# qitianwu/SGFormer

Measured on AMD Instinct MI355X. Metric: SGFormer fwd+bwd nodes/sec on ogbn-products full-graph, higher is better.
Workload: dtype bf16

## Files before the change

### include/sgf.h

```cpp
#ifndef SGF_H_
#define SGF_H_

#include <stddef.h>
#include <stdint.h>

#ifdef __cplusplus
extern "C" {
#endif

#define SGF_VERSION 666

#define SGF_F32 0
#define SGF_BF16 1
#define SGF_F32_BF16X3 2

#define SGF_OK 0
#define SGF_E_INVALID (-1)
#define SGF_E_WORKSPACE (-2)
#define SGF_E_HIP (-3)
#define SGF_E_UNSUPPORTED (-4)

int sgf_version(void);
const char* sgf_last_error(void);
int sgf_reload_env(void);

size_t sgf_csr_workspace_bytes(int64_t nnz, int64_t n);
int sgf_csr_build(const int64_t* edge_index, int64_t nnz, int64_t n, int64_t* rowptr,
                  int32_t* colind, float* val, int32_t* deg, void* workspace,
                  size_t workspace_bytes, void* stream);

int sgf_csr_transpose(const int64_t* edge_index, int64_t nnz, int64_t n, const int32_t* deg,
                      const int64_t* rowptr, const int32_t* colind, int64_t* t_rowptr,
                      int32_t* t_colind, float* t_val, int32_t* is_symmetric, void* workspace,
                      size_t workspace_bytes, void* stream);

size_t sgf_subgraph_workspace_bytes(int64_t nnz, int64_t n);
int sgf_subgraph_plan(const int64_t* edge_index, int64_t nnz, int64_t n, const int64_t* subset,
                      int64_t m, int32_t* relabel, int64_t* total, void* workspace,
                      size_t workspace_bytes, void* stream);
int sgf_subgraph_emit(const int64_t* edge_index, int64_t nnz, int64_t n, const int32_t* relabel,
                      int32_t relabel_nodes, int64_t total, int64_t* out, int64_t* out_eid,
                      void* workspace, size_t workspace_bytes, void* stream);

size_t sgf_subgraph_csr_plan_workspace_bytes(int64_t m);
size_t sgf_subgraph_csr_emit_workspace_bytes(int64_t m, int64_t total);
int sgf_subgraph_csr_plan(const int64_t* rowptr, const int32_t* colind, int64_t n, const int64_t* subset, int64_t m,
                          int32_t* local_of, int64_t* rowptr_b, int32_t* deg_b, int64_t* total, void* workspace,
                          size_t workspace_bytes, void* stream);
int sgf_subgraph_csr_emit(const int64_t* rowptr, const int32_t* colind, int64_t n, const int64_t* subset, int64_t m,
                          int32_t* local_of, const int64_t* rowptr_b, const int32_t* deg_b, int64_t total, int32_t* colind_b,
                          float* val_b, int64_t* edge_index_b, void* workspace, size_t workspace_bytes, void* stream);

size_t sgf_graph_prologue_workspace_bytes(int64_t m, int64_t n);
int sgf_graph_prologue_plan(const int64_t* edge_index, int64_t m, int64_t n, int32_t to_undirected,
                            int32_t remove_self_loops, int32_t add_self_loops, int64_t* total,
                            void* workspace, size_t workspace_bytes, void* stream);
int sgf_graph_prologue_emit(int64_t m, int64_t n, int32_t to_undirected, int32_t add_self_loops,
                            int64_t total, int64_t* out, void* workspace, size_t workspace_bytes,
                            void* stream);

int sgf_spmm(const int64_t* rowptr, const int32_t* colind, const float* val, const void* x,
             int64_t ldx, int64_t n_cols, void* y, int64_t ldy, int64_t n_rows, int32_t d,
             int32_t dtype, void* stream);

int32_t sgf_spmm_segment_len(void);
int32_t sgf_spmm_arm(int32_t d, int32_t dtype, int64_t ldx, int64_t ldy, int64_t n_cols, int32_t aligned16,
                     int32_t stream);
size_t sgf_spmm_split_workspace_bytes(int64_t long_segments, int32_t d);
int sgf_spmm_split(const int64_t* rowptr, const int32_t* colind, const float* val, const void* x,
                   int64_t ldx, int64_t n_cols, void* y, int64_t ldy, int64_t n_rows, int32_t d, int32_t dtype,
                   int64_t long_len, int64_t long_segments, void* workspace, size_t workspace_bytes,
                   void* stream);

size_t sgf_spmm_packed_bytes(int64_t n, int32_t slot_bytes);
int32_t sgf_spmm_packed_supported(int32_t d, int32_t dtype, int64_t ldx, int64_t ldy, int64_t n_cols, int32_t aligned16,
                                  int32_t slot_bytes);
int sgf_spmm_packed(const int64_t* rowptr, const int32_t* colind, const float* val, const void* x, int64_t ldx,
                    int64_t n_cols, const void* packed, int32_t slot_bytes, const int32_t* overflow, void* y, int64_t ldy,
                    int64_t n_rows, int32_t d, int32_t dtype, int64_t long_len, int64_t long_segments, void* workspace,
                    size_t workspace_bytes, void* stream);

int sgf_spmm_stream(const int64_t* rowptr, const int32_t* colind, const float* val, const void* x,
                    int64_t ldx, int64_t n_cols, void* y, int64_t ldy, int64_t n_rows, int32_t d, int32_t dtype,
                    int64_t long_len, int64_t long_segments, void* workspace, size_t workspace_bytes,
                    void* stream);

size_t sgf_reorder_workspace_bytes(int64_t nnz, int64_t n);
int sgf_reorder(const int64_t* edge_index, int64_t nnz, int64_t n, int32_t iters1, int32_t iters2,
                int32_t* perm, int32_t* inv, int32_t* community, void* workspace, size_t workspace_bytes,
                void* stream);
size_t sgf_spmm_plan_workspace_bytes(int64_t nnz, int64_t n, int32_t rows_per_block);
int sgf_spmm_plan(const int64_t* rowptr, const int32_t* colind, const float* val, int64_t n, int64_t nnz,
                  int32_t rows_per_block, int32_t lds_rows, int64_t long_len, int32_t* ecode, float* eval,
// ... 26 lines not shown
int sgf_spmm_tile_pack_layout(const int32_t* blk_row, int64_t nb, const int64_t* tile_ptr, const void* tiles,
                              int64_t n_frag, int32_t* grp, int64_t* pool_units, void* workspace,
                              size_t workspace_bytes, void* stream);
int sgf_spmm_tile_pack(const int32_t* blk_row, int64_t nb, const int64_t* tile_ptr, const void* tiles, int64_t n_frag,
                       const int32_t* grp, void* pool, int64_t pool_units, void* stream);
int sgf_spmm_tile(const int32_t* blk_row, int64_t nb, int32_t block_rows, const int32_t* sh_ptr, const int32_t* sh_cols,
                  const int64_t* tile_ptr, const int32_t* grp, const void* pool, const int64_t* rem_rowptr,
                  const int32_t* rem_col, const float* rem_val, const void* x, int64_t ldx, int64_t n_cols, void* y, int64_t ldy,
                  int64_t n_rows, int32_t d, int32_t dtype, int64_t long_len, int64_t long_segments,
                  void* workspace, size_t workspace_bytes, void* stream);

size_t sgf_neighbor_sample_workspace_bytes(int64_t m, int64_t edge_cap);
int sgf_neighbor_sample_mark(int32_t* local_of, const int32_t* ids, int64_t count, int32_t base, void* stream);
int sgf_neighbor_sample_hop(const int64_t* rowptr, const int32_t* colind, const int32_t* frontier, int64_t m,
                            int32_t frontier_local0, int32_t fanout, uint64_t seed, uint64_t batch, int32_t hop,
                            int32_t* local_of, int32_t n_known, int64_t edge_cap, int32_t* edge_src_local,
                            int32_t* edge_dst_local, int32_t* src_global, int32_t* new_nodes, int64_t* counts,
                            void* workspace, size_t workspace_bytes, void* stream);

size_t sgf_neighbor_sample_batch_workspace_bytes(int64_t batch_size, const int32_t* fanouts, int32_t hops, int64_t* node_cap,
                                                  int64_t* edge_cap);
int sgf_neighbor_sample_batch(const int64_t* rowptr, const int32_t* colind, const int32_t* seeds, int64_t batch_size,
                              const int32_t* fanouts, int32_t hops, uint64_t seed, uint64_t batch, int32_t* local_of,
                              int32_t* nodes, int64_t node_cap, int32_t* edge_src_local, int32_t* edge_dst_local,
                              int64_t edge_cap, int64_t* counts, void* workspace, size_t workspace_bytes, void* stream);

int32_t sgf_sampled_csr_supported(int32_t max_fanout);
size_t sgf_sampled_csr_build_workspace_bytes(int64_t node_cap, int64_t edge_cap);
int sgf_sampled_csr_build(const int32_t* edge_src_local, const int32_t* edge_dst_local, const int64_t* counts,
                          int64_t node_cap, int64_t edge_cap, int32_t max_fanout, int64_t* rowptr_b, int32_t* colind_b,
                          float* val_b, int32_t* deg_b, void* workspace, size_t workspace_bytes, void* stream);
size_t sgf_sampled_csr_transpose_workspace_bytes(int64_t n, int64_t nnz);
int sgf_sampled_csr_transpose(const int64_t* rowptr, const int32_t* colind, const float* val, int64_t n, int64_t nnz,
                              int64_t* t_rowptr, int32_t* t_colind, float* t_val, void* workspace, size_t workspace_bytes,
                              void* stream);

int sgf_gather_rows(const void* src, int64_t lds, int32_t src_dtype, int64_t n_src, const void* idx,
                    int32_t idx_is_int64, int64_t n_out, int32_t d, void* dst, int64_t ldd,
                    int32_t dst_dtype, void* stream);
int sgf_pad_rows(const void* src, int64_t lds, int32_t src_dtype, int64_t n_src, const void* idx, int32_t idx_is_int64,
                 int64_t n_out, int32_t d, int32_t d_pad, void* dst, int64_t ldd, int32_t dst_dtype, void* stream);

int64_t sgf_attn_stats_len(int32_t heads, int32_t d);
size_t sgf_attn_workspace_bytes(int64_t n, int32_t heads, int32_t d);
int32_t sgf_attn_max_blocks(void);
int32_t sgf_attn_tile_rows(int32_t kind, int32_t d, int32_t dtype);

int sgf_attn_fwd_reduce(const void* q, int64_t ldq, const void* k, int64_t ldk, const void* v,
                        int64_t ldv, int64_t n, int32_t heads, int32_t v_heads, int32_t d,
                        int32_t dtype, float* stats, void* workspace, size_t workspace_bytes,
                        void* stream);

int sgf_attn_fwd_apply(const void* q, int64_t ldq, const void* v, int64_t ldv, int64_t n,
                       double n_total, int32_t heads, int32_t v_heads, int32_t d, int32_t dtype,
                       const float* stats, void* out, int64_t ldo, float* den, void* o_heads,
                       void* stream);

int64_t sgf_attn_bstats_len(int32_t heads, int32_t d);

int sgf_attn_bwd_reduce(const void* q, int64_t ldq, const void* g, int64_t ldg, const void* o,
                        int64_t ldo, const float* den, int64_t n, int32_t heads, int32_t d,
                        int32_t dtype, float* bstats, void* workspace, size_t workspace_bytes,
                        void* stream);

int sgf_attn_bwd_apply(const void* q, int64_t ldq, const void* k, int64_t ldk, const void* v,
                       int64_t ldv, const void* g, int64_t ldg, const void* o, int64_t ldo,
                       const float* den, int64_t n, double n_total, int32_t heads,
                       int32_t v_heads, int32_t d, int32_t dtype, const float* stats,
                       float* bstats, void* dq, int64_t lddq, void* dk, int64_t lddk,
                       void* dv, int64_t lddv, void* stream);
int sgf_attn_bwd_reduce_heads(const void* q, int64_t ldq, const void* g, int64_t ldg, const void* o, int64_t ldo,
                              const float* den, int64_t n, int32_t heads, int32_t d, int32_t dtype, float* bstats,
                              void* workspace, size_t workspace_bytes, void* stream);
int sgf_attn_bwd_apply_heads(const void* q, int64_t ldq, const void* k, int64_t ldk, const void* v, int64_t ldv, const void* g,
                             int64_t ldg, const void* o, int64_t ldo, const float* den, int64_t n, double n_total,
                             int32_t heads, int32_t v_heads, int32_t d, int32_t dtype, const float* stats, float* bstats,
                             void* dq, int64_t lddq, void* dk, int64_t lddk, void* dv, int64_t lddv, void* stream);

int64_t sgf_attn_h_bstats_len(int32_t d);
int32_t sgf_attn_h_supported(int32_t d, int32_t dtype);
int sgf_attn_h_fwd(const void* h, int64_t ldh, int64_t n, int32_t d, int32_t dtype, const float* M,
                   const float* m, const float* w, const float* beta, void* out, int64_t ldo,
                   float* den, void* stream);
int sgf_attn_h_bwd_reduce(const void* h, int64_t ldh, const void* g, int64_t ldg, const void* o,
                          int64_t ldo, const float* den, int64_t n, int32_t d, int32_t dtype,
                          float* hstats, void* workspace, size_t workspace_bytes, void* stream);
int sgf_attn_h_bwd_apply(const void* h, int64_t ldh, const void* g, int64_t ldg, const void* o,
                         int64_t ldo, const float* den, int64_t n, int32_t d, int32_t dtype,
                         const float* M, const float* w, const float* D, const float* ds, void* dh,
                         int64_t lddh, void* workspace, size_t workspace_bytes, void* stream);
size_t sgf_attn_h_bwd_apply_workspace_bytes(int64_t n, int32_t d, int32_t dtype);
int32_t sgf_attn_h_bwd_split_supported(int32_t d, int32_t dtype);
int sgf_attn_h_bwd_pre(const void* g, int64_t ldg, const void* o, int64_t ldo, const float* den, int64_t n, int32_t d,
                       int32_t dtype, const float* M, const float* w, void* workspace, size_t workspace_bytes,
                       float* rowscal, void* stream);
int sgf_attn_h_bwd_reduce_scaled(const void* h, int64_t ldh, const void* g, int64_t ldg, const float* rowscal, int64_t n,
                                 int32_t d, int32_t dtype, float* hstats, void* workspace, size_t workspace_bytes,
                                 void* stream);
int sgf_attn_h_bwd_post(const void* h, int64_t ldh, int64_t n, int32_t d, int32_t dtype, const float* D, const float* ds,
                        const void* workspace, size_t workspace_bytes, const void* addend, int64_t ldadd, void* dh,
                        int64_t lddh, void* stream);

size_t sgf_attn_h_small_saved_bytes(int32_t d_in, int32_t d_out);
size_t sgf_attn_h_small_workspace_bytes(int32_t d_in, int32_t d_out);
int sgf_attn_h_small_fwd(const float* G, int64_t ldg, const float* s, float n_rows, float n_total, const float* wq,
                         const float* bq, const float* wk, const float* bk, const float* wv, const float* bv, int64_t ldw,
                         int32_t d_in, int32_t d_out, float* M, int64_t ldm, float* m, float* w, float* beta, void* saved,
                         size_t saved_bytes, void* stream);
int sgf_attn_h_small_bwd(const float* dM, int64_t lddm, const float* dw, const float* dm, const float* dbeta, float n_total,
                         int32_t d_in, int32_t d_out, const void* saved, size_t saved_bytes, float* dG2, int64_t lddg,
                         float* ds, float* gwq, float* gbq, float* gwk, float* gbk, float* gwv, float* gbv, int64_t ldgw,
                         void* workspace, size_t workspace_bytes, void* stream);

size_t sgf_gram_workspace_bytes(int64_t n, int32_t m, int32_t k);
int sgf_gram(const void* a, int64_t lda, int32_t m, const void* b, int64_t ldb, int32_t k,
             int64_t n, int32_t dtype, float* c, int64_t ldc, float* colsum_a, void* workspace,
             size_t workspace_bytes, void* stream);
int sgf_gram2(const void* a, int64_t lda, int32_t m, const void* b1, int64_t ldb1, const void* b2, int64_t ldb2, int32_t k,
              int64_t n, int32_t dtype, float* c1, int64_t ldc1, float* c2, int64_t ldc2, float* colsum_a, void* workspace,
              size_t workspace_bytes, void* stream);

int sgf_ln_fwd(const void* x, int64_t ldx, const void* res, int64_t ldr, float a, float b,
               const float* gamma, const float* beta, int32_t relu, float eps, int64_t n,
               int32_t d, int32_t dtype, void* y, int64_t ldy, float* mean, float* rstd,
               void* stream);

size_t sgf_ln_bwd_workspace_bytes(int64_t n, int32_t d);
int sgf_ln_bwd(const void* dy, int64_t lddy, const void* y, int64_t ldy, const void* x,
               int64_t ldx, const void* res, int64_t ldr, float a, float b, const float* gamma,
               int32_t relu, const float* mean, const float* rstd, int64_t n, int32_t d,
               int32_t dtype, void* dx, int64_t lddx, void* dres, int64_t lddres, float* dgamma,
               float* dbeta, void* workspace, size_t workspace_bytes, void* stream);

size_t sgf_colstats_workspace_bytes(int64_t n, int32_t d);
int sgf_colstats(const void* x, int64_t ldx, const float* shift, int64_t n, int32_t d,
                 int32_t dtype, float* stats, void* workspace, size_t workspace_bytes,
                 void* stream);
int sgf_bn_finalize(const float* sums, const float* shift, double n_total, float eps, float momentum, float* running_mean,
                    float* running_var, int32_t d, float* mean, float* rstd, void* stream);
int sgf_bn_apply(const void* x, int64_t ldx, const float* mean, const float* rstd,
                 const float* gamma, const float* beta, const void* res, int64_t ldr,
                 int32_t relu, int64_t n, int32_t d, int32_t dtype, void* y, int64_t ldy,
                 void* stream);
int sgf_bn_apply_packed(const void* x, int64_t ldx, const float* mean, const float* rstd, const float* gamma,
                        const float* beta, const void* res, int64_t ldr, int32_t relu, int64_t n, int32_t d, int32_t dtype,
                        void* y, int64_t ldy, void* packed, int32_t slot_bytes, int32_t* overflow, void* stream);
int sgf_bn_bwd_stats(const void* dy, int64_t lddy, const void* x, int64_t ldx, const float* mean,
                     const float* rstd, const float* gamma, const float* beta, int32_t relu,
                     int64_t n, int32_t d, int32_t dtype, float* stats, void* workspace,
                     size_t workspace_bytes, void* stream);
int sgf_bn_bwd_stats2(const void* dy, int64_t lddy, const void* dy2, int64_t lddy2, const void* x, int64_t ldx,
                      const float* mean, const float* rstd, const float* gamma, const float* beta, int32_t relu, int64_t n,
                      int32_t d, int32_t dtype, float* stats, void* workspace, size_t workspace_bytes, void* stream);
int32_t sgf_gram_ln_bwd_supported(int32_t m, int32_t k, int32_t dtype);
int sgf_gram_ln_bwd(const void* g, int64_t ldg, const void* xin, int64_t ldx, const float* mean, const float* rstd,
                    const float* gamma, const float* beta, int32_t relu, int32_t m, const void* b, int64_t ldb, int32_t k,
                    int64_t n, int32_t dtype, float* c, int64_t ldc, float* colsum, float* dgamma, float* dbeta, void* workspace,
                    size_t workspace_bytes, void* stream);
int32_t sgf_gram_bn_bwd_supported(int32_t m, int32_t k, int32_t dtype);
int sgf_gram_bn_bwd(const void* g1, int64_t ldg1, const void* g2, int64_t ldg2, const void* z, int64_t ldz, const float* mean,
                    const float* rstd, const float* gamma, const float* beta, int32_t relu, const float* stats, float inv_n,
                    int32_t training, int32_t m, const void* b, int64_t ldb, int32_t k, int64_t n, int32_t dtype, float* c,
                    int64_t ldc, float* colsum, void* workspace, size_t workspace_bytes, void* stream);
int32_t sgf_gram2_bn_bwd_supported(int32_t m, int32_t k, int64_t n, int32_t dtype);
int sgf_gram2_bn_bwd(const void* g, int64_t ldg, const void* z, int64_t ldz, const float* mean, const float* rstd,
                     const float* gamma, const float* beta, int32_t relu, const float* stats, float inv_n, int32_t training,
                     int32_t m, const void* b1, int64_t ldb1, const void* b2, int64_t ldb2, int32_t k, int64_t n, int32_t dtype,
                     void* dz, int64_t lddz, float* c1, int64_t ldc1, float* c2, int64_t ldc2, float* colsum, void* workspace,
                     size_t workspace_bytes, void* stream);
int sgf_bn_bwd_apply(const void* dy, int64_t lddy, const void* x, int64_t ldx, const float* mean,
                     const float* rstd, const float* gamma, const float* beta, int32_t relu,
                     const float* stats, float inv_n, int32_t training, int64_t n, int32_t d,
                     int32_t dtype, void* dx, int64_t lddx, void* stream);

int32_t sgf_combine_fc_supported(int32_t d, int32_t classes, int32_t dtype);
int sgf_combine_fc_fwd(const void* x1, int64_t ld1, float a, const void* x2, int64_t ld2, float b,
                       const float* w, const float* bias, int64_t n, int32_t d, int32_t classes,
                       int32_t dtype, float* logits, int64_t ldl, void* stream);
int sgf_combine_fc_bwd(const float* dlogits, int64_t lddl, const float* w, int64_t n, int32_t d,
                       int32_t classes, float a, float b, int32_t dtype, void* dx1, int64_t ld1, void* dx2,
                       int64_t ld2, void* stream);
int sgf_combine_fc_fwd_mapped(const void* x1, int64_t ld1, float a, const void* x2, int64_t ld2, float b, const float* w,
                              const float* bias, int64_t n, int32_t d, int32_t classes, int32_t dtype, float* logits,
                              int64_t ldl, const int32_t* row_map, void* stream);
int sgf_combine_fc_bwd_mapped(const float* dlogits, int64_t lddl, const float* w, int64_t n, int32_t d, int32_t classes,
                              float a, float b, int32_t dtype, void* dx1, int64_t ld1, void* dx2, int64_t ld2,
                              const int32_t* row_map, void* stream);
int sgf_combine_fc_bwd_g(const float* dlogits, int64_t lddl, const float* w, int64_t n, int32_t d, int32_t classes, float a,
                         float b, int32_t dtype, void* dx1, int64_t ld1, void* dx2, int64_t ld2, const int32_t* row_map,
                         void* g_out, int64_t ldg, void* stream);

int32_t sgf_gcn_epilogue_supported(int32_t d_in, int32_t d_out, int32_t dtype);
size_t sgf_gcn_epilogue_workspace_bytes(int64_t n, int32_t d_out);
int sgf_gcn_epilogue_stats(const void* a, int64_t lda, const void* w, int64_t ldw, const float* bias,
                           int64_t n, int32_t d_in, int32_t d_out, int32_t dtype, void* y, int64_t ldy,
                           const float* shift, float* stats, void* workspace, size_t workspace_bytes,
                           void* stream);
int sgf_gcn_epilogue_dx2(const void* dy, int64_t lddy, const void* w1, const void* w2, int64_t ldw, int64_t n, int32_t d,
                         int32_t dtype, void* dx1, int64_t lddx1, void* dx2, int64_t lddx2, int32_t pair, void* stream);

int32_t sgf_gcn_epilogue_dx2_acc_supported(int32_t d, int32_t dtype);
int sgf_gcn_epilogue_dx2_acc(const void* dz, int64_t lddz, const void* w, int64_t ldw, int64_t n, int32_t d, int32_t dtype,
                             void* dy, int64_t lddy, const void* gadd, int64_t ldg, const void* acc_in, int64_t ldai,
                             void* acc_out, int64_t ldao, void* stream);
int sgf_gcn_epilogue_dx(const void* dy, int64_t lddy, const void* w, int64_t ldw, int64_t n, int32_t d_in,
                        int32_t d_out, int32_t dtype, void* dx, int64_t lddx, void* stream);
int sgf_gcn_epilogue_apply(const void* y, int64_t ldy, const float* mean, const float* rstd, const float* gamma,
                           const float* beta, const void* res, int64_t ldr, int32_t relu, int64_t n, int32_t d,
                           int32_t dtype, void* out, int64_t ldo, void* stream);
int32_t sgf_gcn_bn_bwd_dx_supported(int32_t d, int32_t dtype);
size_t sgf_gcn_bn_bwd_dx_workspace_bytes(int64_t n, int32_t d);
int sgf_gcn_bn_bwd_dx(const void* gy, int64_t ldg, const void* z, int64_t ldz, const float* mean, const float* rstd,
                      const float* gamma, const float* beta, int32_t relu, const float* stats, float inv_n,
                      int32_t training, const void* w, int64_t ldw, int64_t n, int32_t d, int32_t dtype, void* dz,
                      int64_t lddz, void* dy, int64_t lddy, const void* acc_in, void* acc_out, size_t acc_bytes,
                      void* dx0, int64_t lddx0, int32_t add_gy, void* workspace, size_t workspace_bytes, void* stream);
int32_t sgf_gcn_epilogue_cat_supported(int32_t d, int32_t dtype);
int sgf_gcn_epilogue_cat(const void* a1, int64_t lda1, const void* a2, int64_t lda2, const void* w, int64_t ldw,
                         const float* bias, int64_t n, int32_t d, int32_t dtype, void* y, int64_t ldy, const float* shift,
                         float* stats, void* workspace, size_t workspace_bytes, void* stream);
size_t sgf_gcn_epilogue_partial_bytes(int64_t n, int32_t d_out);
size_t sgf_gcn_epilogue_dtype_partial_bytes(int64_t n, int32_t d_out, int32_t dtype);
int sgf_gcn_epilogue_partial(const void* a, int64_t lda, const void* w, int64_t ldw, const float* bias, int64_t n,
                             int32_t d_in, int32_t d_out, int32_t dtype, void* partial, size_t partial_bytes,
                             void* stream);
int sgf_gcn_epilogue_stats_add(const void* a, int64_t lda, const void* w, int64_t ldw, const void* partial,
                               size_t partial_bytes, int64_t n, int32_t d_in, int32_t d_out, int32_t dtype,
                               void* y, int64_t ldy, const float* shift, float* stats, void* workspace,
                               size_t workspace_bytes, void* stream);

int32_t sgf_stem_pair_supported(int32_t d_in, int32_t d_out, int32_t dtype);
int32_t sgf_row_lap_rows(int32_t kind, int32_t d, int32_t dtype);
int sgf_stem_pair(const void* x, int64_t ldx, int64_t n, int32_t d_in, const void* w0, int64_t ldw0,
                  const float* bias0, const void* w1, int64_t ldw1, const float* bias1, int32_t d_out, int32_t dtype,
                  void* y0, int64_t ldy0, void* y1, int64_t ldy1, const float* shift0, float* stats0, void* workspace,
                  size_t workspace_bytes, void* stream);

int sgf_gemm(const void* a, int64_t a_rs, int64_t a_cs, int32_t a_dtype, const void* b, int64_t b_rs, int64_t b_cs,
             int32_t b_dtype, int64_t m, int32_t n, int64_t k, float alpha, const float* alpha_dev, const float* bias,
             float beta, const void* addend, int64_t ldadd, int32_t add_dtype, void* c, int64_t ldc, int32_t c_dtype,
             void* stream);

int sgf_axpby(const void* x1, int64_t ld1, float a, const void* x2, int64_t ld2, float b,
              int64_t n, int32_t d, int32_t dtype, void* y, int64_t ldy, void* stream);

int sgf_dropout(const void* x, int64_t ldx, const void* res, int64_t ldr, float p, uint64_t seed,
                int64_t n, int32_t d, int32_t dtype, void* y, int64_t ldy, void* stream);

int sgf_dropout_dev(const void* x, int64_t ldx, const void* res, int64_t ldr, float p,
                    const uint64_t* seed_slot, int64_t n, int32_t d, int32_t dtype, void* y, int64_t ldy,
                    void* stream);

size_t sgf_nll_workspace_bytes(int64_t m);
int sgf_nll_fwd(const void* logits, int64_t ldl, int64_t n, int32_t c, int32_t dtype,
                const int64_t* labels, const int64_t* idx, int64_t m, float* loss_sum,
                void* workspace, size_t workspace_bytes, void* stream);
int sgf_nll_bwd(const void* logits, int64_t ldl, int64_t n, int32_t c, int32_t dtype,
                const int64_t* labels, const int64_t* idx, int64_t m, const float* gout,
                float inv_denom, void* dlogits, int64_t ldd, void* stream);

#define SGF_BCE_TARGET_F32 0
#define SGF_BCE_TARGET_I64 1
#define SGF_BCE_TARGET_CLASS 2
size_t sgf_bce_workspace_bytes(int64_t m, int32_t c);
int sgf_bce_fwd(const void* logits, int64_t ldl, int64_t n, int32_t c, int32_t dtype, const void* target,
                int64_t ldt, int32_t target_kind, const int64_t* idx, int64_t m, float inv_denom,
                float* loss_sum, void* workspace, size_t workspace_bytes, void* stream);
int sgf_bce_bwd(const void* logits, int64_t ldl, int64_t n, int32_t c, int32_t dtype, const void* target,
                int64_t ldt, int32_t target_kind, const int64_t* idx, int64_t m, const float* gout,
                float inv_denom, void* dlogits, int64_t ldd, void* stream);

#define SGF_METRIC_TARGET_F32 0
#define SGF_METRIC_TARGET_I64 1
size_t sgf_rocauc_workspace_bytes(int64_t m, int32_t c);
int sgf_rocauc_counts(const void* logits, int64_t ldl, int64_t n, int32_t c, int32_t dtype, const void* target,
                      int64_t ldt, int32_t target_kind, const int64_t* idx, int64_t m, int64_t* counts,
                      void* workspace, size_t workspace_bytes, void* stream);
size_t sgf_argmax_workspace_bytes(int64_t m, int32_t c);
int sgf_argmax_count(const void* logits, int64_t ldl, int64_t n, int32_t c, int32_t dtype, const void* labels,
                     int64_t label_stride, int32_t label_kind, const int64_t* idx, int64_t m, int64_t* counts,
                     void* workspace, size_t workspace_bytes, void* stream);

int32_t sgf_head_rows_supported(int32_t d, int32_t classes, int32_t dtype);
size_t sgf_head_rows_fwd_workspace_bytes(int64_t m);
size_t sgf_head_rows_bwd_workspace_bytes(int64_t m, int32_t d, int32_t classes);
int sgf_head_rows_fwd(const void* x1, int64_t ld1, float a, const void* x2, int64_t ld2, float b, const float* w,
                      const float* bias, int64_t n, int32_t d, int32_t classes, int32_t dtype, const int64_t* idx,
                      int64_t m, float* logits, int64_t ldl, const int64_t* labels, float* lse, float* loss_sum,
                      int64_t* counts, void* workspace, size_t workspace_bytes, void* stream);
int sgf_head_rows_bwd(const void* x1, int64_t ld1, float a, const void* x2, int64_t ld2, float b, const float* w,
                      int64_t n, int32_t d, int32_t classes, int32_t dtype, const int64_t* idx, int64_t m,
                      const float* dlogits, int64_t lddl, const float* logits, int64_t ldl, const float* lse,
                      const int64_t* labels, const float* gout, float inv_denom, void* dx1, int64_t ldd1, void* dx2,
                      int64_t ldd2, float* dw, float* db, void* workspace, size_t workspace_bytes, void* stream);

int32_t sgf_pair_sigmoid_supported(int32_t heads, int32_t v_heads, int32_t d, int32_t dtype);
size_t sgf_pair_sigmoid_workspace_bytes(int64_t n, int64_t l, int32_t heads);
int64_t sgf_pair_sigmoid_lap_rows(int32_t which, int32_t heads, int32_t d, int32_t dtype, int32_t laps);
int sgf_pair_sigmoid_fwd(const void* q, int64_t ldq, const void* k, int64_t ldk, const void* v, int64_t ldv, int64_t n,
                         int64_t l, int32_t heads, int32_t v_heads, int32_t d, int32_t dtype, void* out, int64_t ldo,
                         float* rowsum, void* stream);
int sgf_pair_sigmoid_bwd_q(const void* g, int64_t ldg, const void* out, int64_t ldo, const float* rowsum, const void* q,
                           int64_t ldq, const void* k, int64_t ldk, const void* v, int64_t ldv, int64_t n, int64_t l,
                           int32_t heads, int32_t v_heads, int32_t d, int32_t dtype, void* dq, int64_t lddq, void* workspace,
                           size_t workspace_bytes, void* stream);
int sgf_pair_sigmoid_bwd_kv(const void* g, int64_t ldg, const float* rowsum, const void* q, int64_t ldq, const void* k,
                            int64_t ldk, const void* v, int64_t ldv, int64_t n, int64_t l, int32_t heads, int32_t v_heads,
                            int32_t d, int32_t dtype, void* dk, int64_t lddk, void* dv, int64_t lddv, const void* workspace,
                            size_t workspace_bytes, void* stream);

int sgf_sum_n(const void* const* xs_host, const int64_t* lds_host, int32_t k, int64_t n, int32_t d,
              int32_t dtype, void* y, int64_t ldy, void* stream);

size_t sgf_colsum_workspace_bytes(int64_t n, int32_t d);
int sgf_colsum(const void* x, int64_t ldx, int64_t n, int32_t d, int32_t dtype, float* out,
               void* workspace, size_t workspace_bytes, void* stream);

int32_t sgf_comm_available(void);
int32_t sgf_comm_unique_id_bytes(void);
// ... 13 lines not shown
```

### sgformer_amd/_lib.py

```python
from __future__ import annotations

import ctypes
import os
from ctypes import c_char_p, c_double, c_float, c_int32, c_int64, c_size_t, c_uint64, c_void_p

_HERE = os.path.dirname(os.path.abspath(__file__))
LIB_PATH = os.path.join(_HERE, "lib", "libsgf.so")

SGF_F32 = 0
SGF_BF16 = 1
SGF_F32_BF16X3 = 2
SGF_OK = 0
SGF_E_INVALID = -1
SGF_E_WORKSPACE = -2
SGF_E_HIP = -3
SGF_E_UNSUPPORTED = -4
SGF_BCE_TARGET_F32 = 0
SGF_BCE_TARGET_I64 = 1
SGF_BCE_TARGET_CLASS = 2
SGF_METRIC_TARGET_F32 = 0
SGF_METRIC_TARGET_I64 = 1

_lib = None

# ... 6 lines not shown
    "sgf_csr_build": (c_int32, [_P, c_int64, c_int64, _P, _P, _P, _P, _P, c_size_t, _P]),
    "sgf_csr_transpose": (c_int32, [_P, c_int64, c_int64, _P, _P, _P, _P, _P, _P, _P, _P, c_size_t, _P]),
    "sgf_subgraph_workspace_bytes": (c_size_t, [c_int64, c_int64]),
    "sgf_subgraph_plan": (c_int32, [_P, c_int64, c_int64, _P, c_int64, _P, _P, _P, c_size_t, _P]),
    "sgf_subgraph_emit": (c_int32, [_P, c_int64, c_int64, _P, c_int32, c_int64, _P, _P, _P, c_size_t, _P]),
    "sgf_subgraph_csr_plan_workspace_bytes": (c_size_t, [c_int64]),
    "sgf_subgraph_csr_emit_workspace_bytes": (c_size_t, [c_int64, c_int64]),
    "sgf_subgraph_csr_plan": (c_int32, [_P, _P, c_int64, _P, c_int64, _P, _P, _P, _P, _P, c_size_t, _P]),
    "sgf_subgraph_csr_emit": (c_int32, [_P, _P, c_int64, _P, c_int64, _P, _P, _P, c_int64, _P, _P, _P, _P, c_size_t, _P]),
    "sgf_graph_prologue_workspace_bytes": (c_size_t, [c_int64, c_int64]),
    "sgf_graph_prologue_plan": (c_int32, [_P, c_int64, c_int64, c_int32, c_int32, c_int32, _P, _P, c_size_t, _P]),
    "sgf_graph_prologue_emit": (c_int32, [c_int64, c_int64, c_int32, c_int32, c_int64, _P, _P, c_size_t, _P]),
    "sgf_spmm": (c_int32, [_P, _P, _P, _P, c_int64, c_int64, _P, c_int64, c_int64, c_int32, c_int32, _P]),
    "sgf_spmm_segment_len": (c_int32, []),
    "sgf_spmm_arm": (c_int32, [c_int32, c_int32, c_int64, c_int64, c_int64, c_int32, c_int32]),
    "sgf_spmm_split_workspace_bytes": (c_size_t, [c_int64, c_int32]),
    "sgf_spmm_split": (c_int32, [_P, _P, _P, _P, c_int64, c_int64, _P, c_int64, c_int64, c_int32, c_int32, c_int64,
                                 c_int64, _P, c_size_t, _P]),
    "sgf_spmm_packed_bytes": (c_size_t, [c_int64, c_int32]),
    "sgf_spmm_packed_supported": (c_int32, [c_int32, c_int32, c_int64, c_int64, c_int64, c_int32, c_int32]),
    "sgf_spmm_packed": (c_int32, [_P, _P, _P, _P, c_int64, c_int64, _P, c_int32, _P, _P, c_int64, c_int64, c_int32, c_int32,
                                  c_int64, c_int64, _P, c_size_t, _P]),
    "sgf_spmm_stream": (c_int32, [_P, _P, _P, _P, c_int64, c_int64, _P, c_int64, c_int64, c_int32, c_int32, c_int64,
                                  c_int64, _P, c_size_t, _P]),
    "sgf_reorder_workspace_bytes": (c_size_t, [c_int64, c_int64]),
    "sgf_reorder": (c_int32, [_P, c_int64, c_int64, c_int32, c_int32, _P, _P, _P, _P, c_size_t, _P]),
    "sgf_spmm_plan_workspace_bytes": (c_size_t, [c_int64, c_int64, c_int32]),
    "sgf_spmm_plan": (c_int32, [_P, _P, _P, c_int64, c_int64, c_int32, c_int32, c_int64, _P, _P, _P, _P, _P, _P,
                                _P, c_size_t, _P]),
    "sgf_spmm_lds_rows_len": (c_int32, [c_int32]),
    "sgf_spmm_blocked_arm": (c_int32, [c_int32, c_int32, c_int64, c_int64, c_int64, c_int32, c_int32, c_int32]),
    "sgf_spmm_blocked": (c_int32, [_P, _P, _P, _P, _P, _P, _P, c_int64, _P, c_int64, c_int64, c_int32, c_int32,
                                   c_int32, c_int32, c_int64, c_int64, _P, c_size_t, _P]),
    "sgf_spmm_tile_supported": (c_int32, [c_int32, c_int32]),
    "sgf_spmm_tile_blocks": (c_int32, [_P, c_int64, c_int32, _P, c_int64, _P, _P]),
    "sgf_spmm_tile_plan_workspace_bytes": (c_size_t, [c_int64, c_int64, c_int64]),
    "sgf_spmm_tile_plan": (c_int32, [_P, _P, _P, c_int64, c_int64, _P, c_int64, c_int32, c_int32, c_int64, _P, _P, _P,
                                     _P, _P, _P, _P, _P, _P, c_size_t, _P]),
    "sgf_spmm_tile_fill": (c_int32, [_P, _P, _P, _P, c_int64, c_int64, _P, c_int64, _P, c_int64, _P, _P, _P, _P, _P]),
    "sgf_spmm_tile_sparse_len": (c_int32, []),
    "sgf_spmm_tile_pack_workspace_bytes": (c_size_t, [c_int64]),
    "sgf_spmm_tile_pack_layout": (c_int32, [_P, c_int64, _P, _P, c_int64, _P, _P, _P, c_size_t, _P]),
    "sgf_spmm_tile_pack": (c_int32, [_P, c_int64, _P, _P, c_int64, _P, _P, c_int64, _P]),
    "sgf_spmm_tile": (c_int32, [_P, c_int64, c_int32, _P, _P, _P, _P, _P, _P, _P, _P, _P, c_int64, c_int64, _P, c_int64,
                                c_int64, c_int32, c_int32, c_int64, c_int64, _P, c_size_t, _P]),
    "sgf_neighbor_sample_workspace_bytes": (c_size_t, [c_int64, c_int64]),
    "sgf_neighbor_sample_mark": (c_int32, [_P, _P, c_int64, c_int32, _P]),
    "sgf_neighbor_sample_batch_workspace_bytes": (c_size_t, [c_int64, _P, c_int32, _P, _P]),
    "sgf_neighbor_sample_batch": (c_int32, [_P, _P, _P, c_int64, _P, c_int32, c_uint64, c_uint64, _P, _P, c_int64, _P, _P,
                                            c_int64, _P, _P, c_size_t, _P]),
    "sgf_neighbor_sample_hop": (c_int32, [_P, _P, _P, c_int64, c_int32, c_int32, c_uint64, c_uint64, c_int32, _P, c_int32,
                                          c_int64, _P, _P, _P, _P, _P, _P, c_size_t, _P]),
    "sgf_sampled_csr_supported": (c_int32, [c_int32]),
    "sgf_sampled_csr_build_workspace_bytes": (c_size_t, [c_int64, c_int64]),
    "sgf_sampled_csr_build": (c_int32, [_P, _P, _P, c_int64, c_int64, c_int32, _P, _P, _P, _P, _P, c_size_t, _P]),
    "sgf_sampled_csr_transpose_workspace_bytes": (c_size_t, [c_int64, c_int64]),
    "sgf_sampled_csr_transpose": (c_int32, [_P, _P, _P, c_int64, c_int64, _P, _P, _P, _P, c_size_t, _P]),
    "sgf_gather_rows": (c_int32, [_P, c_int64, c_int32, c_int64, _P, c_int32, c_int64, c_int32, _P, c_int64,
                                  c_int32, _P]),
    "sgf_pad_rows": (c_int32, [_P, c_int64, c_int32, c_int64, _P, c_int32, c_int64, c_int32, c_int32, _P, c_int64,
                               c_int32, _P]),
    "sgf_attn_stats_len": (c_int64, [c_int32, c_int32]),
    "sgf_attn_bstats_len": (c_int64, [c_int32, c_int32]),
    "sgf_attn_workspace_bytes": (c_size_t, [c_int64, c_int32, c_int32]),
    "sgf_attn_max_blocks": (c_int32, []),
    "sgf_attn_tile_rows": (c_int32, [c_int32, c_int32, c_int32]),
    "sgf_row_lap_rows": (c_int32, [c_int32, c_int32, c_int32]),
    "sgf_attn_fwd_reduce": (c_int32, [_P, c_int64, _P, c_int64, _P, c_int64, c_int64, c_int32, c_int32,
                                      c_int32, c_int32, _P, _P, c_size_t, _P]),
    "sgf_attn_fwd_apply": (c_int32, [_P, c_int64, _P, c_int64, c_int64, c_double, c_int32, c_int32,
                                     c_int32, c_int32, _P, _P, c_int64, _P, _P, _P]),
    "sgf_attn_bwd_reduce": (c_int32, [_P, c_int64, _P, c_int64, _P, c_int64, _P, c_int64, c_int32,
                                      c_int32, c_int32, _P, _P, c_size_t, _P]),
    "sgf_attn_bwd_apply": (c_int32, [_P, c_int64, _P, c_int64, _P, c_int64, _P, c_int64, _P, c_int64,
                                     _P, c_int64, c_double, c_int32, c_int32, c_int32, c_int32, _P, _P,
                                     _P, c_int64, _P, c_int64, _P, c_int64, _P]),
    "sgf_attn_bwd_reduce_heads": (c_int32, [_P, c_int64, _P, c_int64, _P, c_int64, _P, c_int64, c_int32,
                                            c_int32, c_int32, _P, _P, c_size_t, _P]),
    "sgf_attn_bwd_apply_heads": (c_int32, [_P, c_int64, _P, c_int64, _P, c_int64, _P, c_int64, _P, c_int64,
                                           _P, c_int64, c_double, c_int32, c_int32, c_int32, c_int32, _P, _P,
                                           _P, c_int64, _P, c_int64, _P, c_int64, _P]),
    "sgf_attn_h_bstats_len": (c_int64, [c_int32]),
    "sgf_attn_h_fwd": (c_int32, [_P, c_int64, c_int64, c_int32, c_int32, _P, _P, _P, _P, _P, c_int64, _P, _P]),
    "sgf_attn_h_bwd_reduce": (c_int32, [_P, c_int64, _P, c_int64, _P, c_int64, _P, c_int64, c_int32, c_int32,
                                        _P, _P, c_size_t, _P]),
    "sgf_attn_h_bwd_apply": (c_int32, [_P, c_int64, _P, c_int64, _P, c_int64, _P, c_int64, c_int32, c_int32,
                                       _P, _P, _P, _P, _P, c_int64, _P, c_size_t, _P]),
    "sgf_attn_h_bwd_apply_workspace_bytes": (c_size_t, [c_int64, c_int32, c_int32]),
    "sgf_attn_h_bwd_split_supported": (c_int32, [c_int32, c_int32]),
    "sgf_attn_h_supported": (c_int32, [c_int32, c_int32]),
    "sgf_attn_h_bwd_pre": (c_int32, [_P, c_int64, _P, c_int64, _P, c_int64, c_int32, c_int32, _P, _P, _P, c_size_t, _P, _P]),
    "sgf_attn_h_bwd_reduce_scaled": (c_int32, [_P, c_int64, _P, c_int64, _P, c_int64, c_int32, c_int32, _P, _P, c_size_t,
                                               _P]),
    "sgf_attn_h_bwd_post": (c_int32, [_P, c_int64, c_int64, c_int32, c_int32, _P, _P, _P, c_size_t, _P, c_int64, _P,
                                      c_int64, _P]),
    "sgf_attn_h_small_saved_bytes": (c_size_t, [c_int32, c_int32]),
    "sgf_attn_h_small_workspace_bytes": (c_size_t, [c_int32, c_int32]),
    "sgf_attn_h_small_fwd": (c_int32, [_P, c_int64, _P, c_float, c_float, _P, _P, _P, _P, _P, _P, c_int64, c_int32, c_int32,
                                       _P, c_int64, _P, _P, _P, _P, c_size_t, _P]),
    "sgf_attn_h_small_bwd": (c_int32, [_P, c_int64, _P, _P, _P, c_float, c_int32, c_int32, _P, c_size_t, _P, c_int64, _P,
                                       _P, _P, _P, _P, _P, _P, c_int64, _P, c_size_t, _P]),
    "sgf_gram_workspace_bytes": (c_size_t, [c_int64, c_int32, c_int32]),
    "sgf_gram": (c_int32, [_P, c_int64, c_int32, _P, c_int64, c_int32, c_int64, c_int32, _P, c_int64, _P,
                           _P, c_size_t, _P]),
    "sgf_gram2": (c_int32, [_P, c_int64, c_int32, _P, c_int64, _P, c_int64, c_int32, c_int64, c_int32, _P, c_int64, _P,
                            c_int64, _P, _P, c_size_t, _P]),
    "sgf_ln_fwd": (c_int32, [_P, c_int64, _P, c_int64, c_float, c_float, _P, _P, c_int32, c_float,
                             c_int64, c_int32, c_int32, _P, c_int64, _P, _P, _P]),
    "sgf_ln_bwd_workspace_bytes": (c_size_t, [c_int64, c_int32]),
    "sgf_ln_bwd": (c_int32, [_P, c_int64, _P, c_int64, _P, c_int64, _P, c_int64, c_float, c_float, _P,
                             c_int32, _P, _P, c_int64, c_int32, c_int32, _P, c_int64, _P, c_int64, _P,
                             _P, _P, c_size_t, _P]),
    "sgf_colstats_workspace_bytes": (c_size_t, [c_int64, c_int32]),
    "sgf_colstats": (c_int32, [_P, c_int64, _P, c_int64, c_int32, c_int32, _P, _P, c_size_t, _P]),
    "sgf_bn_finalize": (c_int32, [_P, _P, c_double, c_float, c_float, _P, _P, c_int32, _P, _P, _P]),
    "sgf_bn_apply": (c_int32, [_P, c_int64, _P, _P, _P, _P, _P, c_int64, c_int32, c_int64, c_int32,
                               c_int32, _P, c_int64, _P]),
    "sgf_bn_apply_packed": (c_int32, [_P, c_int64, _P, _P, _P, _P, _P, c_int64, c_int32, c_int64, c_int32, c_int32, _P,
                                      c_int64, _P, c_int32, _P, _P]),
    "sgf_bn_bwd_stats": (c_int32, [_P, c_int64, _P, c_int64, _P, _P, _P, _P, c_int32, c_int64, c_int32,
                                   c_int32, _P, _P, c_size_t, _P]),
    "sgf_bn_bwd_stats2": (c_int32, [_P, c_int64, _P, c_int64, _P, c_int64, _P, _P, _P, _P, c_int32, c_int64, c_int32,
                                    c_int32, _P, _P, c_size_t, _P]),
    "sgf_gram_ln_bwd_supported": (c_int32, [c_int32, c_int32, c_int32]),
    "sgf_gram_ln_bwd": (c_int32, [_P, c_int64, _P, c_int64, _P, _P, _P, _P, c_int32, c_int32, _P, c_int64, c_int32, c_int64,
                                  c_int32, _P, c_int64, _P, _P, _P, _P, c_size_t, _P]),
    "sgf_gram_bn_bwd_supported": (c_int32, [c_int32, c_int32, c_int32]),
    "sgf_gram_bn_bwd": (c_int32, [_P, c_int64, _P, c_int64, _P, c_int64, _P, _P, _P, _P, c_int32, _P, c_float, c_int32,
                                  c_int32, _P, c_int64, c_int32, c_int64, c_int32, _P, c_int64, _P, _P, c_size_t, _P]),
    "sgf_gram2_bn_bwd_supported": (c_int32, [c_int32, c_int32, c_int64, c_int32]),
    "sgf_gram2_bn_bwd": (c_int32, [_P, c_int64, _P, c_int64, _P, _P, _P, _P, c_int32, _P, c_float, c_int32, c_int32, _P, c_int64,
                                   _P, c_int64, c_int32, c_int64, c_int32, _P, c_int64, _P, c_int64, _P, c_int64, _P, _P,
                                   c_size_t, _P]),
    "sgf_bn_bwd_apply": (c_int32, [_P, c_int64, _P, c_int64, _P, _P, _P, _P, c_int32, _P, c_float,
                                   c_int32, c_int64, c_int32, c_int32, _P, c_int64, _P]),
    "sgf_dropout": (c_int32, [_P, c_int64, _P, c_int64, c_float, c_uint64, c_int64, c_int32, c_int32, _P,
                              c_int64, _P]),
    "sgf_dropout_dev": (c_int32, [_P, c_int64, _P, c_int64, c_float, _P, c_int64, c_int32, c_int32, _P,
                                  c_int64, _P]),
    "sgf_nll_workspace_bytes": (c_size_t, [c_int64]),
    "sgf_nll_fwd": (c_int32, [_P, c_int64, c_int64, c_int32, c_int32, _P, _P, c_int64, _P, _P, c_size_t, _P]),
    "sgf_nll_bwd": (c_int32, [_P, c_int64, c_int64, c_int32, c_int32, _P, _P, c_int64, _P, c_float, _P,
                              c_int64, _P]),
    "sgf_bce_workspace_bytes": (c_size_t, [c_int64, c_int32]),
    "sgf_bce_fwd": (c_int32, [_P, c_int64, c_int64, c_int32, c_int32, _P, c_int64, c_int32, _P, c_int64, c_float, _P, _P,
                              c_size_t, _P]),
    "sgf_bce_bwd": (c_int32, [_P, c_int64, c_int64, c_int32, c_int32, _P, c_int64, c_int32, _P, c_int64, _P, c_float, _P,
                              c_int64, _P]),
    "sgf_rocauc_workspace_bytes": (c_size_t, [c_int64, c_int32]),
    "sgf_rocauc_counts": (c_int32, [_P, c_int64, c_int64, c_int32, c_int32, _P, c_int64, c_int32, _P, c_int64, _P, _P,
                                    c_size_t, _P]),
    "sgf_argmax_workspace_bytes": (c_size_t, [c_int64, c_int32]),
    "sgf_argmax_count": (c_int32, [_P, c_int64, c_int64, c_int32, c_int32, _P, c_int64, c_int32, _P, c_int64, _P, _P,
                                   c_size_t, _P]),
    "sgf_head_rows_supported": (c_int32, [c_int32, c_int32, c_int32]),
    "sgf_head_rows_fwd_workspace_bytes": (c_size_t, [c_int64]),
    "sgf_head_rows_bwd_workspace_bytes": (c_size_t, [c_int64, c_int32, c_int32]),
    "sgf_head_rows_fwd": (c_int32, [_P, c_int64, c_float, _P, c_int64, c_float, _P, _P, c_int64, c_int32, c_int32, c_int32,
                                    _P, c_int64, _P, c_int64, _P, _P, _P, _P, _P, c_size_t, _P]),
    "sgf_head_rows_bwd": (c_int32, [_P, c_int64, c_float, _P, c_int64, c_float, _P, c_int64, c_int32, c_int32, c_int32,
                                    _P, c_int64, _P, c_int64, _P, c_int64, _P, _P, _P, c_float, _P, c_int64, _P, c_int64,
                                    _P, _P, _P, c_size_t, _P]),
    "sgf_pair_sigmoid_supported": (c_int32, [c_int32, c_int32, c_int32, c_int32]),
    "sgf_pair_sigmoid_workspace_bytes": (c_size_t, [c_int64, c_int64, c_int32]),
    "sgf_pair_sigmoid_lap_rows": (c_int64, [c_int32, c_int32, c_int32, c_int32, c_int32]),
    "sgf_pair_sigmoid_fwd": (c_int32, [_P, c_int64, _P, c_int64, _P, c_int64, c_int64, c_int64, c_int32, c_int32, c_int32,
                                       c_int32, _P, c_int64, _P, _P]),
    "sgf_pair_sigmoid_bwd_q": (c_int32, [_P, c_int64, _P, c_int64, _P, _P, c_int64, _P, c_int64, _P, c_int64, c_int64,
                                         c_int64, c_int32, c_int32, c_int32, c_int32, _P, c_int64, _P, c_size_t, _P]),
    "sgf_pair_sigmoid_bwd_kv": (c_int32, [_P, c_int64, _P, _P, c_int64, _P, c_int64, _P, c_int64, c_int64, c_int64, c_int32,
                                          c_int32, c_int32, c_int32, _P, c_int64, _P, c_int64, _P, c_size_t, _P]),
    "sgf_sum_n": (c_int32, [_P, _P, c_int32, c_int64, c_int32, c_int32, _P, c_int64, _P]),
    "sgf_colsum_workspace_bytes": (c_size_t, [c_int64, c_int32]),
    "sgf_colsum": (c_int32, [_P, c_int64, c_int64, c_int32, c_int32, _P, _P, c_size_t, _P]),
    "sgf_combine_fc_supported": (c_int32, [c_int32, c_int32, c_int32]),
    "sgf_combine_fc_fwd": (c_int32, [_P, c_int64, c_float, _P, c_int64, c_float, _P, _P, c_int64, c_int32, c_int32,
                                     c_int32, _P, c_int64, _P]),
    "sgf_combine_fc_bwd": (c_int32, [_P, c_int64, _P, c_int64, c_int32, c_int32, c_float, c_float, c_int32, _P,
                                     c_int64, _P, c_int64, _P]),
    "sgf_combine_fc_fwd_mapped": (c_int32, [_P, c_int64, c_float, _P, c_int64, c_float, _P, _P, c_int64, c_int32, c_int32,
                                     c_int32, _P, c_int64, _P, _P]),
    "sgf_combine_fc_bwd_g": (c_int32, [_P, c_int64, _P, c_int64, c_int32, c_int32, c_float, c_float, c_int32, _P, c_int64, _P,
                                       c_int64, _P, _P, c_int64, _P]),
    "sgf_combine_fc_bwd_mapped": (c_int32, [_P, c_int64, _P, c_int64, c_int32, c_int32, c_float, c_float, c_int32, _P,
                                     c_int64, _P, c_int64, _P, _P]),
    "sgf_gcn_epilogue_supported": (c_int32, [c_int32, c_int32, c_int32]),
    "sgf_gcn_epilogue_workspace_bytes": (c_size_t, [c_int64, c_int32]),
    "sgf_gcn_epilogue_stats": (c_int32, [_P, c_int64, _P, c_int64, _P, c_int64, c_int32, c_int32, c_int32, _P, c_int64,
                                         _P, _P, _P, c_size_t, _P]),
    "sgf_gcn_epilogue_dx": (c_int32, [_P, c_int64, _P, c_int64, c_int64, c_int32, c_int32, c_int32, _P, c_int64, _P]),
    "sgf_gcn_epilogue_dx2": (c_int32, [_P, c_int64, _P, _P, c_int64, c_int64, c_int32, c_int32, _P, c_int64, _P, c_int64,
                                       c_int32, _P]),
    "sgf_gcn_epilogue_dx2_acc_supported": (c_int32, [c_int32, c_int32]),
    "sgf_gcn_epilogue_dx2_acc": (c_int32, [_P, c_int64, _P, c_int64, c_int64, c_int32, c_int32, _P, c_int64, _P, c_int64, _P,
                                           c_int64, _P, c_int64, _P]),
    "sgf_gcn_epilogue_apply": (c_int32, [_P, c_int64, _P, _P, _P, _P, _P, c_int64, c_int32, c_int64, c_int32,
                               c_int32, _P, c_int64, _P]),
    "sgf_gcn_bn_bwd_dx_supported": (c_int32, [c_int32, c_int32]),
    "sgf_gcn_bn_bwd_dx_workspace_bytes": (c_size_t, [c_int64, c_int32]),
    "sgf_gcn_bn_bwd_dx": (c_int32, [_P, c_int64, _P, c_int64, _P, _P, _P, _P, c_int32, _P, c_float, c_int32, _P, c_int64,
                                    c_int64, c_int32, c_int32, _P, c_int64, _P, c_int64, _P, _P, c_size_t, _P, c_int64,
                                    c_int32, _P, c_size_t, _P]),
    "sgf_gcn_epilogue_cat_supported": (c_int32, [c_int32, c_int32]),
    "sgf_gcn_epilogue_cat": (c_int32, [_P, c_int64, _P, c_int64, _P, c_int64, _P, c_int64, c_int32, c_int32, _P, c_int64,
                                       _P, _P, _P, c_size_t, _P]),
    "sgf_gcn_epilogue_partial_bytes": (c_size_t, [c_int64, c_int32]),
    "sgf_gcn_epilogue_dtype_partial_bytes": (c_size_t, [c_int64, c_int32, c_int32]),
    "sgf_gcn_epilogue_partial": (c_int32, [_P, c_int64, _P, c_int64, _P, c_int64, c_int32, c_int32, c_int32, _P,
                                           c_size_t, _P]),
    "sgf_gcn_epilogue_stats_add": (c_int32, [_P, c_int64, _P, c_int64, _P, c_size_t, c_int64, c_int32, c_int32,
                                             c_int32, _P, c_int64, _P, _P, _P, c_size_t, _P]),
    "sgf_stem_pair_supported": (c_int32, [c_int32, c_int32, c_int32]),
    "sgf_stem_pair": (c_int32, [_P, c_int64, c_int64, c_int32, _P, c_int64, _P, _P, c_int64, _P, c_int32, c_int32, _P,
                                c_int64, _P, c_int64, _P, _P, _P, c_size_t, _P]),
    "sgf_gemm": (c_int32, [_P, c_int64, c_int64, c_int32, _P, c_int64, c_int64, c_int32, c_int64, c_int32, c_int64, c_float,
                           _P, _P, c_float, _P, c_int64, c_int32, _P, c_int64, c_int32, _P]),
    "sgf_comm_available": (c_int32, []),
    "sgf_comm_unique_id_bytes": (c_int32, []),
    "sgf_comm_unique_id": (c_int32, [_P]),
    "sgf_comm_create": (c_int32, [_P, c_int32, c_int32, _P]),
    "sgf_comm_destroy": (c_int32, [_P]),
    "sgf_comm_all_reduce_f32": (c_int32, [_P, _P, c_int64, _P]),
    "sgf_comm_all_gather": (c_int32, [_P, _P, _P, c_int64, _P]),
    "sgf_comm_all_to_all": (c_int32, [_P, _P, _P, _P, _P, _P, _P, _P]),
    "sgf_axpby": (c_int32, [_P, c_int64, c_float, _P, c_int64, c_float, c_int64, c_int32, c_int32, _P,
                            c_int64, _P]),
}


class SgfError(RuntimeError):
    """A libsgf call returned a non-zero status (mirrors PyTorch: RuntimeError)."""


def load():
    global _lib
    if _lib is not None:
        return _lib
    if not os.path.exists(LIB_PATH):
        raise SgfError(
            f"libsgf.so not found at {LIB_PATH}: build it with `make` (or "
            "`python -c 'import __graft_entry__ as g; g.build()'`).  sgformer_amd has no CPU / "
            "eager fallback by design.")
    import torch
    lib = ctypes.CDLL(LIB_PATH, mode=ctypes.RTLD_GLOBAL)
    for name, (res, args) in SIGNATURES.items():
        fn = getattr(lib, name)
        fn.restype = res
        fn.argtypes = args
    _lib = lib
    return lib


def available() -> bool:
    return os.path.exists(LIB_PATH)


def check(rc: int, what: str):
    if rc != SGF_OK:
        msg = load().sgf_last_error()
        raise SgfError(f"{what} failed (rc={rc}): {msg.decode() if msg else '?'}")


def call(name: str, *args):
    rc = getattr(load(), name)(*args)
    check(rc, name)
```

### sgformer_amd/csrc/head.hip

```cpp
#include "common.h"

namespace sgf {
namespace {

typedef short bf16x8 __attribute__((ext_vector_type(8)));

constexpr int kHeadThreads = 256;
constexpr int kMaxClasses = 64;

__device__ __forceinline__ uint32_t pack2(float lo, float hi) {
  return static_cast<uint32_t>(f32_to_bf16(lo)) | (static_cast<uint32_t>(f32_to_bf16(hi)) << 16);
}
__device__ __forceinline__ float lo16(uint32_t u) { return __uint_as_float(u << 16); }
__device__ __forceinline__ float hi16(uint32_t u) { return __uint_as_float(u & 0xffff0000u); }

union Frag {
  bf16x8 v;
  uint4 u;
};

template <int DP>
__global__ __launch_bounds__(kHeadThreads) void k_head_fwd_bf16(
    const uint16_t* __restrict__ x1, int64_t ld1, float a, const uint16_t* __restrict__ x2, int64_t ld2, float b,
    const float* __restrict__ w, const float* __restrict__ bias, int64_t n, int d, int c,
// ... 101 lines not shown
  unsigned char* const patch = patch_all + wid * 32 * PROW;
  unsigned char* const pw = patch + 4 * hi * PROW + 2 * i31;
  const unsigned char* const pr = patch + (lane / LPR) * PROW + 16 * (lane % LPR);
  const int ks = (c + 15) / 16;
  const int64_t ntiles = (n + 31) / 32;
  constexpr int W = kHeadBwdThreads / 64;

  struct Raw {
    float g[KSMAX][8];
  };
  auto row_of = [&](int64_t t) -> int32_t {
    int64_t row = t * 32 + i31;
    if (row >= n) row = n - 1;
    if (t >= ntiles) return 0;
    return rmap ? rmap[row] : static_cast<int32_t>(row);
  };
  auto load_raw = [&](int32_t row, Raw& r) {
    const float* pg = dl + static_cast<int64_t>(row) * lddl;
#pragma unroll
    for (int s = 0; s < KSMAX; ++s) {
      if (s < ks) {
        const int k0 = 16 * s + 8 * hi;
#pragma unroll
        for (int j = 0; j < 8; ++j) r.g[s][j] = pg[k0 + j < c ? k0 + j : c - 1];
      }
    }
  };
  auto pack_frags = [&](const Raw& r, Frag (&fa)[KSMAX]) {
#pragma unroll
    for (int s = 0; s < KSMAX; ++s) {
      if (s < ks) {
        const int k0 = 16 * s + 8 * hi;
        float g[8];
#pragma unroll
        for (int j = 0; j < 8; ++j) g[j] = k0 + j < c ? r.g[s][j] : 0.f;
        fa[s].u.x = pack2(g[0], g[1]);
        fa[s].u.y = pack2(g[2], g[3]);
        fa[s].u.z = pack2(g[4], g[5]);
        fa[s].u.w = pack2(g[6], g[7]);
      }
    }
  };

  Frag cur[KSMAX];
  Raw raw_cur, raw_nxt;
  int64_t tile = static_cast<int64_t>(blockIdx.x) * W + wid;
  const int64_t step = static_cast<int64_t>(gridDim.x) * W;
  int32_t row_nxt = 0;
  if (tile < ntiles) {
    load_raw(row_of(tile), raw_cur);
    row_nxt = row_of(tile + step);
  }
  for (; tile < ntiles; tile += step) {
    const bool more = tile + step < ntiles;
    if (more) load_raw(row_nxt, raw_nxt);
    const int32_t row_nn = row_of(tile + 2 * step);
    pack_frags(raw_cur, cur);
    if (gout != nullptr && tile * 32 + i31 < n) {
#pragma unroll
      for (int s = 0; s < KSMAX; ++s)
        if (s < ks) *reinterpret_cast<uint4*>(gout + (tile * 32 + i31) * ldgo + 16 * s + 8 * hi) = cur[s].u;
    }
#pragma unroll
    for (int h = 0; h < NH; ++h) {
      if (HW * h >= d) break;
      f32x16 acc[NT];
#pragma unroll
      for (int t = 0; t < NT; ++t)
#pragma unroll
        for (int r = 0; r < 16; ++r) acc[t][r] = 0.f;
#pragma unroll
      for (int s = 0; s < KSMAX; ++s) {
        if (s < ks) {
          const int k0 = 16 * s + 8 * hi;
#pragma unroll
          for (int t = 0; t < NT; ++t) {
            const bf16x8 bt = *reinterpret_cast<const bf16x8*>(&wt[(HW * h + 32 * t + i31) * PITCH + k0]);
            acc[t] = __builtin_amdgcn_mfma_f32_32x32x16_bf16(cur[s].v, bt, acc[t], 0, 0, 0);
          }
        }
      }
#pragma unroll
      for (int which = 0; which < 2; ++which) {
        const float sc = which == 0 ? a : b;
        uint16_t* const dst = which == 0 ? dx1 : dx2;
        const int64_t ld = which == 0 ? ld1 : ld2;
#pragma unroll
        for (int t = 0; t < NT; ++t) {
#pragma unroll
          for (int r = 0; r < 16; r += 2) {
            const uint32_t v = pack2(sc * acc[t][r], sc * acc[t][r + 1]);
            const int rl = (r & 3) + 8 * (r >> 2);
            *reinterpret_cast<uint16_t*>(pw + rl * PROW + 64 * t) = static_cast<uint16_t>(v & 0xffffu);
            *reinterpret_cast<uint16_t*>(pw + (rl + 1) * PROW + 64 * t) = static_cast<uint16_t>(v >> 16);
          }
        }
        __builtin_amdgcn_fence(__ATOMIC_RELEASE, "wavefront");
        __builtin_amdgcn_wave_barrier();
        __builtin_amdgcn_fence(__ATOMIC_ACQUIRE, "wavefront");
        const int fcol = HW * h + 8 * (lane % LPR);
#pragma unroll
        for (int j = 0; j < 32 / RPI; ++j) {
          const uint4 v = *reinterpret_cast<const uint4*>(pr + RPI * j * PROW);
          const int64_t orow = tile * 32 + RPI * j + lane / LPR;
          if (fcol < d && orow < n) *reinterpret_cast<uint4*>(dst + orow * ld + fcol) = v;
        }
        __builtin_amdgcn_fence(__ATOMIC_RELEASE, "wavefront");
        __builtin_amdgcn_wave_barrier();
        __builtin_amdgcn_fence(__ATOMIC_ACQUIRE, "wavefront");
      }
    }
    raw_cur = raw_nxt;
    row_nxt = row_nn;
  }
}

inline int head_grid(int64_t n) {
  int64_t b = (n + 127) / 128;
  const int64_t cap = static_cast<int64_t>(kNumCU) * 4;
  if (b > cap) b = cap;
  if (b < 1) b = 1;
  return static_cast<int>(b);
}

inline int head_bwd_grid(int64_t n) {
  int64_t nb = ((n + 31) / 32 + kHeadBwdThreads / 64 - 1) / (kHeadBwdThreads / 64);
  if (nb > kNumCU) nb = kNumCU;
  return static_cast<int>(nb);
}

int check_head(const char* fn, int64_t n, int d, int c, int dtype) {
  SGF_REQUIRE(n >= 0 && d > 0 && c > 0, SGF_E_INVALID, "%s: bad size", fn);
  if (f32_storage(dtype)) {
    SGF_REQUIRE(linear_f32_supported(d, c), SGF_E_UNSUPPORTED,
                "%s: fp32 storage needs d and classes multiples of 4 up to 256 (d=%d, classes=%d; pad the class rows of W)", fn, d, c);
    return SGF_OK;
  }
  SGF_REQUIRE(dtype == SGF_BF16, SGF_E_UNSUPPORTED, "%s: unknown dtype %d", fn, dtype);
  if (c > kMaxClasses) {
    SGF_REQUIRE(linear_f32_supported(d, c), SGF_E_UNSUPPORTED,
                "%s: more than %d classes need d and classes multiples of 4 up to 256 (d=%d, classes=%d)", fn, kMaxClasses, d, c);
    return SGF_OK;
  }
  SGF_REQUIRE(d % 32 == 0 && d <= 256 && c <= kMaxClasses, SGF_E_UNSUPPORTED,
              "%s: needs d %% 32 == 0, d <= 256, classes <= %d (d=%d, classes=%d)", fn, kMaxClasses, d, c);
  return SGF_OK;
}

}

int64_t head_lap_rows(bool bwd, int64_t n) {
  return bwd ? static_cast<int64_t>(head_bwd_grid(n)) * (kHeadBwdThreads / 64) * 32
             : static_cast<int64_t>(head_grid(n)) * (kHeadThreads / 64) * 32;
}

}

using namespace sgf;

extern "C" int32_t sgf_combine_fc_supported(int32_t d, int32_t classes, int32_t dtype) {
  if (f32_storage(dtype)) return linear_f32_supported(d, classes) ? 1 : 0;
  if (dtype != SGF_BF16 || d <= 0 || classes <= 0) return 0;
  if (classes > kMaxClasses) return linear_f32_supported(d, classes) ? 1 : 0;
  return d % 32 == 0 && d <= 256 ? 1 : 0;
}

static int combine_fc_fwd_impl(const char* fn, const void* x1, int64_t ld1, float a, const void* x2, int64_t ld2, float b,
                               const float* w, const float* bias, int64_t n, int32_t d, int32_t classes, int32_t dtype,
                               float* logits, int64_t ldl, const int32_t* rmap, void* stream) {
  int rc = check_head(fn, n, d, classes, dtype);
  if (rc != SGF_OK) return rc;
  if (n == 0) return SGF_OK;
  SGF_REQUIRE(!rmap || (dtype == SGF_BF16 && classes <= kMaxClasses), SGF_E_UNSUPPORTED,
              "%s: a row map needs bf16 storage and at most %d classes", fn, kMaxClasses);
  if (f32_storage(dtype)) {
    SGF_REQUIRE(x1 && x2 && w && logits && ld1 >= d && ld2 >= d && ldl >= classes, SGF_E_INVALID,
                "%s: bad pointer / ld", fn);
    return linear_f32_dual(x1, ld1, x2, ld2, a, b, n, d, classes, w, d, 1, bias, logits, ldl, nullptr, 0, 1.f, 1.f, 0, 0,
                           static_cast<hipStream_t>(stream), dtype == SGF_F32_BF16X3);
  }
  if (classes > kMaxClasses) {
    SGF_REQUIRE(x1 && x2 && w && logits && ld1 >= d && ld2 >= d && ldl >= classes, SGF_E_INVALID,
                "%s: bad pointer / ld", fn);
    return linear_f32_dual(x1, ld1, x2, ld2, a, b, n, d, classes, w, d, 1, bias, logits, ldl, nullptr, 0, 1.f, 1.f, 1, 0,
                           static_cast<hipStream_t>(stream));
  }
  SGF_REQUIRE(x1 && x2 && w && bias && logits && ld1 % 8 == 0 && ld2 % 8 == 0 && ld1 >= d && ld2 >= d && ldl >= classes,
              SGF_E_INVALID, "%s: bad pointer / ld", fn);
  SGF_REQUIRE(reinterpret_cast<uintptr_t>(x1) % 16 == 0 && reinterpret_cast<uintptr_t>(x2) % 16 == 0 &&
                  reinterpret_cast<uintptr_t>(w) % 16 == 0,
              SGF_E_INVALID, "%s: x1 / x2 / w must be 16-byte aligned", fn);
  hipStream_t st = static_cast<hipStream_t>(stream);
  const dim3 grid(head_grid(n)), block(kHeadThreads);
#define SGF_HEAD_FWD(DP_)                                                                                        \
  hipLaunchKernelGGL((k_head_fwd_bf16<DP_>), grid, block, 0, st, static_cast<const uint16_t*>(x1), ld1, a,       \
                     static_cast<const uint16_t*>(x2), ld2, b, w, bias, n, d, classes, logits, ldl, rmap)
  if (d <= 64) SGF_HEAD_FWD(64);
  else if (d <= 128) SGF_HEAD_FWD(128);
  else SGF_HEAD_FWD(256);
#undef SGF_HEAD_FWD
  SGF_LAUNCH_CHECK();
  return SGF_OK;
}

extern "C" int sgf_combine_fc_fwd(const void* x1, int64_t ld1, float a, const void* x2, int64_t ld2, float b,
                                  const float* w, const float* bias, int64_t n, int32_t d, int32_t classes,
                                  int32_t dtype, float* logits, int64_t ldl, void* stream) {
  return combine_fc_fwd_impl("sgf_combine_fc_fwd", x1, ld1, a, x2, ld2, b, w, bias, n, d, classes, dtype, logits, ldl, nullptr,
                             stream);
}

extern "C" int sgf_combine_fc_fwd_mapped(const void* x1, int64_t ld1, float a, const void* x2, int64_t ld2, float b,
                                         const float* w, const float* bias, int64_t n, int32_t d, int32_t classes,
                                         int32_t dtype, float* logits, int64_t ldl, const int32_t* row_map, void* stream) {
  SGF_REQUIRE(row_map || n == 0, SGF_E_INVALID, "sgf_combine_fc_fwd_mapped: null row_map");
  return combine_fc_fwd_impl("sgf_combine_fc_fwd_mapped", x1, ld1, a, x2, ld2, b, w, bias, n, d, classes, dtype, logits, ldl,
                             row_map, stream);
}

static int combine_fc_bwd_impl(const char* fn, const float* dlogits, int64_t lddl, const float* w, int64_t n, int32_t d,
                               int32_t classes, float a, float b, int32_t dtype, void* dx1, int64_t ld1, void* dx2,
                               int64_t ld2, const int32_t* rmap, void* stream, void* gout = nullptr, int64_t ldgo = 0) {
  int rc = check_head(fn, n, d, classes, dtype);
  if (rc != SGF_OK) return rc;
  if (n == 0) return SGF_OK;
  SGF_REQUIRE(!rmap || (dtype == SGF_BF16 && classes <= kMaxClasses), SGF_E_UNSUPPORTED,
              "%s: a row map needs bf16 storage and at most %d classes", fn, kMaxClasses);
  if (f32_storage(dtype)) {
    SGF_REQUIRE(dlogits && w && dx1 && dx2 && lddl >= classes && ld1 >= d && ld2 >= d, SGF_E_INVALID,
                "%s: bad pointer / ld", fn);
    return linear_f32_dual(dlogits, lddl, nullptr, 0, 1.f, 0.f, n, classes, d, w, d, 0, nullptr, dx1, ld1, dx2, ld2, a, b, 0, 0,
                           static_cast<hipStream_t>(stream), dtype == SGF_F32_BF16X3);
  }
  if (classes > kMaxClasses) {
    SGF_REQUIRE(dlogits && w && dx1 && dx2 && lddl >= classes && ld1 >= d && ld2 >= d, SGF_E_INVALID,
                "%s: bad pointer / ld", fn);
    return linear_f32_dual(dlogits, lddl, nullptr, 0, 1.f, 0.f, n, classes, d, w, d, 0, nullptr, dx1, ld1, dx2, ld2, a, b, 0, 1,
                           static_cast<hipStream_t>(stream));
  }
  SGF_REQUIRE(dlogits && w && dx1 && dx2 && lddl >= classes && ld1 >= d && ld2 >= d && ld1 % 8 == 0 && ld2 % 8 == 0 &&
                  reinterpret_cast<uintptr_t>(dx1) % 16 == 0 && reinterpret_cast<uintptr_t>(dx2) % 16 == 0,
              SGF_E_INVALID, "%s: bad pointer / ld (dx1 / dx2: 16-byte aligned, ld %% 8 == 0)", fn);
  SGF_REQUIRE(n < (static_cast<int64_t>(1) << 31), SGF_E_UNSUPPORTED, "%s: more than 2^31 - 1 rows", fn);
  hipStream_t st = static_cast<hipStream_t>(stream);
  const dim3 grid(static_cast<unsigned>(head_bwd_grid(n))), block(kHeadBwdThreads);
#define SGF_HEAD_BWD(DP_)                                                                                   \
  hipLaunchKernelGGL((k_head_bwd_bf16<DP_>), grid, block, 0, st, dlogits, lddl, w, n, d, classes, a, b,       \
                     static_cast<uint16_t*>(dx1), ld1, static_cast<uint16_t*>(dx2), ld2, rmap,                \
                     static_cast<uint16_t*>(gout), ldgo)
  if (d <= 64) SGF_HEAD_BWD(64);
  else if (d <= 128) SGF_HEAD_BWD(128);
  else SGF_HEAD_BWD(256);
#undef SGF_HEAD_BWD
  SGF_LAUNCH_CHECK();
  return SGF_OK;
}

extern "C" int sgf_combine_fc_bwd(const float* dlogits, int64_t lddl, const float* w, int64_t n, int32_t d,
                                  int32_t classes, float a, float b, int32_t dtype, void* dx1, int64_t ld1,
                                  void* dx2, int64_t ld2, void* stream) {
  return combine_fc_bwd_impl("sgf_combine_fc_bwd", dlogits, lddl, w, n, d, classes, a, b, dtype, dx1, ld1, dx2, ld2, nullptr,
                             stream);
}

extern "C" int sgf_combine_fc_bwd_g(const float* dlogits, int64_t lddl, const float* w, int64_t n, int32_t d, int32_t classes,
                                    float a, float b, int32_t dtype, void* dx1, int64_t ld1, void* dx2, int64_t ld2,
                                    const int32_t* row_map, void* g_out, int64_t ldg, void* stream) {
  const char* fn = "sgf_combine_fc_bwd_g";
  SGF_REQUIRE(dtype == SGF_BF16 && classes >= 1 && classes <= kMaxClasses, SGF_E_UNSUPPORTED,
              "%s: bf16 storage and at most %d classes", fn, kMaxClasses);
  SGF_REQUIRE(n == 0 || (g_out && ldg >= (classes + 15) / 16 * 16 && ldg % 8 == 0 && reinterpret_cast<uintptr_t>(g_out) % 16 == 0),
              SGF_E_INVALID, "%s: g_out must be 16-byte aligned with ldg %% 8 == 0 and ldg >= classes rounded up to 16", fn);
  return combine_fc_bwd_impl(fn, dlogits, lddl, w, n, d, classes, a, b, dtype, dx1, ld1, dx2, ld2, row_map, stream, g_out, ldg);
}

extern "C" int sgf_combine_fc_bwd_mapped(const float* dlogits, int64_t lddl, const float* w, int64_t n, int32_t d,
                                         int32_t classes, float a, float b, int32_t dtype, void* dx1, int64_t ld1,
                                         void* dx2, int64_t ld2, const int32_t* row_map, void* stream) {
  SGF_REQUIRE(row_map || n == 0, SGF_E_INVALID, "sgf_combine_fc_bwd_mapped: null row_map");
  return combine_fc_bwd_impl("sgf_combine_fc_bwd_mapped", dlogits, lddl, w, n, d, classes, a, b, dtype, dx1, ld1, dx2, ld2,
                             row_map, stream);
}
```

### sgformer_amd/csrc/rowgemm.hip

```cpp
#include "common.h"

#include <cstdlib>

namespace sgf {
namespace {

typedef short bf16x8 __attribute__((ext_vector_type(8)));
typedef float f32x16 __attribute__((ext_vector_type(16)));
typedef float f32x2 __attribute__((ext_vector_type(2)));
typedef __bf16 bf16x2 __attribute__((ext_vector_type(2)));
typedef uint32_t u32x4 __attribute__((ext_vector_type(4)));

constexpr int kRgWaves = 8;
constexpr int kRgThreads = kRgWaves * 64;
constexpr int kStageStride = 144;
constexpr int kStageBytes = 16 * kStageStride;

struct RowGemmArgs {
  const uint16_t* a; int64_t lda;
  const uint16_t* w; int64_t ldw; int trans;
  const float* bias;
  const float* shift;
  float* spart;
  uint16_t* y; int64_t ldy;
// ... 768 lines not shown
    f32x16 acc[NS];
#pragma unroll
    for (int w = 0; w < NS; ++w)
#pragma unroll
      for (int r = 0; r < 16; ++r) acc[w][r] = 0.f;

#pragma unroll
    for (int half = 0; half < KS / RING; ++half) {
      if (half == role)
        bn_bwd_dx_phase<D, ROLES, true, DBG>(half, G, Z, acc, coef, bfrag0, identp, dzrsrc, dzoff, row_ok, grsrc, zrsrc, cg, cz,
                                             ng, nz, hi);
      else
        bn_bwd_dx_phase<D, ROLES, false, DBG>(half, G, Z, acc, coef, bfrag0, identp, dzrsrc, dzoff, row_ok, grsrc, zrsrc, cg, cz,
                                              ng, nz, hi);
    }

    const uint32_t acc_off = static_cast<uint32_t>((t * (NSD * 2 * 64) + (2 * role * 2) * 64 + lane) * 16);
    if (p.acc_in != nullptr) {
      u32x4 av[2][2];
#pragma unroll
      for (int c = 0; c < 2; ++c)
#pragma unroll
        for (int q = 0; q < 2; ++q)
          av[c][q] = __builtin_amdgcn_raw_buffer_load_b128(airsrc, static_cast<int>(acc_off + (c * 2 + q) * 1024), 0, kStreamIn);
#pragma unroll
      for (int c = 0; c < 2; ++c)
#pragma unroll
        for (int q = 0; q < 2; ++q) {
          const uint32_t d4[4] = {av[c][q].x, av[c][q].y, av[c][q].z, av[c][q].w};
#pragma unroll
          for (int e = 0; e < 4; ++e) {
            acc[2 + c][8 * q + 2 * e] += __uint_as_float(d4[e] << 16);
            acc[2 + c][8 * q + 2 * e + 1] += __uint_as_float(d4[e] & 0xffff0000u);
          }
        }
    }
#pragma unroll
    for (int u = 0; u < 2; ++u) {
      if (u == 1 && p.dx0 == nullptr) {
#pragma unroll
        for (int c = 0; c < 2; ++c)
#pragma unroll
          for (int q = 0; q < 2; ++q) {
            const u32x4 v = {cvt_pk_bf16(acc[2 + c][8 * q + 0], acc[2 + c][8 * q + 1]),
                             cvt_pk_bf16(acc[2 + c][8 * q + 2], acc[2 + c][8 * q + 3]),
                             cvt_pk_bf16(acc[2 + c][8 * q + 4], acc[2 + c][8 * q + 5]),
                             cvt_pk_bf16(acc[2 + c][8 * q + 6], acc[2 + c][8 * q + 7])};
            if (!(DBG & 4))
              __builtin_amdgcn_raw_buffer_store_b128(v, aorsrc, static_cast<int>(acc_off + (c * 2 + q) * 1024), 0, kStreamOut);
          }
        continue;
      }
      const int64_t ldo = u == 1 ? p.lddx0 : p.lddy;
      const uint32_t ooff = static_cast<uint32_t>(((row0 + (lane >> 3)) * ldo + c0 + 8 * (lane & 7)) * 2);
#pragma unroll
      for (int hh = 0; hh < 2; ++hh) {
#pragma unroll
        for (int c = 0; c < 2; ++c) {
#pragma unroll
          for (int r = 8 * hh; r < 8 * hh + 8; r += 2) {
            const uint32_t v = cvt_pk_bf16(acc[2 * u + c][r], acc[2 * u + c][r + 1]);
            const int rl = (r & 3) + 8 * ((r >> 2) & 1);
            *reinterpret_cast<uint16_t*>(st_w + rl * kStageStride + 64 * c) = static_cast<uint16_t>(v & 0xffffu);
            *reinterpret_cast<uint16_t*>(st_w + (rl + 1) * kStageStride + 64 * c) = static_cast<uint16_t>(v >> 16);
          }
        }
        wave_lds_sync();
#pragma unroll
        for (int q = 0; q < 2; ++q) {
          const uint4 v4 = *reinterpret_cast<const uint4*>(st_r + 8 * q * kStageStride);
          const u32x4 v = {v4.x, v4.y, v4.z, v4.w};
          const bool ok = !tail || row0 + 16 * hh + 8 * q + (lane >> 3) < p.n;
          const uint32_t off = ok ? ooff + static_cast<uint32_t>((16 * hh + 8 * q) * ldo * 2) : 0xffffff00u;
          if (DBG & 4) continue;
          if (u == 1) __builtin_amdgcn_raw_buffer_store_b128(v, dxrsrc, static_cast<int>(off), 0, kStreamOut);
          else __builtin_amdgcn_raw_buffer_store_b128(v, dyrsrc, static_cast<int>(off), 0, kStreamOut);
        }
        wave_lds_sync();
      }
    }
  }
}

constexpr int kHF = 0, kHB1 = 1, kHB2 = 2;

struct HRowArgs {
  const uint16_t* a; int64_t lda;
  const uint16_t* a2; int64_t lda2;
  const float* bmat; int trans_b;
  const float* cvec;
  const float* dvec; const float* beta;
  float* den;
  uint16_t* out; int64_t ldo;
  uint4* part;
  int64_t n;
  float2* rowscal;
  const uint16_t* addend; int64_t ldadd;
};

template <int D, int MODE>
__global__ __launch_bounds__(kRgThreads, 2) void k_hrow_bf16(HRowArgs p) {
  constexpr int KS = D / 16, NS = D / 32;
  constexpr int BT = D * 2 + 16;
  __shared__ __attribute__((aligned(16))) unsigned char lds[D * BT + kRgWaves * kStageBytes + D * 4 + 2 * D * 2];
  unsigned char* const ldsB = lds;
  const int tid = threadIdx.x;
  const int lane = tid & 63;
  const int wave = __builtin_amdgcn_readfirstlane(tid >> 6);
  const int i31 = lane & 31;
  const int hi = lane >> 5;
  unsigned char* const stg = lds + D * BT + wave * kStageBytes;
  float* const cvec = reinterpret_cast<float*>(lds + D * BT + kRgWaves * kStageBytes);
  uint16_t* const wdot = reinterpret_cast<uint16_t*>(lds + D * BT + kRgWaves * kStageBytes + D * 4);

  if (p.trans_b) {
    for (int c = tid; c < D * (D / 8); c += kRgThreads) {
      const int j = c / (D / 8), q = c % (D / 8);
      const float4 f0 = *reinterpret_cast<const float4*>(p.bmat + j * D + 8 * q);
      const float4 f1 = *reinterpret_cast<const float4*>(p.bmat + j * D + 8 * q + 4);
      uint4 v;
      v.x = cvt_pk_bf16(f0.x, f0.y); v.y = cvt_pk_bf16(f0.z, f0.w);
      v.z = cvt_pk_bf16(f1.x, f1.y); v.w = cvt_pk_bf16(f1.z, f1.w);
      *reinterpret_cast<uint4*>(ldsB + j * BT + 16 * q) = v;
    }
  } else {
    for (int c = tid; c < D * (D / 4); c += kRgThreads) {
      const int k = c / (D / 4), q = c % (D / 4);
      const float4 f = *reinterpret_cast<const float4*>(p.bmat + k * D + 4 * q);
      const uint32_t lo = cvt_pk_bf16(f.x, f.y), hi2 = cvt_pk_bf16(f.z, f.w);
      *reinterpret_cast<uint16_t*>(ldsB + (4 * q + 0) * BT + 2 * k) = static_cast<uint16_t>(lo & 0xffffu);
      *reinterpret_cast<uint16_t*>(ldsB + (4 * q + 1) * BT + 2 * k) = static_cast<uint16_t>(lo >> 16);
      *reinterpret_cast<uint16_t*>(ldsB + (4 * q + 2) * BT + 2 * k) = static_cast<uint16_t>(hi2 & 0xffffu);
      *reinterpret_cast<uint16_t*>(ldsB + (4 * q + 3) * BT + 2 * k) = static_cast<uint16_t>(hi2 >> 16);
    }
  }
  for (int c = tid; c < D; c += kRgThreads) {
    cvec[c] = p.cvec[c];
    if (MODE == kHF) {
      const float wv = p.dvec[c];
      const uint32_t whi = cvt_pk_bf16(wv, 0.f) & 0xffffu;
      wdot[c] = static_cast<uint16_t>(whi);
      wdot[D + c] = static_cast<uint16_t>(cvt_pk_bf16(wv - __uint_as_float(whi << 16), 0.f) & 0xffffu);
    }
  }
  __syncthreads();
  const float beta = MODE == kHF ? p.beta[0] : 0.f;

  const int64_t ntiles = (p.n + 31) / 32;
  const int64_t nwaves = static_cast<int64_t>(gridDim.x) * kRgWaves;
  auto load_tile = [&](int64_t t, bf16x8 (&dst)[KS]) {
    int64_t row = t * 32 + i31;
    if (row >= p.n) row = p.n - 1;
    const uint16_t* src = p.a + row * p.lda + 8 * hi;
#pragma unroll
    for (int s = 0; s < KS; ++s) dst[s] = *reinterpret_cast<const bf16x8*>(src + 16 * s);
  };
  const unsigned char* const bfrag0 = ldsB + i31 * BT + 16 * hi;
  unsigned char* const st_w = stg + 4 * hi * kStageStride + 2 * i31;
  const unsigned char* const st_r = stg + (lane >> 3) * kStageStride + 16 * (lane & 7);

  bf16x8 cur[KS], nxt[KS];
  int64_t t = static_cast<int64_t>(blockIdx.x) * kRgWaves + wave;
  if (t < ntiles) load_tile(t, cur);
  for (; t < ntiles; t += nwaves) {
    const int64_t tn = t + nwaves;
    if (tn < ntiles) load_tile(tn, nxt);
    const int64_t row0 = t * 32;
    const bool tail = row0 + 32 > p.n;
    uint16_t* const yrow = p.out + (row0 + (lane >> 3)) * p.ldo + 8 * (lane & 7);
    uint4* const ptile = MODE != kHF ? p.part + t * (NS * 2 * 64) + lane : nullptr;

    float rs[16], rc[16];
    if (MODE == kHF) {
      f32x16 dacc;
#pragma unroll
      for (int r = 0; r < 16; ++r) dacc[r] = 0.f;
#pragma unroll
      for (int s = 0; s < KS; ++s) {
        const unsigned char* wb = reinterpret_cast<const unsigned char*>(wdot) + 32 * s + 16 * hi;
        const bf16x8 b = *reinterpret_cast<const bf16x8*>(wb);
        const bf16x8 bl = *reinterpret_cast<const bf16x8*>(wb + 2 * D);
        dacc = __builtin_amdgcn_mfma_f32_32x32x16_bf16(cur[s], b, dacc, 0, 0, 0);
        dacc = __builtin_amdgcn_mfma_f32_32x32x16_bf16(cur[s], bl, dacc, 0, 0, 0);
      }
#pragma unroll
      for (int r = 0; r < 16; ++r) {
        const float den = dacc[r] + beta;
        rs[r] = 1.0f / den;
        rc[r] = rs[r];
        dacc[r] = den;
      }
      if (i31 == 0) {
#pragma unroll
        for (int q = 0; q < 4; ++q) {
          const int64_t r0 = row0 + 8 * q + 4 * hi;
          if (!tail) {
            *reinterpret_cast<float4*>(p.den + r0) = make_float4(dacc[4 * q], dacc[4 * q + 1], dacc[4 * q + 2], dacc[4 * q + 3]);
          } else {
#pragma unroll
            for (int j = 0; j < 4; ++j)
              if (r0 + j < p.n) p.den[r0 + j] = dacc[4 * q + j];
          }
        }
      }
    } else if (MODE == kHB1) {
      int64_t row = row0 + i31;
      if (row >= p.n) row = p.n - 1;
      const uint16_t* po = p.a2 + row * p.lda2 + 8 * hi;
      float dot = 0.f;
#pragma unroll
      for (int s = 0; s < KS; ++s) {
        const uint4 o = *reinterpret_cast<const uint4*>(po + 16 * s);
        const uint4 g = *reinterpret_cast<const uint4*>(&cur[s]);
        const uint32_t ov[4] = {o.x, o.y, o.z, o.w}, gv[4] = {g.x, g.y, g.z, g.w};
#pragma unroll
        for (int e = 0; e < 4; ++e) {
          dot = fmaf(__uint_as_float(gv[e] << 16), __uint_as_float(ov[e] << 16), dot);
          dot = fmaf(__uint_as_float(gv[e] & 0xffff0000u), __uint_as_float(ov[e] & 0xffff0000u), dot);
        }
      }
      dot += __shfl_xor(dot, 32, 64);
      const float inv_row = 1.0f / p.den[row];
      const float coef_row = -dot * inv_row;
      if (p.rowscal && hi == 0 && row0 + i31 < p.n) p.rowscal[row0 + i31] = make_float2(inv_row, coef_row);
#pragma unroll
      for (int r = 0; r < 16; ++r) {
        const int src = (r & 3) + 8 * (r >> 2) + 4 * hi;
        rs[r] = __shfl(inv_row, src, 64);
        rc[r] = __shfl(coef_row, src, 64);
      }
    } else {
#pragma unroll
      for (int r = 0; r < 16; ++r) {
        rs[r] = 1.f;
        rc[r] = 1.f;
      }
    }

#pragma unroll
    for (int u = 0; u < NS / 2; ++u) {
      f32x16 acc[2];
#pragma unroll
      for (int r = 0; r < 16; ++r) {
        acc[0][r] = 0.f;
        acc[1][r] = 0.f;
      }
      const unsigned char* const bu = bfrag0 + 64 * u * BT;
      uint4 addend[2][2];
      if (MODE == kHB2) {
#pragma unroll
        for (int c = 0; c < 2; ++c)
#pragma unroll
          for (int q = 0; q < 2; ++q) addend[c][q] = ptile[((2 * u + c) * 2 + q) * 64];
      }
#pragma unroll
      for (int s = 0; s < KS; ++s) {
        const bf16x8 b0 = *reinterpret_cast<const bf16x8*>(bu + 32 * s);
        const bf16x8 b1 = *reinterpret_cast<const bf16x8*>(bu + 32 * BT + 32 * s);
        acc[0] = __builtin_amdgcn_mfma_f32_32x32x16_bf16(cur[s], b0, acc[0], 0, 0, 0);
        acc[1] = __builtin_amdgcn_mfma_f32_32x32x16_bf16(cur[s], b1, acc[1], 0, 0, 0);
      }
      float vc[2];
#pragma unroll
      for (int c = 0; c < 2; ++c) vc[c] = cvec[32 * (2 * u + c) + i31];
#pragma unroll
      for (int c = 0; c < 2; ++c)
#pragma unroll
        for (int r = 0; r < 16; ++r) {
          if (MODE == kHB2) acc[c][r] += vc[c];
          else acc[c][r] = fmaf(rs[r], acc[c][r], rc[r] * vc[c]);
        }
      if (MODE == kHB2) {
#pragma unroll
        for (int c = 0; c < 2; ++c)
#pragma unroll
          for (int q = 0; q < 2; ++q) {
            const uint4 v = addend[c][q];
            const uint32_t d4[4] = {v.x, v.y, v.z, v.w};
#pragma unroll
            for (int e = 0; e < 4; ++e) {
              acc[c][8 * q + 2 * e] += __uint_as_float(d4[e] << 16);
              acc[c][8 * q + 2 * e + 1] += __uint_as_float(d4[e] & 0xffff0000u);
            }
          }
      }
      if (MODE == kHB1) {
#pragma unroll
        for (int c = 0; c < 2; ++c)
#pragma unroll
          for (int q = 0; q < 2; ++q) {
            uint4 v;
            v.x = cvt_pk_bf16(acc[c][8 * q + 0], acc[c][8 * q + 1]);
            v.y = cvt_pk_bf16(acc[c][8 * q + 2], acc[c][8 * q + 3]);
            v.z = cvt_pk_bf16(acc[c][8 * q + 4], acc[c][8 * q + 5]);
            v.w = cvt_pk_bf16(acc[c][8 * q + 6], acc[c][8 * q + 7]);
            ptile[((2 * u + c) * 2 + q) * 64] = v;
          }
        __builtin_amdgcn_sched_barrier(0);
        continue;
      }
#pragma unroll
      for (int hh = 0; hh < 2; ++hh) {
#pragma unroll
        for (int c = 0; c < 2; ++c) {
#pragma unroll
          for (int r = 8 * hh; r < 8 * hh + 8; r += 2) {
            const uint32_t v = cvt_pk_bf16(acc[c][r], acc[c][r + 1]);
            const int rl = (r & 3) + 8 * ((r >> 2) & 1);
            *reinterpret_cast<uint16_t*>(st_w + rl * kStageStride + 64 * c) = static_cast<uint16_t>(v & 0xffffu);
            *reinterpret_cast<uint16_t*>(st_w + (rl + 1) * kStageStride + 64 * c) = static_cast<uint16_t>(v >> 16);
          }
        }
        wave_lds_sync();
#pragma unroll
        for (int q = 0; q < 2; ++q) {
          uint4 v = *reinterpret_cast<const uint4*>(st_r + 8 * q * kStageStride);
          if (!tail || row0 + 16 * hh + 8 * q + (lane >> 3) < p.n) {
            if (MODE == kHB2 && p.addend) {
              const uint4 ad = *reinterpret_cast<const uint4*>(p.addend + (row0 + 16 * hh + 8 * q + (lane >> 3)) * p.ldadd +
                                                               64 * u + 8 * (lane & 7));
              const uint32_t a4[4] = {ad.x, ad.y, ad.z, ad.w};
              uint32_t v4[4] = {v.x, v.y, v.z, v.w};
#pragma unroll
              for (int e = 0; e < 4; ++e)
                v4[e] = cvt_pk_bf16(__uint_as_float(v4[e] << 16) + __uint_as_float(a4[e] << 16),
                                    __uint_as_float(v4[e] & 0xffff0000u) + __uint_as_float(a4[e] & 0xffff0000u));
              v = make_uint4(v4[0], v4[1], v4[2], v4[3]);
            }
            *reinterpret_cast<uint4*>(yrow + (16 * hh + 8 * q) * p.ldo + 64 * u) = v;
          }
        }
        wave_lds_sync();
      }
    }
#pragma unroll
    for (int s = 0; s < KS; ++s) cur[s] = nxt[s];
  }
}

constexpr int kStemMaxK = 128;
constexpr int kStemKS = kStemMaxK / 16;

struct StemArgs {
  const uint16_t* x; int64_t ldx; int d_in;
  const uint16_t* w0; int64_t ldw0; const float* b0;
  const uint16_t* w1; int64_t ldw1; const float* b1;
  const float* shift;
  float* spart;
  uint16_t* y0; int64_t ldy0;
  uint16_t* y1; int64_t ldy1;
  int64_t n;
};

template <int D, bool STATS>
__global__ __launch_bounds__(kRgThreads, 2) void k_stem_bf16(StemArgs p) {
  constexpr int NS1 = D / 32;
  constexpr int BT = kStemMaxK * 2 + 16;
  __shared__ __attribute__((aligned(16))) unsigned char lds[2 * D * BT + kRgWaves * kStageBytes + 3 * D * 4];
  const int tid = threadIdx.x;
  const int lane = tid & 63;
  const int wave = __builtin_amdgcn_readfirstlane(tid >> 6);
  const int i31 = lane & 31;
  const int hi = lane >> 5;
  unsigned char* const ldsB = lds;
  unsigned char* const stg = lds + 2 * D * BT + wave * kStageBytes;
  float* const cvec = reinterpret_cast<float*>(lds + 2 * D * BT + kRgWaves * kStageBytes);
  const int nout = p.w1 ? 2 : 1;
  const int ks = (p.d_in + 15) / 16;

  for (int c = tid; c < nout * D * (kStemMaxK / 4); c += kRgThreads) {
    const int j = c / (kStemMaxK / 4), q = c % (kStemMaxK / 4);
    const uint16_t* wsrc = j < D ? p.w0 + static_cast<int64_t>(j) * p.ldw0 : p.w1 + static_cast<int64_t>(j - D) * p.ldw1;
    uint2 v = make_uint2(0u, 0u);
    if (4 * q < p.d_in) v = *reinterpret_cast<const uint2*>(wsrc + 4 * q);
    *reinterpret_cast<uint2*>(ldsB + j * BT + 8 * q) = v;
  }
  for (int c = tid; c < D; c += kRgThreads) {
    cvec[c] = p.b0 ? p.b0[c] : 0.f;
    cvec[D + c] = (p.w1 && p.b1) ? p.b1[c] : 0.f;
    cvec[2 * D + c] = (STATS && p.shift) ? p.shift[c] : 0.f;
  }
  __syncthreads();

  float s1[NS1], s2[NS1];
#pragma unroll
  for (int w = 0; w < NS1; ++w) {
    s1[w] = 0.f;
    s2[w] = 0.f;
  }

  const int64_t ntiles = (p.n + 31) / 32;
  const int64_t nwaves = static_cast<int64_t>(gridDim.x) * kRgWaves;
  auto load_tile = [&](int64_t t, bf16x8 (&dst)[kStemKS]) {
    int64_t row = t * 32 + i31;
    if (row >= p.n) row = p.n - 1;
    const uint16_t* src = p.x + row * p.ldx + 8 * hi;
#pragma unroll
    for (int s = 0; s < kStemKS; ++s) {
      const int k0 = 16 * s + 8 * hi;
      uint2 lo = make_uint2(0u, 0u), hi2 = make_uint2(0u, 0u);
      if (k0 < p.d_in) lo = *reinterpret_cast<const uint2*>(src + 16 * s);
      if (k0 + 4 < p.d_in) hi2 = *reinterpret_cast<const uint2*>(src + 16 * s + 4);
      const uint4 v = make_uint4(lo.x, lo.y, hi2.x, hi2.y);
      dst[s] = *reinterpret_cast<const bf16x8*>(&v);
    }
  };
  const unsigned char* const bfrag0 = ldsB + i31 * BT + 16 * hi;
  unsigned char* const st_w = stg + 4 * hi * kStageStride + 2 * i31;
  const unsigned char* const st_r = stg + (lane >> 3) * kStageStride + 16 * (lane & 7);

  bf16x8 cur[kStemKS], nxt[kStemKS];
  int64_t t = static_cast<int64_t>(blockIdx.x) * kRgWaves + wave;
  if (t < ntiles) load_tile(t, cur);
  for (; t < ntiles; t += nwaves) {
    const int64_t tn = t + nwaves;
    if (tn < ntiles) load_tile(tn, nxt);
    const int64_t row0 = t * 32;
    const bool tail = row0 + 32 > p.n;
    for (int o = 0; o < nout; ++o) {
      uint16_t* const yrow = (o == 0 ? p.y0 + (row0 + (lane >> 3)) * p.ldy0 : p.y1 + (row0 + (lane >> 3)) * p.ldy1) +
                             8 * (lane & 7);
      const int64_t ldy = o == 0 ? p.ldy0 : p.ldy1;
#pragma unroll
      for (int u = 0; u < NS1 / 2; ++u) {
        f32x16 acc[2];
#pragma unroll
        for (int r = 0; r < 16; ++r) {
          acc[0][r] = 0.f;
          acc[1][r] = 0.f;
        }
        const unsigned char* const bu = bfrag0 + (o * D + 64 * u) * BT;
#pragma unroll
        for (int s = 0; s < kStemKS; ++s) {
          if (s < ks) {
            const bf16x8 b0 = *reinterpret_cast<const bf16x8*>(bu + 32 * s);
            const bf16x8 b1 = *reinterpret_cast<const bf16x8*>(bu + 32 * BT + 32 * s);
            acc[0] = __builtin_amdgcn_mfma_f32_32x32x16_bf16(cur[s], b0, acc[0], 0, 0, 0);
            acc[1] = __builtin_amdgcn_mfma_f32_32x32x16_bf16(cur[s], b1, acc[1], 0, 0, 0);
          }
        }
        float bias_c[2], shift_c[2];
#pragma unroll
        for (int c = 0; c < 2; ++c) {
          bias_c[c] = cvec[o * D + 32 * (2 * u + c) + i31];
          shift_c[c] = STATS ? cvec[2 * D + 32 * (2 * u + c) + i31] : 0.f;
        }
#pragma unroll
        for (int hh = 0; hh < 2; ++hh) {
          uint32_t pk[2][4];
#pragma unroll
          for (int c = 0; c < 2; ++c) {
#pragma unroll
            for (int r = 8 * hh; r < 8 * hh + 8; r += 2) {
              const uint32_t v = cvt_pk_bf16(acc[c][r] + bias_c[c], acc[c][r + 1] + bias_c[c]);
              const int rl = (r & 3) + 8 * ((r >> 2) & 1);
              *reinterpret_cast<uint16_t*>(st_w + rl * kStageStride + 64 * c) = static_cast<uint16_t>(v & 0xffffu);
              *reinterpret_cast<uint16_t*>(st_w + (rl + 1) * kStageStride + 64 * c) = static_cast<uint16_t>(v >> 16);
              pk[c][(r >> 1) & 3] = v;
            }
          }
          if (STATS && o == 0) {
#pragma unroll
            for (int c = 0; c < 2; ++c)
#pragma unroll
              for (int q = 0; q < 4; ++q) {
                const int64_t ra = row0 + 16 * hh + ((2 * q) & 3) + 8 * (q >> 1) + 4 * hi;
                const float v0 = (!tail || ra < p.n) ? __uint_as_float(pk[c][q] << 16) - shift_c[c] : 0.f;
                const float v1 = (!tail || ra + 1 < p.n) ? __uint_as_float(pk[c][q] & 0xffff0000u) - shift_c[c] : 0.f;
                s1[2 * u + c] += v0 + v1;
                s2[2 * u + c] = fmaf(v0, v0, fmaf(v1, v1, s2[2 * u + c]));
              }
          }
          wave_lds_sync();
#pragma unroll
          for (int q = 0; q < 2; ++q) {
            const uint4 v = *reinterpret_cast<const uint4*>(st_r + 8 * q * kStageStride);
            if (!tail || row0 + 16 * hh + 8 * q + (lane >> 3) < p.n)
              *reinterpret_cast<uint4*>(yrow + (16 * hh + 8 * q) * ldy + 64 * u) = v;
          }
          wave_lds_sync();
        }
      }
    }
#pragma unroll
    for (int s = 0; s < kStemKS; ++s) cur[s] = nxt[s];
  }

  if (STATS) {
    __syncthreads();
    static_assert(kRgWaves * 2 * D * 4 <= kRgWaves * kStageBytes, "reduction scratch must fit the staging patches");
    float* const redb = reinterpret_cast<float*>(lds + 2 * D * BT);
#pragma unroll
    for (int w = 0; w < NS1; ++w) {
      const float a1s = s1[w] + __shfl_xor(s1[w], 32, 64);
      const float a2s = s2[w] + __shfl_xor(s2[w], 32, 64);
      if (hi == 0) {
        redb[(wave * 2 + 0) * D + 32 * w + i31] = a1s;
        redb[(wave * 2 + 1) * D + 32 * w + i31] = a2s;
      }
    }
    __syncthreads();
    for (int c = tid; c < 2 * D; c += kRgThreads) {
      float s = 0.f;
#pragma unroll
      for (int v = 0; v < kRgWaves; ++v) s += redb[v * 2 * D + c];
      p.spart[static_cast<int64_t>(blockIdx.x) * 2 * D + c] = s;
    }
  }
}

__global__ __launch_bounds__(256) void k_rowgemm_stats(const float* __restrict__ part, int nblk, int len,
                                                       float* __restrict__ stats) {
  __shared__ float red[256];
  const int c = blockIdx.x * 64 + (threadIdx.x & 63);
  const int g = threadIdx.x >> 6;
  float s = 0.f;
  if (c < len)
    for (int b = g; b < nblk; b += 4) s += part[static_cast<int64_t>(b) * len + c];
  red[threadIdx.x] = s;
  __syncthreads();
  if (g == 0 && c < len) stats[c] = (red[threadIdx.x] + red[64 + threadIdx.x]) + (red[128 + threadIdx.x] + red[192 + threadIdx.x]);
}

int grid_blocks(int64_t n) {
  const int64_t tiles = (n + 31) / 32;
  int64_t b = (tiles + kRgWaves - 1) / kRgWaves;
  if (b > kNumCU) b = kNumCU;
  if (b < 1) b = 1;
  return static_cast<int>(b);
}

int dx2_pair_vblocks(int64_t n) { return grid_blocks(n) / 16 * 8; }
int dx2_acc_vblocks(int64_t n, int d) {
  if (d != 256) return grid_blocks(n);
  const int pairs = dx2_pair_vblocks(n);
  return pairs < 8 ? 8 : pairs;
}
int bn_bwd_dx_vblocks(int64_t n, int d) {
  const int roles = d / 64;
  int vblocks = (grid_blocks(n) + roles - 1) / roles;
  if (roles > 1) {
    vblocks = (vblocks + 7) / 8 * 8;
    if (vblocks > kNumCU / roles) vblocks = kNumCU / roles;
  }
  return vblocks;
}
int cat_vblocks(int64_t n, int d) {
  int vblocks = grid_blocks(n);
  if (d == 256) {
    vblocks = (vblocks + 1) / 2;
    vblocks = (vblocks + 7) / 8 * 8;
    if (vblocks > kNumCU / 2) vblocks = kNumCU / 2;
  }
  return vblocks;
}

inline const uint16_t* bf(const void* p) { return static_cast<const uint16_t*>(p); }
inline uint16_t* bf(void* p) { return static_cast<uint16_t*>(p); }
inline const float* fl(const void* p) { return static_cast<const float*>(p); }
inline float* fl(void* p) { return static_cast<float*>(p); }

inline bool bf16_rows(int d, int dtype) { return dtype == SGF_BF16 && (d == 64 || d == 128 || d == 256); }
template <typename F>
int by_width(const char* fn, int d, F&& f) {
// ... 26 lines not shown
        case 6: return launch(k_rowgemm_bf16<256, false, 0, 6>, blocks, a, st);
      }
    }
#endif
    return launch(k_rowgemm_bf16<D, STATS, IO>, blocks, a, st);
  });
}

bool supported(int32_t d_in, int32_t d_out, int32_t dtype) {
  if (f32_storage(dtype)) return linear_f32_supported(d_in, d_out);
  return d_in == d_out && bf16_rows(d_in, dtype);
}

struct RowOp {
  const void* p;
  int64_t ld;
  int width;
  bool optional = false;
};
bool rows16(const void* p, int64_t ld) { return reinterpret_cast<uintptr_t>(p) % 16 == 0 && ld % 8 == 0; }
template <size_t K>
bool rows_given(const RowOp (&ops)[K]) {
  for (const RowOp& o : ops)
    if (!o.p && !o.optional) return false;
  return true;
}
template <size_t K>
int rows_fit(const char* fn, const RowOp (&ops)[K]) {
  for (const RowOp& o : ops)
    SGF_REQUIRE(!o.p || o.ld >= o.width, SGF_E_INVALID, "%s: leading dimension smaller than the width", fn);
  for (const RowOp& o : ops)
    SGF_REQUIRE(!o.p || rows16(o.p, o.ld), SGF_E_INVALID,
                "%s: rows must be 16-byte aligned (pointers %% 16, leading dims %% 8 elements)", fn);
  return SGF_OK;
}
inline bool fits_u32_bytes(int64_t n, int64_t ld) {
  return static_cast<uint64_t>(n) * static_cast<uint64_t>(ld) * 2 < 0xffffff00ull;
}
inline size_t tile_bytes(int64_t n, int d) { return static_cast<size_t>((n + 31) / 32) * 32 * static_cast<size_t>(d) * 2; }

int check_common(const char* who, const void* a, int64_t lda, const void* w, int64_t ldw, int64_t n, int32_t d_in,
                 int32_t d_out, int32_t dtype, const void* y, int64_t ldy) {
  SGF_REQUIRE(n >= 0, SGF_E_INVALID, "%s: negative n", who);
  SGF_REQUIRE(supported(d_in, d_out, dtype), SGF_E_UNSUPPORTED,
              "%s: bf16 storage with d_in == d_out in {64, 128, 256}, or fp32 storage with widths %% 4 == 0 up to 256 "
              "(got %d -> %d, dtype %d)", who, d_in, d_out, dtype);
  if (n == 0) return SGF_OK;
  SGF_REQUIRE(a && w && y, SGF_E_INVALID, "%s: null pointer", who);
  if (f32_storage(dtype)) {
    SGF_REQUIRE(lda >= d_in && ldy >= d_out && lda % 4 == 0 && ldy % 4 == 0 && ldw % 4 == 0 &&
                    reinterpret_cast<uintptr_t>(a) % 16 == 0 && reinterpret_cast<uintptr_t>(y) % 16 == 0,
                SGF_E_INVALID, "%s: rows must be 16-byte aligned (pointers %% 16, leading dims %% 4 elements)", who);
    return SGF_OK;
  }
  const RowOp rows[] = {{a, lda, d_in}, {y, ldy, d_out}, {w, ldw, d_in > d_out ? d_in : d_out}};
  return rows_fit(who, rows);
}

int check_bf16_rows(const char* fn, int64_t n, int d, int dtype) {
  SGF_REQUIRE(n >= 0, SGF_E_INVALID, "%s: negative n", fn);
  SGF_REQUIRE(bf16_rows(d, dtype), SGF_E_UNSUPPORTED, "%s: bf16 storage, d in {64, 128, 256} (got d = %d, dtype %d)", fn, d,
              dtype);
  return SGF_OK;
}

template <int MODE>
int launch_hrow(const char* fn, const HRowArgs& a, int d, hipStream_t st) {
  return by_width(fn, d, [&](auto w) { return launch(k_hrow_bf16<decltype(w)::value, MODE>, grid_blocks(a.n), a, st); });
}

}

bool hrow_supported(int d, int dtype, const void* a, int64_t lda, const void* b, int64_t ldb, const void* c, int64_t ldc,
                    const void* o, int64_t ldo) {
  return bf16_rows(d, dtype) && rows16(a, lda) && (!b || rows16(b, ldb)) && (!c || rows16(c, ldc)) && rows16(o, ldo);
}

size_t hrow_partial_bytes(int64_t n, int d) { return tile_bytes(n, d); }

int hrow_fwd(const void* h, int64_t ldh, int64_t n, int d, const float* M, const float* m, const float* w,
             const float* beta, void* out, int64_t ldo, float* den, hipStream_t st) {
  HRowArgs a{bf(h), ldh, nullptr, 0, M, 0, m, w, beta, den, bf(out), ldo, nullptr, n, nullptr, nullptr, 0};
  return launch_hrow<kHF>("hrow_fwd", a, d, st);
}

int hrow_bwd_pre(const void* g, int64_t ldg, const void* o, int64_t ldo, const float* den, int64_t n, int d,
                 const float* M, const float* w, void* partial, float* rowscal, hipStream_t st) {
  HRowArgs a{bf(g), ldg, bf(o), ldo, M, 1, w, nullptr, nullptr, const_cast<float*>(den), nullptr, 0,
             static_cast<uint4*>(partial), n, reinterpret_cast<float2*>(rowscal), nullptr, 0};
  return launch_hrow<kHB1>("hrow_bwd_pre", a, d, st);
}

int hrow_bwd_post(const void* h, int64_t ldh, int64_t n, int d, const float* Dm, const float* ds, const void* partial,
                  const void* addend, int64_t ldadd, void* dh, int64_t lddh, hipStream_t st) {
  HRowArgs b{bf(h), ldh, nullptr, 0, Dm, 0, ds, nullptr, nullptr, nullptr, bf(dh), lddh,
             const_cast<uint4*>(static_cast<const uint4*>(partial)), n, nullptr, bf(addend), ldadd};
  return launch_hrow<kHB2>("hrow_bwd_post", b, d, st);
}

int hrow_bwd(const void* h, int64_t ldh, const void* g, int64_t ldg, const void* o, int64_t ldo, const float* den,
             int64_t n, int d, const float* M, const float* w, const float* Dm, const float* ds, void* dh, int64_t lddh,
             void* partial, hipStream_t st) {
  int rc = hrow_bwd_pre(g, ldg, o, ldo, den, n, d, M, w, partial, nullptr, st);
  if (rc != SGF_OK) return rc;
  return hrow_bwd_post(h, ldh, n, d, Dm, ds, partial, nullptr, 0, dh, lddh, st);
}

}

using namespace sgf;

extern "C" int32_t sgf_row_lap_rows(int32_t kind, int32_t d, int32_t dtype) {
  if (dtype != SGF_BF16) return -1;
  const int64_t cap_n = static_cast<int64_t>(1) << 40;
  if (kind == 6 || kind == 7) {
    if (d <= 0 || d % 32 != 0 || d > 256) return -1;
    return static_cast<int32_t>(head_lap_rows(kind == 7, cap_n));
  }
  if (!bf16_rows(d, dtype)) return -1;
  int vblocks;
  switch (kind) {
    case 0: case 5: vblocks = grid_blocks(cap_n); break;
    case 1: vblocks = dx2_pair_vblocks(cap_n); break;
    case 2: vblocks = dx2_acc_vblocks(cap_n, d); break;
    case 3: vblocks = bn_bwd_dx_vblocks(cap_n, d); break;
    case 4: vblocks = cat_vblocks(cap_n, d); break;
    default: return -1;
  }
  return vblocks * kRgWaves * 32;
}

extern "C" int32_t sgf_gcn_epilogue_supported(int32_t d_in, int32_t d_out, int32_t dtype) {
  return supported(d_in, d_out, dtype) ? 1 : 0;
}

extern "C" size_t sgf_gcn_epilogue_workspace_bytes(int64_t n, int32_t d_out) {
  if (n < 0 || d_out <= 0) return 0;
  int b = grid_blocks(n) > linear_f32_blocks(n) ? grid_blocks(n) : linear_f32_blocks(n);
  if (b < 8) b = 8;
  return static_cast<size_t>(b) * 2 * static_cast<size_t>(d_out) * sizeof(float);
}

namespace {

int zero_stats(float* stats, int d_out, hipStream_t st) {
  return stats ? zero_floats(stats, 2 * d_out, st) : SGF_OK;
}

int stats_partials(const char* fn, const float* stats, void* workspace, size_t bytes, int64_t n, int d_out, float** spart) {
  *spart = nullptr;
  if (!stats) return SGF_OK;
  const size_t need = sgf_gcn_epilogue_workspace_bytes(n, d_out);
  SGF_REQUIRE(workspace && bytes >= need, SGF_E_WORKSPACE, "%s: workspace %zu < %zu", fn, bytes, need);
  *spart = static_cast<float*>(workspace);
  return SGF_OK;
}

int finalize_stats(int rc, const float* spart, int nblk, int d_out, float* stats, hipStream_t st) {
  if (rc != SGF_OK || !stats) return rc;
  hipLaunchKernelGGL(k_rowgemm_stats, dim3((2 * d_out + 63) / 64), dim3(256), 0, st, spart, nblk, 2 * d_out, stats);
  SGF_LAUNCH_CHECK();
  return SGF_OK;
}

int linear_f32_stats(const void* a, int64_t lda, int64_t n, int d_in, int d_out, const void* w, int64_t ldw, const float* bias,
                     const void* addend, const float* shift, void* y, int64_t ldy, float* spart, float* stats, int dtype,
// ... 168 lines not shown
extern "C" size_t sgf_gcn_epilogue_partial_bytes(int64_t n, int32_t d_out) {
  return n < 0 || d_out <= 0 ? 0 : tile_bytes(n, d_out);
}

extern "C" size_t sgf_gcn_epilogue_dtype_partial_bytes(int64_t n, int32_t d_out, int32_t dtype) {
  if (f32_storage(dtype)) return n < 0 || d_out <= 0 ? 0 : static_cast<size_t>(n) * static_cast<size_t>(d_out) * 4;
  return sgf_gcn_epilogue_partial_bytes(n, d_out);
}

extern "C" int sgf_gcn_epilogue_partial(const void* a, int64_t lda, const void* w, int64_t ldw, const float* bias,
                                        int64_t n, int32_t d_in, int32_t d_out, int32_t dtype, void* partial,
                                        size_t partial_bytes, void* stream) {
  const char* fn = "sgf_gcn_epilogue_partial";
  int rc = check_common(fn, a, lda, w, ldw, n, d_in, d_out, dtype, partial, d_out);
  if (rc != SGF_OK || n == 0) return rc;
  const size_t need = sgf_gcn_epilogue_dtype_partial_bytes(n, d_out, dtype);
  SGF_REQUIRE(partial_bytes >= need, SGF_E_WORKSPACE, "%s: partial buffer %zu < %zu", fn, partial_bytes, need);
  hipStream_t st = static_cast<hipStream_t>(stream);
  if (f32_storage(dtype))
    return linear_f32(fl(a), lda, n, d_in, d_out, fl(w), ldw, 1, bias, nullptr, 0, nullptr, fl(partial), d_out, nullptr, st,
                      dtype == SGF_F32_BF16X3);
  RowGemmArgs args{bf(a), lda, bf(w), ldw, 0, bias, nullptr, nullptr, nullptr, 0, n, static_cast<uint4*>(partial)};
  return launch_rowgemm<false, 1>(fn, args, d_out, grid_blocks(n), st);
}

extern "C" int sgf_gcn_epilogue_stats_add(const void* a, int64_t lda, const void* w, int64_t ldw, const void* partial,
                                          size_t partial_bytes, int64_t n, int32_t d_in, int32_t d_out, int32_t dtype,
                                          void* y, int64_t ldy, const float* shift, float* stats, void* workspace,
                                          size_t workspace_bytes, void* stream) {
  const char* fn = "sgf_gcn_epilogue_stats_add";
  int rc = check_common(fn, a, lda, w, ldw, n, d_in, d_out, dtype, y, ldy);
  if (rc != SGF_OK) return rc;
  hipStream_t st = static_cast<hipStream_t>(stream);
  if (n == 0) return zero_stats(stats, d_out, st);
  SGF_REQUIRE(partial && reinterpret_cast<uintptr_t>(partial) % 16 == 0 &&
                  partial_bytes >= sgf_gcn_epilogue_dtype_partial_bytes(n, d_out, dtype),
              SGF_E_INVALID, "%s: partial buffer missing, misaligned or too small", fn);
  float* spart;
  rc = stats_partials(fn, stats, workspace, workspace_bytes, n, d_out, &spart);
  if (rc != SGF_OK) return rc;
  if (f32_storage(dtype))
    return linear_f32_stats(a, lda, n, d_in, d_out, w, ldw, nullptr, partial, shift, y, ldy, spart, stats, dtype, st);
  const int blocks = grid_blocks(n);
  RowGemmArgs args{bf(a), lda, bf(w), ldw, 0, nullptr, shift, spart, bf(y), ldy, n,
                   const_cast<uint4*>(static_cast<const uint4*>(partial))};
  rc = !stats ? launch_rowgemm<false, 2>(fn, args, d_out, blocks, st) : launch_rowgemm<true, 2>(fn, args, d_out, blocks, st);
  return finalize_stats(rc, spart, blocks, d_out, stats, st);
}

extern "C" int sgf_gcn_epilogue_apply(const void* y, int64_t ldy, const float* mean, const float* rstd,
                                      const float* gamma, const float* beta, const void* res, int64_t ldr,
                                      int32_t relu, int64_t n, int32_t d, int32_t dtype, void* out, int64_t ldo,
                                      void* stream) {
  SGF_REQUIRE(n <= 0 || (y && mean && rstd && out), SGF_E_INVALID, "sgf_gcn_epilogue_apply: null pointer");
  return sgf_bn_apply(y, ldy, mean, rstd, gamma, beta, res, ldr, relu, n, d, dtype, out, ldo, stream);
}

extern "C" int32_t sgf_stem_pair_supported(int32_t d_in, int32_t d_out, int32_t dtype) {
  return d_in > 0 && d_in % 4 == 0 && d_in <= kStemMaxK && bf16_rows(d_out, dtype) ? 1 : 0;
}

extern "C" int sgf_stem_pair(const void* x, int64_t ldx, int64_t n, int32_t d_in, const void* w0, int64_t ldw0,
                             const float* bias0, const void* w1, int64_t ldw1, const float* bias1, int32_t d_out,
                             int32_t dtype, void* y0, int64_t ldy0, void* y1, int64_t ldy1, const float* shift0,
                             float* stats0, void* workspace, size_t workspace_bytes, void* stream) {
  const char* fn = "sgf_stem_pair";
  SGF_REQUIRE(n >= 0, SGF_E_INVALID, "%s: negative n", fn);
  SGF_REQUIRE(sgf_stem_pair_supported(d_in, d_out, dtype), SGF_E_UNSUPPORTED,
              "%s: bf16 storage, d_in %% 4 == 0, d_in <= %d, d_out in {64, 128, 256} (got %d -> %d, dtype %d)", fn,
              kStemMaxK, d_in, d_out, dtype);
  hipStream_t st = static_cast<hipStream_t>(stream);
  if (n == 0) return zero_stats(stats0, d_out, st);
  SGF_REQUIRE(x && w0 && y0 && (!w1 || y1), SGF_E_INVALID, "%s: null pointer", fn);
  SGF_REQUIRE(ldx >= d_in && ldx % 4 == 0 && reinterpret_cast<uintptr_t>(x) % 8 == 0 && ldw0 >= d_in && ldw0 % 4 == 0 &&
                  reinterpret_cast<uintptr_t>(w0) % 8 == 0 &&
                  (!w1 || (ldw1 >= d_in && ldw1 % 4 == 0 && reinterpret_cast<uintptr_t>(w1) % 8 == 0)),
              SGF_E_INVALID, "%s: rows of x / W must be 8-byte aligned (pointers %% 8, leading dims %% 4 elements)", fn);
  SGF_REQUIRE(ldy0 >= d_out && rows16(y0, ldy0) && (!w1 || (ldy1 >= d_out && rows16(y1, ldy1))), SGF_E_INVALID,
              "%s: rows of y must be 16-byte aligned", fn);
  float* spart;
  int rc = stats_partials(fn, stats0, workspace, workspace_bytes, n, d_out, &spart);
  if (rc != SGF_OK) return rc;
  const int blocks = grid_blocks(n);
  StemArgs a{bf(x), ldx, d_in, bf(w0), ldw0, bias0, bf(w1), ldw1, bias1, shift0, spart, bf(y0), ldy0, bf(y1), ldy1, n};
  rc = by_width(fn, d_out, [&](auto w_) {
    return by_flag(stats0, [&](auto s) { return launch(k_stem_bf16<decltype(w_)::value, decltype(s)::value>, blocks, a, st); });
  });
  return finalize_stats(rc, spart, blocks, d_out, stats0, st);
}
```

### sgformer_amd/linear.py

```python
from __future__ import annotations

import os
from functools import partial
from typing import NamedTuple, Optional

import torch
import torch.nn.functional as F

from .kernels import _pair_gram, _rows, _rows16

_F32 = torch.float32
_BF16 = torch.bfloat16

from .graph import K, _has


def _f32c(t):
    return None if t is None else t.detach().float().contiguous()


def _switch(name: str, default: bool) -> bool:
    v = os.environ.get(name)
    return default if v is None else (v != "0" if default else v == "1")


_BN_SAMPLE_ROWS = 1024


class BNSums(NamedTuple):
    sums: torch.Tensor
    shift: Optional[torch.Tensor]
    count: float

    def moments(self):
        d = self.sums.numel() // 2
        m1 = self.sums[:d] / max(self.count, 1.0)
        mean = m1 if self.shift is None else self.shift + m1
        return mean, (self.sums[d:] / max(self.count, 1.0) - m1 * m1).clamp_min_(0.0), self.count


def _shifted_sums(launch, d: int, n: int, device, shard):
    ns = min(n, _BN_SAMPLE_ROWS)
    _, st_s = launch(ns, None, True)
    count = float(n)
    if shard is None:
        shift = st_s[:d] * (1.0 / float(max(ns, 1)))
    else:
        samp = torch.cat([st_s[:d], torch.full((1,), float(ns), dtype=_F32, device=device)])
        shard.all_reduce(samp)
        count = float(shard.n_global)
        shift = (samp[:d] / samp[d].clamp_min(1.0)).contiguous()
    out, st = launch(None, shift, True)
    if shard is not None:
        shard.all_reduce(st)
    return out, BNSums(st, shift, count)


def _column_sums(x: torch.Tensor, shard=None) -> BNSums:
    x = _rows(x.detach())
    return _shifted_sums(lambda rows, shift, _: (None, K.colstats(x if rows is None else x[:rows], shift)),
                         x.shape[1], x.shape[0], x.device, shard)[1]


def batch_stats(x: torch.Tensor, shard=None):
    K.check(x)
    return _column_sums(x, shard).moments()


def _bn_param_grads(stats, d: int, g32, be32, dtype, shard):
    dgamma = stats[d:].to(dtype) if g32 is not None else None
    dbeta = stats[:d].to(dtype) if be32 is not None else None
    if shard is not None and g32 is not None:
        dgamma, dbeta = shard.unsum(dgamma), shard.unsum(dbeta)
    return dgamma, dbeta


class _Linear(torch.autograd.Function):

    @staticmethod
    def forward(ctx, w, b, want_stats: bool, shard, *xs):
        K.check(*xs)
        dt = xs[0].dtype
        wc = w if w.dtype == dt else w.to(dt)
        widths = [x.shape[1] for x in xs]
        if sum(widths) != w.shape[1]:
            raise RuntimeError(f"linear: input widths {widths} do not add up to {w.shape[1]}")
        offs = [sum(widths[:i]) for i in range(len(widths))]
        fused = (len(xs) <= 2 and all(_streaming_linear_ok(x, wc[:, o:o + k]) for x, o, k in zip(xs, offs, widths)))
        if fused:
            xr = [_rows16(x) for x in xs]
            y, stats = _linear_with_stats(xr, wc, _f32c(b), shard) if want_stats else _streaming_linear(xr, wc, _f32c(b))
        else:
            y = K.gemm(xs[0], wc[:, :widths[0]].t(), bias=_f32c(b))
            off = widths[0]
            for x, k in zip(xs[1:], widths[1:]):
                K.gemm(x, wc[:, off:off + k].t(), out=y, beta=1.0, addend=y)
                off += k
            stats = _column_sums(y, shard) if want_stats else None
        ctx.save_for_backward(wc, *xs)
        ctx.meta = (w.dtype, None if b is None else b.dtype, widths)
        return y, stats

    @staticmethod
    def backward(ctx, g, _):
        wc, *xs = ctx.saved_tensors
        wdtype, bdtype, widths = ctx.meta
        g = g.contiguous()
        need_w, need_b = ctx.needs_input_grad[0], ctx.needs_input_grad[1] and bdtype is not None
        dxs, off = [], 0
        for i, k in enumerate(widths):
            if not ctx.needs_input_grad[4 + i]:
                dxs.append(None)
            elif _streaming_linear_ok(g, wc[:, off:off + k], dx=True):
                dxs.append(K.gcn_epilogue_dx(_rows16(g), wc[:, off:off + k]))
            else:
                dxs.append(K.gemm(g, wc[:, off:off + k]))
            off += k
        dw, db = _linear_param_grads(g, xs, widths, need_w, need_b, wdtype, bdtype)
        return (dw, db, None, None, *dxs)


def _linear_param_grads(g, xs, widths, need_w, need_b, wdtype, bdtype):
    dw = db = None
    if need_w or need_b:
        m = g.shape[1]
        gp = _rows(g if m % 4 == 0 else F.pad(g, (0, 4 - m % 4)))
        dw = torch.empty((gp.shape[1], sum(widths)), dtype=_F32, device=g.device)
        off = 0
        if (len(xs) == 2 and widths[0] == widths[1] and widths[0] % 4 == 0 and _has(K, "gram2") and gp.dtype == _BF16
                and xs[0].dtype == _BF16 and xs[1].dtype == _BF16 and _pair_gram()):
            k = widths[0]
            db = K.gram2(gp, _rows(xs[0]), _rows(xs[1]), dw[:, :k], dw[:, k:], want_colsum=need_b)
            xs, widths = [], []
        for i, (x, k) in enumerate(zip(xs, widths)):
            if k % 4 == 0 and off % 4 == 0:
                _, cs = K.gram(gp, _rows(x), out=dw[:, off:off + k], want_colsum=(i == 0 and need_b))
            elif k % 4 == 0:
                blk, cs = K.gram(gp, _rows(x), want_colsum=(i == 0 and need_b))
                dw[:, off:off + k] = blk
            else:
                xp = _rows(F.pad(x, (0, 4 - k % 4)))
                blk, cs = K.gram(gp, xp, want_colsum=(i == 0 and need_b))
                dw[:, off:off + k] = blk[:, :k]
            if i == 0:
                db = cs
            off += k
        dw = dw[:m].to(wdtype) if need_w else None
        db = db[:m].to(bdtype) if need_b else None
    return dw, db


def _batchnorm_of(book, launch, d: int, n: int, device, shard):
    if book.use_batch():
        out, stats = _shifted_sums(launch, d, n, device, shard)
        mean, rstd, count, used = book.from_sums(stats)
    else:
        out = launch(None, None, False)[0]
        mean, rstd, count, used = book.running()
    return out, _f32c(mean), _f32c(rstd), count, used


def _stem_launch(x, w0c, w1c, b32):
    def launch(rows, shift, want_stats):
        if rows is not None:
            return None, K.stem_pair(x[:rows], w0c, b32[0], None, None, None, want_stats0=True)[2]
        y0, y1, st = K.stem_pair(x, w0c, b32[0], w1c, b32[1], shift, want_stats0=want_stats)
        return (y0, y1), st
    return launch


class _StemPair(torch.autograd.Function):

    @staticmethod
    def forward(ctx, x, w0, b0, w1, b1, want_stats: bool, shard):
        K.check(x)
        dt = x.dtype
        w0c, w1c = w0.to(dt), w1.to(dt)
        launch = _stem_launch(x, w0c, w1c, [_f32c(b0), _f32c(b1)])
        if want_stats:
            (y0, y1), stats = _shifted_sums(launch, w0.shape[0], x.shape[0], x.device, shard)
        else:
            (y0, y1), stats = launch(None, None, False)[0], None
        ctx.save_for_backward(x, w0c, w1c)
        ctx.meta = (w0.dtype, None if b0 is None else b0.dtype, w1.dtype, None if b1 is None else b1.dtype)
        return y0, y1, stats

    @staticmethod
    def backward(ctx, g0, g1, _):
        x, w0c, w1c = ctx.saved_tensors
        wd0, bd0, wd1, bd1 = ctx.meta
        k = [x.shape[1]]
        dw0, db0 = _linear_param_grads(g0.contiguous(), [x], k, ctx.needs_input_grad[1],
                                       ctx.needs_input_grad[2] and bd0 is not None, wd0, bd0)
        dw1, db1 = _linear_param_grads(g1.contiguous(), [x], k, ctx.needs_input_grad[3],
                                       ctx.needs_input_grad[4] and bd1 is not None, wd1, bd1)
        dx = None
        if ctx.needs_input_grad[0]:
            dx = K.gemm(g0.contiguous(), w0c)
            K.gemm(g1.contiguous(), w1c, out=dx, beta=1.0, addend=dx)
        return dx, dw0, db0, dw1, db1, None, None


class _StemPairBN(torch.autograd.Function):

    @staticmethod
    def forward(ctx, x, w0, b0, w1, b1, gamma, beta, book, shard, ln_gamma=None, ln_beta=None, ln_cfg=None, pack=None):
        K.check(x)
        dt = x.dtype
        w0c, w1c = w0.to(dt), w1.to(dt)
        (y0, y1), mean, rstd, n_tot, training = _batchnorm_of(book, _stem_launch(x, w0c, w1c, [_f32c(b0), _f32c(b1)]),
                                                              w0.shape[0], x.shape[0], x.device, shard)
        g32, be32 = _f32c(gamma), _f32c(beta)
        if pack is not None:
            x0, pack["out"] = K.bn_apply_packed(y0, mean, rstd, g32, be32, None, True, pack["slot_bytes"])
        else:
            x0 = K.bn_apply(y0, mean, rstd, g32, be32, None, True)
        out1, ln_saved = y1, (None, None, None, None, None)
        if ln_cfg is not None:
            eps, ln_relu, affine = ln_cfg
            lg32, lb32 = (_f32c(ln_gamma), _f32c(ln_beta)) if affine else (None, None)
            out1, lmean, lrstd = K.ln_fwd(_rows(y1), None, 1.0, 0.0, lg32, lb32, bool(ln_relu), float(eps))
            ln_saved = (y1, lmean, lrstd, lg32, lb32)
        ctx.save_for_backward(x, w0c, w1c, y0, g32, be32, mean, rstd, *ln_saved)
        ctx.meta = (w0.dtype, None if b0 is None else b0.dtype, w1.dtype, None if b1 is None else b1.dtype,
                    None if gamma is None else gamma.dtype, bool(training), float(n_tot), shard,
                    None if ln_cfg is None else (bool(ln_cfg[1]), None if ln_gamma is None else ln_gamma.dtype))
        return x0, x0.view_as(x0), out1

    @staticmethod
    def backward(ctx, ga, gb, g1):
        x, w0c, w1c, y0, g32, be32, mean, rstd, y1, lmean, lrstd, lg32, lb32 = ctx.saved_tensors
        wd0, bd0, wd1, bd1, gdt, training, n_tot, shard, ln_meta = ctx.meta
        d = y0.shape[1]
        if ga is None:
            ga, gb = gb, None
        if ga is None:
            ga = torch.zeros_like(y0)
        ga = _rows(ga.contiguous())
        gb = None if gb is None else _rows(gb.contiguous())
        stats = K.bn_bwd_stats2(ga, gb, y0, mean, rstd, g32, be32, True)
        if shard is not None:
            shard.all_reduce(stats)
        inv_n = 1.0 / max(n_tot, 1.0)
        dw0, db0 = K.gram_bn_bwd(ga, gb, y0, mean, rstd, g32, be32, True, stats, inv_n, training, _rows(x))
        dw0 = dw0.to(wd0) if ctx.needs_input_grad[1] else None
        db0 = db0.to(bd0) if (ctx.needs_input_grad[2] and bd0 is not None) else None
        dlg = dlb = None
        if ln_meta is not None:
            ln_relu, lgdt = ln_meta
            dw1, db1, dlg, dlb = K.gram_ln_bwd(_rows(g1.contiguous()), y1, lmean, lrstd, lg32, lb32, ln_relu, _rows(x))
            dw1 = dw1.to(wd1) if ctx.needs_input_grad[3] else None
            db1 = db1.to(bd1) if (ctx.needs_input_grad[4] and bd1 is not None) else None
            dlg, dlb = (dlg.to(lgdt), dlb.to(lgdt)) if lg32 is not None else (None, None)
        else:
            dw1, db1 = _linear_param_grads(g1.contiguous(), [x], [x.shape[1]], ctx.needs_input_grad[3],
                                           ctx.needs_input_grad[4] and bd1 is not None, wd1, bd1)
        dgamma, dbeta = _bn_param_grads(stats, d, g32, be32, gdt, shard)
        dx = None
        if ctx.needs_input_grad[0]:
            g = ga if gb is None else ga + gb
            dz = K.bn_bwd_apply(g, y0, mean, rstd, g32, be32, True, stats, inv_n, training)
            gl = g1
            if ln_meta is not None:
                gl = K.ln_bwd(_rows(g1.contiguous()), None, y1, None, 1.0, 0.0, lg32, False, lmean, lrstd)[0] \
                    if not ln_meta[0] else None
                if gl is None:
                    raise NotImplementedError("features that require a gradient behind the fused LayerNorm stem: set "
                                              "SGF_STEM_LN_FUSED=0")
            dx = K.gemm(dz, w0c)
            K.gemm(gl.contiguous(), w1c, out=dx, beta=1.0, addend=dx)
        return dx, dw0, db0, dw1, db1, dgamma, dbeta, None, None, dlg, dlb, None, None


def stem_pair_bn_supported(x, w0, w1) -> bool:
    return stem_pair_supported(x, w0, w1) and _has(K, "gram_bn_bwd_supported", w0.shape[0], x.shape[1], x.dtype)


def stem_pair_bn(x, w0, b0, w1, b1, gamma, beta, book, shard=None, ln=None, pack=None):
    if ln is None:
        return _StemPairBN.apply(x, w0, b0, w1, b1, gamma, beta, book, shard, None, None, None, pack)
    lg, lb, eps, relu = ln
    return _StemPairBN.apply(x, w0, b0, w1, b1, gamma, beta, book, shard, lg, lb, (eps, relu, lg is not None), pack)


def stem_ln_supported(x, w1) -> bool:
    return (_has(K, "gram_ln_bwd_supported", w1.shape[0], x.shape[1], x.dtype) and not x.requires_grad
            and _switch("SGF_STEM_LN_FUSED", True))


def stem_pair_supported(x, w0, w1) -> bool:
    return (x.dim() == 2 and x.shape[0] > 0 and w0.shape == w1.shape and x.stride(-1) == 1
            and (x.stride(0) * x.element_size()) % 8 == 0 and x.data_ptr() % 8 == 0
            and K.stem_pair_supported(x.shape[1], w0.shape[0], x.dtype))


def stem_pair(x, w0, b0, w1, b1, want_stats0=False, shard=None):
    y0, y1, stats = _StemPair.apply(x, w0, b0, w1, b1, bool(want_stats0), shard)
    return (y0, y1), (None if stats is None else stats.moments())


def _streaming_linear_ok(x: torch.Tensor, wc: torch.Tensor, dx: bool = False) -> bool:
    return (x.dim() == 2 and x.shape[0] > 0 and wc.stride(-1) == 1 and (wc.stride(0) * wc.element_size()) % 16 == 0
            and wc.data_ptr() % 16 == 0 and x.shape[1] == (wc.shape[0] if dx else wc.shape[1])
            and K.gcn_epilogue_supported(wc.shape[1], wc.shape[0], x.dtype))
# ... 146 lines not shown
```

### sgformer_amd/ops.py

```python
from __future__ import annotations

from typing import Optional

import torch
import torch.nn.functional as F

from . import kernels as _kernels
from .kernels import HipKernels, LONG_ROW, _SEGMENT, _workspace
from .kernels import _rows, _rows16

_F32 = torch.float32
_BF16 = torch.bfloat16


from . import graph as _graph
from .graph import *
from .graph import K, graph_cache, _own_block_spmm, _sharded_spmm, _tile_params, _block_shape, _mode
from .linear import _bn_param_grads, _f32c, _has, _switch


def set_kernels(table):
    global K
    prev, K = K, table
    _graph.K = _linear.K = table
# ... 30 lines not shown
                n_total = float(shard.n_global)
        out, den, o_heads = K.attn_fwd_apply(q, v, stats, n_total, heads, v_heads, d)
        per_head = bool(per_head) and heads > 1
        ctx.save_for_backward(qkv, v_ext, out, den, o_heads, stats)
        ctx.meta = (heads, d, n_total, shard, per_head)
        return o_heads if per_head else out

    @staticmethod
    def backward(ctx, g):
        qkv, v_ext, out, den, o_heads, stats = ctx.saved_tensors
        heads, d, n_total, shard, per_head = ctx.meta
        g = _rows(g.contiguous())
        hd = heads * d
        q, k, v, v_heads = _split(qkv, v_ext, heads, d)
        o = out if heads == 1 else o_heads
        kw = {"per_head": True} if per_head else {}
        bstats = K.attn_bwd_reduce(q, g, o, den, heads, d, **kw)
        if shard is not None:
            shard.all_reduce(bstats)
        dqkv = torch.empty_like(qkv)
        dv_ext = torch.empty_like(v_ext) if v_ext is not None else None
        dv = dqkv[:, 2 * hd:] if v_ext is None else dv_ext
        K.attn_bwd_apply(q, k, v, g, o, den, stats, bstats, n_total, heads, v_heads, d,
                         dqkv[:, :hd], dqkv[:, hd:2 * hd], dv, **kw)
        return dqkv, dv_ext, None, None, None, None, None


def attention(qkv: torch.Tensor, v_ext: Optional[torch.Tensor], heads: int, d: int, shard=None,
              n_total=None, per_head: bool = False):
    return _Attention.apply(qkv, v_ext, heads, d, shard, n_total, per_head)


class _MM(torch.autograd.Function):

    @staticmethod
    def forward(ctx, a, b):
        ctx.save_for_backward(a, b)
        return K.gemm(a, b)

    @staticmethod
    def backward(ctx, g):
        a, b = ctx.saved_tensors
        ga = K.gemm(g, b.t()) if ctx.needs_input_grad[0] else None
        gb = K.gemm(a.t(), g) if ctx.needs_input_grad[1] else None
        return ga, gb


def mm(a: torch.Tensor, b: torch.Tensor) -> torch.Tensor:
    return _MM.apply(a, b)


def _attn_h_small_packed(Gt, Wqk, Wv, n_total: float, sum_v: bool = False):
    d = Wv.shape[0]
    D = Gt.shape[0] - 1
    PG = mm(Wqk, Gt)
    ssq = (PG * Wqk).view(2, -1).sum(1)
    c = torch.rsqrt(ssq[0] * ssq[1])
    PK = PG[d:]
    SZ = torch.cat([mm(PK, Wv.t()), PK[:, D:]], 1)
    U = mm(Wqk[:d].t(), SZ) * c
    if sum_v:
        Mm = torch.cat([U[:D, :d], (U[D, :d] + mm(Wv, Gt[:, D:]).view(-1))[None]], 0)
    else:
        Mm = torch.add(U[:, :d], Wv.t(), alpha=n_total)
    wb = U[:, d].contiguous()
    return Mm[:D], Mm[D], wb[:D], wb[D:] + n_total


def _attn_h_pack(G, s, n_rows: float, wq, bq, wk, bk, wv, bv):
    D = G.shape[0]
    Gt = torch.empty((D + 1, D + 1), dtype=_F32, device=G.device)
    Gt[:D, :D] = G
    Gt[:D, D] = s
    Gt[D, :D] = s
    Gt[D, D].fill_(n_rows)
    Wqk = torch.cat([torch.cat([wq, wk], 0), torch.cat([bq, bk])[:, None]], 1)
    Wv = torch.cat([wv, bv[:, None]], 1)
    return Gt, Wqk, Wv


class _AttentionFromInput(torch.autograd.Function):

    @staticmethod
    def forward(ctx, h, wq, bq, wk, bk, wv, bv, shard, n_override, sum_v=False, tap=None):
        K.check(h)
        h = _rows(h)
        n, d = h.shape
        ctx.tap = tap
        if tap is not None:
            tap["armed"] = tap["sibling"] = True
        f32 = [t.detach().float() for t in (wq, bq, wk, bk)]
        if wv is None:
            f32 += [torch.eye(d, dtype=_F32, device=h.device), torch.zeros(d, dtype=_F32, device=h.device)]
        else:
            f32 += [wv.detach().float(), bv.detach().float()]
        G, s = K.gram(h, h)
        n_rows = float(n)
        if shard is not None:
            gs = torch.cat([G.reshape(-1), s])
            shard.all_reduce(gs)
            G, s = gs[:d * d].reshape(d, d), gs[d * d:]
            n_rows = float(shard.n_global)
        n_total = n_rows if n_override is None else float(n_override)
        di = f32[0].shape[1]
        if sum_v:
            with torch.enable_grad():
                leaves = [t.requires_grad_(True) for t in _attn_h_pack(G, s, n_rows, *f32)]
                small = _attn_h_small_packed(*leaves, n_total, sum_v=True)
            M, m, w, beta = (t.detach().contiguous() for t in small)
            ctx.small = (leaves, small, None)
        else:
            M, m, w, beta, saved = K.attn_h_small_fwd(G, s, n_rows, n_total, f32[0], f32[1], f32[2], f32[3],
                                                      None if wv is None else f32[4], None if wv is None else f32[5])
            ctx.small = (None, None, saved)
        out, den = K.attn_h_fwd(h, M, m, w, beta)
        ctx.save_for_backward(h, out, den, G, s, M, w, *f32)
        ctx.meta = (n_rows, n_total, shard, wv is None,
                    [None if t is None else t.dtype for t in (wq, bq, wk, bk, wv, bv)], bool(sum_v))
        return out

    @staticmethod
    def backward(ctx, g):
        h, out, den, G, s, M, w, *f32 = ctx.saved_tensors
        n_rows, n_total, shard, v_is_h, dtypes, sum_v = ctx.meta
        d = h.shape[1]
        g = _rows(g.contiguous())
        split = K.attn_h_bwd_split_supported(h, g, out)
        if split:
            rowscal = K.attn_h_bwd_pre(g, out, den, M, w)
            hstats = K.attn_h_bwd_reduce_scaled(h, g, rowscal)
        else:
            hstats = K.attn_h_bwd_reduce(h, g, out, den)
        if shard is not None:
            shard.all_reduce(hstats)
        dM, dw_, dm = hstats[:d * d].reshape(d, d), hstats[d * d:d * d + d], hstats[d * d + d:d * d + 2 * d]
        dbeta = hstats[d * d + 2 * d:]
        leaves, small, saved = ctx.small
        do, di = f32[0].shape
        if saved is None:
            gGt, gWqk, gWv = torch.autograd.grad(small, leaves, grad_outputs=(dM, dm, dw_, dbeta), retain_graph=True)
            Dm = gGt[:di, :di]
            D = (Dm + Dm.t()).contiguous()
            ds = gGt[:di, di] + gGt[di, :di]
            grads = (None, None, gWqk[:do, :di].contiguous(), gWqk[:do, di].contiguous(), gWqk[do:, :di].contiguous(),
                     gWqk[do:, di].contiguous(), gWv[:, :di].contiguous(), gWv[:, di].contiguous())
        else:
            D, ds, *pgr = K.attn_h_small_bwd(dM, dw_, dm, dbeta, n_total, saved, di, do, want_v=not v_is_h)
            grads = (None, None, *pgr)
        extra = None
        if ctx.tap is not None:
            extra = ctx.tap.pop("grad", None)
            if extra is None:
                ctx.tap["armed"] = False
        if split:
            fold = extra is not None and extra.dtype == h.dtype and extra.shape == h.shape
            dh = K.attn_h_bwd_post(h, D, ds.contiguous(), _rows16(extra) if fold else None)
            if extra is not None and not fold:
                dh = dh + extra
        else:
            dh = K.attn_h_bwd_apply(h, g, out, den, M, w, D, ds.contiguous())
            if extra is not None:
                dh = dh + extra
        pg = list(grads[2:])
        if shard is not None:
            pg = [None if t is None else shard.unsum(t) for t in pg]
        if v_is_h:
            pg[4] = pg[5] = None
        pg = [None if (t is None or dt is None) else t.to(dt) for t, dt in zip(pg, dtypes)]
        return (dh, *pg, None, None, None, None)


def attention_from_input(h, wq, bq, wk, bk, wv=None, bv=None, shard=None, n_total=None, sum_v=False, tap=None):
    return _AttentionFromInput.apply(h, wq, bq, wk, bk, wv, bv, shard, n_total, sum_v, tap)


class _GradTap(torch.autograd.Function):

    @staticmethod
    def forward(ctx, x, holder):
        ctx.holder = holder
        return x.view_as(x)

    @staticmethod
    def backward(ctx, g):
        holder = ctx.holder
        if holder.get("armed"):
            holder["grad"] = g
            return None, None
        holder["armed"] = bool(holder.get("sibling"))
        return g, None


def grad_tap(x, holder):
    if not (torch.is_grad_enabled() and x.requires_grad):
        return x
    return _GradTap.apply(x, holder)


def attention_stats(q: torch.Tensor, k: torch.Tensor, v: torch.Tensor):
    K.check(q, k, v)
    n, heads, d = q.shape
    q2, k2, v2 = (_rows(t.reshape(n, -1)) for t in (q, k, v))
    return K.attn_fwd_reduce(q2, k2, v2, heads, v.shape[1], d)


class _LNResAct(torch.autograd.Function):
    @staticmethod
    def forward(ctx, x, res, a: float, b: float, gamma, beta, relu: bool, eps: float):
        K.check(x, res, gamma)
        x, res = _rows(x), _rows(res)
        has_ln = gamma is not None
        g32, b32 = (_f32c(gamma), _f32c(beta)) if has_ln else (None, None)
        y, mean, rstd = K.ln_fwd(x, res, a, b, g32, b32, relu, eps)
        ctx.save_for_backward(x, res, y if relu else None, g32, mean, rstd)
        ctx.meta = (float(a), float(b), bool(relu), gamma.dtype if has_ln else None)
        return y

    @staticmethod
    def backward(ctx, gy):
        x, res, y, g32, mean, rstd = ctx.saved_tensors
        a, b, relu, pdtype = ctx.meta
        gy = _rows(gy.contiguous())
        dx, dres, dgamma, dbeta = K.ln_bwd(gy, y, x, res, a, b, g32, relu, mean, rstd)
        if g32 is not None:
            dgamma, dbeta = dgamma.to(pdtype), dbeta.to(pdtype)
        return dx, dres, None, None, dgamma, dbeta, None, None


def ln_res_act(x, res, a, b, gamma, beta, relu, eps=1e-5):
    return _LNResAct.apply(x, res, a, b, gamma, beta, relu, eps)


class _BNActRes(torch.autograd.Function):
    @staticmethod
    def forward(ctx, x, res, gamma, beta, mean, rstd, relu: bool, training: bool, n_tot: float,
                shard):
        K.check(x, res)
        x, res = _rows(x), _rows(res)
        g32, b32, mean, rstd = _f32c(gamma), _f32c(beta), _f32c(mean), _f32c(rstd)
        y = K.bn_apply(x, mean, rstd, g32, b32, res, relu)
        ctx.save_for_backward(x, g32, b32, mean, rstd)
        ctx.meta = (bool(relu), bool(training), float(n_tot), shard, res is not None,
                    gamma.dtype if gamma is not None else None)
        return y

    @staticmethod
    def backward(ctx, gy):
        x, g32, b32, mean, rstd = ctx.saved_tensors
        relu, training, n_tot, shard, has_res, pdtype = ctx.meta
        gy = _rows(gy.contiguous())
        d = x.shape[1]
        stats = K.bn_bwd_stats(gy, x, mean, rstd, g32, b32, relu)
        if shard is not None:
            shard.all_reduce(stats)
        dx = K.bn_bwd_apply(gy, x, mean, rstd, g32, b32, relu, stats, 1.0 / max(n_tot, 1.0), training)
        dgamma, dbeta = _bn_param_grads(stats, d, g32, b32, pdtype, shard)
# ... 150 lines not shown
    def backward(ctx, g):
        (idx_inv,) = ctx.saved_tensors
        return K.gather_rows(g, idx_inv, ctx.in_dtype), None, None, None


def permute_rows(x: torch.Tensor, idx: torch.Tensor, idx_inv: torch.Tensor, out_dtype=None) -> torch.Tensor:
    return _PermuteRows.apply(x, idx, idx_inv, out_dtype)


def gather_rows(x: torch.Tensor, idx: torch.Tensor, out_dtype=None) -> torch.Tensor:
    K.check(x, idx)
    return K.gather_rows(x, idx, out_dtype)


class _FanOut(torch.autograd.Function):
    @staticmethod
    def forward(ctx, x, k: int):
        ctx.k = k
        return tuple(x.view_as(x) for _ in range(k))

    @staticmethod
    def backward(ctx, *grads):
        gs = [g for g in grads if g is not None]
        if not gs:
            return None, None
        if len(gs) == 1:
            return gs[0], None
        if gs[0].shape[1] % 4 != 0 or len(gs) > 8:
            out = gs[0]
            for g in gs[1:]:
                out = out + g
            return out, None
        return K.sum_n(gs), None


def fan_out(x: torch.Tensor, k: int):
    if k <= 1 or not x.requires_grad:
        return tuple(x for _ in range(max(k, 1)))
    return _FanOut.apply(x, k)


class _Axpby(torch.autograd.Function):
    @staticmethod
    def forward(ctx, x1, x2, a: float, b: float):
        K.check(x1, x2)
        ctx.ab = (float(a), float(b))
        return K.axpby(_rows(x1), a, _rows(x2), b)

    @staticmethod
    def backward(ctx, g):
        a, b = ctx.ab
        ga = g * a
        return ga, (ga if a == b else g * b), None, None


def axpby(x1, x2, a, b):
    return _Axpby.apply(x1, x2, a, b)


class _CombineFC(torch.autograd.Function):
    @staticmethod
    def forward(ctx, x1, x2, w, bias, a: float, b: float, row_map=None):
        K.check(x1, x2)
        x1, x2 = _rows16(x1), _rows16(x2)
        ctx.row_map = row_map
        w32, b32 = _f32c(w), _f32c(bias)
        c = w32.shape[0]
        if (x1.dtype == _F32 or c > 64) and c % 4 != 0:
            w32, b32 = F.pad(w32, (0, 0, 0, 4 - c % 4)), F.pad(b32, (0, 4 - c % 4))
        ctx.save_for_backward(x1, x2, w32)
        ctx.meta = (float(a), float(b), w.dtype, bias.dtype, c)
        out = K.combine_fc_fwd(x1, a, x2, b, w32, b32) if row_map is None else K.combine_fc_fwd(x1, a, x2, b, w32, b32, row_map)
        return out if out.shape[1] == c else out[:, :c]

    @staticmethod
    def backward(ctx, g):
        x1, x2, w32 = ctx.saved_tensors
        a, b, wdtype, bdtype, c = ctx.meta
        g = g.float()
        if w32.shape[0] != g.shape[1]:
            g = F.pad(g, (0, w32.shape[0] - g.shape[1]))
        g = g.contiguous()
        row_map = ctx.row_map
        if x1.dtype == _BF16 and _has(K, "combine_fc_bwd_g") and g.shape[1] <= 64:
            dx1, dx2, gp = K.combine_fc_bwd_g(g, w32, a, b, row_map)
        else:
            dx1, dx2 = K.combine_fc_bwd(g, w32, a, b, x1.dtype) if row_map is None else K.combine_fc_bwd(g, w32, a, b, x1.dtype,
                                                                                                           row_map)
            gp = K.gather_rows(g, row_map, x1.dtype) if row_map is not None else g.to(x1.dtype)
            if gp.shape[1] % 4 != 0:
                gp = F.pad(gp, (0, 4 - gp.shape[1] % 4))
            gp = _rows(gp)
        dw1, db = K.gram(gp, x1, want_colsum=True)
        dw2, _ = K.gram(gp, x2, want_colsum=False)
        return dx1, dx2, (a * dw1 + b * dw2)[:c].to(wdtype), db[:c].to(bdtype), None, None, None


def combine_fc(x1, x2, w, bias, a: float, b: float, row_map=None) -> torch.Tensor:
    return _CombineFC.apply(x1, x2, w, bias, a, b, row_map)


def combine_fc_mapped_supported(x: torch.Tensor, classes: int) -> bool:
    return (x.dim() == 2 and _switch("SGF_HEAD_MAPPED", True)
            and _has(K, "combine_fc_mapped_supported", x.shape[1], classes, x.dtype))


def combine_fc_supported(x: torch.Tensor, classes: int) -> bool:
    if x.dim() == 2 and x.dtype == _BF16 and classes > 64 and not _switch("SGF_HEAD_WIDE", False):
        return False
    return x.dim() == 2 and K.combine_fc_supported(x.shape[1], classes, x.dtype)



from . import linear as _linear
from .linear import *
from .linear import (_BN_SAMPLE_ROWS, _Linear, _LinearBNActRes, _StemPair, _StemPairBN, _acc_in_place, _fused_bwd, _linear_param_grads,
                     _linear_with_stats, _streaming_linear, _streaming_linear_ok)
```

### sgformer_amd/ours.py

```python
from __future__ import annotations

from dataclasses import dataclass
from typing import Optional

import torch
import torch.nn as nn
import torch.nn.functional as F

from . import head_rows, ops

__all__ = ["GraphConvLayer", "GraphConv", "TransConvLayer", "TransConv", "SGFormer",
           "full_attention_conv"]

_NO_SHARD = None

DEFAULT_COMPUTE_DTYPE = None

import os as _os
OVERLAP_BRANCHES = _os.environ.get("SGF_OVERLAP", "1") == "1"
OVERLAP_MIN_NODES = 65536

PACKED_SLOT_BYTES = (384, 0, 0)
_side_streams = {}

# ... 222 lines not shown
    def _fused_layers(self, x0):
        return (self.use_bn and not self._drop_on and len(self.convs) > 0 and all(c.use_init for c in self.convs)
                and all(ops.gcn_layer_fused_ok(x0, c.W.weight) for c in self.convs))

    def _stage(self, bn, x, res, relu, stats=None):
        fuse_res = res is not None and not self._drop_on
        if self.use_bn:
            x = self._bn_act_res(bn, x, res if fuse_res else None, relu, stats)
        else:
            if relu:
                x = torch.relu(x)
            if fuse_res:
                x = x + res
        return _drop(x, self.dropout, self.training, res if (res is not None and not fuse_res) else None)

    def forward(self, x, edge_index, stem=None):
        ops._require_cuda(x, None if isinstance(edge_index, ops.CSRGraph) else edge_index)
        x_first = packed = None
        if stem is not None and stem.gcn_first is not None:
            x, x_first = stem.gcn, stem.gcn_first
            packed = stem.pack.pop("out", None) if stem.pack is not None else None
        else:
            if stem is not None:
                x, stats0 = stem.gcn, stem.gcn_stats
            else:
                x, stats0 = _lin(x, self.fcs[0]), None
            x = self._stage(self.bns[0], x, None, True, stats0)
        if self._fused_layers(x):
            x0, chain = x, ops.GradChain()
            if x_first is not None:
                x = x_first
            for i, conv in enumerate(self.convs):
                bn = self.bns[i + 1]
                y = conv.propagate(x, edge_index, packed)
                packed = None
                req = self.pack_request(i + 1, x0.shape[0], x0.dtype, edge_index) if self.use_act else None
                x = ops.linear_bn_act_res(y, x0, conv.W.weight, conv.W.bias, bn.weight, bn.bias, _BNBook(self, bn),
                                          self.use_act, self.use_residual, self._shard, chain, i == 0, req)
                packed = req.pop("out", None) if req is not None else None
            return x
        uses_init = [c.use_init for c in self.convs]
        k = 1 + sum(uses_init) + (len(self.convs) if self.use_residual else 0)
        hub = list(ops.fan_out(x, k)) if k <= 8 else [x] * k
        x = hub.pop()
        for i, conv in enumerate(self.convs):
            want = self.use_bn and _BNBook(self, self.bns[i + 1]).use_batch()
            x0 = hub.pop() if uses_init[i] else None
            if want:
                x, stats = conv(x, edge_index, x0, bn_stats=True)
            else:
                x, stats = conv(x, edge_index, x0), None
            x = self._stage(self.bns[i + 1], x, hub.pop() if self.use_residual else None, self.use_act, stats)
        return x


class TransConvLayer(nn.Module):

    def __init__(self, in_channels, out_channels, num_heads, use_weight=True):
        super().__init__()
        self.Wk = nn.Linear(in_channels, out_channels * num_heads)
        self.Wq = nn.Linear(in_channels, out_channels * num_heads)
        if use_weight:
            self.Wv = nn.Linear(in_channels, out_channels * num_heads)
        self.out_channels = out_channels
        self.num_heads = num_heads
        self.use_weight = use_weight
        self._shard = _NO_SHARD

    def reset_parameters(self):
        self.Wk.reset_parameters()
        self.Wq.reset_parameters()
        if self.use_weight:
            self.Wv.reset_parameters()

    def _project(self, query_input, source_input):
        ws = [self.Wq.weight, self.Wk.weight] + ([self.Wv.weight] if self.use_weight else [])
        bs = [self.Wq.bias, self.Wk.bias] + ([self.Wv.bias] if self.use_weight else [])
        if query_input is source_input:
            return ops.linear(query_input, torch.cat(ws, 0), torch.cat(bs, 0))
        q = ops.linear(query_input, ws[0], bs[0])
        kv = ops.linear(source_input, torch.cat(ws[1:], 0), torch.cat(bs[1:], 0))
        return torch.cat([q, kv], 1)

    def forward(self, query_input, source_input, output_attn=False, grad_tap=None):
        ops._require_cuda(query_input, source_input)
        h, d = self.num_heads, self.out_channels
        if (h == 1 and query_input is source_input and not output_attn and query_input.shape[1] == d
                and d % 4 == 0 and d <= 256):
            wv, bv = (self.Wv.weight, self.Wv.bias) if self.use_weight else (None, None)
            return ops.attention_from_input(query_input, self.Wq.weight, self.Wq.bias, self.Wk.weight,
                                            self.Wk.bias, wv, bv, self._shard, tap=grad_tap)
        qkv = self._project(query_input, source_input)
        v_ext = None
        if not self.use_weight:
            if source_input.shape[1] != d:
                raise RuntimeError(f"use_weight=False needs in_channels == out_channels ({d})")
            v_ext = source_input
        final_output = ops.attention(qkv, v_ext, h, d, self._shard)
        if output_attn:
            n = qkv.shape[0]
            qs = qkv[:, :h * d].reshape(n, h, d)
            ks = qkv[:, h * d:2 * h * d].reshape(n, h, d)
            return final_output, _attention_matrix(qs, ks)
        return final_output


class TransConv(nn.Module):

    def __init__(self, in_channels, hidden_channels, num_layers=2, num_heads=1, dropout=0.5,
                 use_bn=True, use_residual=True, use_weight=True, use_act=True, alpha=None,
                 layer_cls=None):
        super().__init__()
        layer_cls = layer_cls or TransConvLayer
        self.convs = nn.ModuleList()
        self.fcs = nn.ModuleList()
        self.fcs.append(nn.Linear(in_channels, hidden_channels))
        self.bns = nn.ModuleList()
        self.bns.append(nn.LayerNorm(hidden_channels))
        for _ in range(num_layers):
            self.convs.append(layer_cls(hidden_channels, hidden_channels, num_heads=num_heads,
                                        use_weight=use_weight))
            self.bns.append(nn.LayerNorm(hidden_channels))
        self.dropout = dropout
        self.activation = F.relu
        self.use_bn = use_bn
        self.use_residual = use_residual
        self.use_act = use_act
        self.alpha = alpha

    _attn_post_act = True

    def reset_parameters(self):
        for conv in self.convs:
            conv.reset_parameters()
        for bn in self.bns:
            bn.reset_parameters()
        for fc in self.fcs:
            fc.reset_parameters()

    def _mix(self):
        return (0.5, 0.5) if self.alpha is None else (float(self.alpha), 1.0 - float(self.alpha))

    def _ln(self, ln: nn.LayerNorm, x, res, a, b, relu):
        if res is None and not self.use_bn and not relu:
            return x
        gamma, beta = (ln.weight, ln.bias) if self.use_bn else (None, None)
        return ops.ln_res_act(x, res, a, b, gamma, beta, relu, ln.eps)

    def _embed(self, x, training, stem=None):
        if stem is not None and stem.trans_normed:
            return _drop(stem.trans, self.dropout, training)
        x = _lin(x, self.fcs[0]) if stem is None else stem.trans
        x = self._ln(self.bns[0], x, None, 1.0, 0.0, True)
        return _drop(x, self.dropout, training)

    def forward(self, x, stem=None):
        ops._require_cuda(x)
        x = self._embed(x, self.training, stem)
        layer_ = [x]
        a, b = self._mix()
        for i, conv in enumerate(self.convs):
            if self.use_residual and layer_[i] is x:
                holder = {}
                h = conv(x, x, grad_tap=holder)
                x = self._ln(self.bns[i + 1], h, ops.grad_tap(x, holder), a, b, self.use_act)
            elif self.use_residual:
                h = conv(x, x)
                x = self._ln(self.bns[i + 1], h, layer_[i], a, b, self.use_act)
            else:
                h = conv(x, x)
                x = self._ln(self.bns[i + 1], h, None, 1.0, 0.0, self.use_act)
            x = _drop(x, self.dropout, self.training)
            layer_.append(x)
        return x

    def get_attentions(self, x):
        x = self._embed(x, False)
        layer_, attentions = [x], []
        a, b = self._mix()
        for i, conv in enumerate(self.convs):
            h, attn = conv(x, x, output_attn=True)
            attentions.append(attn)
            res = layer_[i] if self.use_residual else None
            x = self._ln(self.bns[i + 1], h, res, a if res is not None else 1.0,
                         b if res is not None else 0.0, self.use_act and self._attn_post_act)
            layer_.append(x)
        return torch.stack(attentions, dim=0)


class SGFormer(nn.Module):

    def __init__(self, in_channels, hidden_channels, out_channels,
                 trans_num_layers=1, trans_num_heads=1, trans_dropout=0.5, trans_use_bn=True,
                 trans_use_residual=True, trans_use_weight=True, trans_use_act=True,
                 gnn_num_layers=1, gnn_dropout=0.5, gnn_use_weight=True, gnn_use_init=False,
                 gnn_use_bn=True, gnn_use_residual=True, gnn_use_act=True,
                 use_graph=True, graph_weight=0.8, aggregate='add', alpha=None, compute_dtype='default',
                 trans_cls=None):
        super().__init__()
        self.compute_dtype = DEFAULT_COMPUTE_DTYPE if isinstance(compute_dtype, str) else compute_dtype
        self.logits_dtype = None
        self.trans_conv = (trans_cls or TransConv)(
            in_channels, hidden_channels, num_layers=trans_num_layers, num_heads=trans_num_heads,
            dropout=trans_dropout, use_bn=trans_use_bn, use_residual=trans_use_residual,
            use_weight=trans_use_weight, use_act=trans_use_act, alpha=alpha)
        self.graph_conv = GraphConv(in_channels, hidden_channels, gnn_num_layers, gnn_dropout,
                                    gnn_use_bn, gnn_use_residual, gnn_use_weight, gnn_use_init,
                                    gnn_use_act)
        self.use_graph = use_graph
        self.graph_weight = graph_weight
        self.aggregate = aggregate
        self.overlap_branches = OVERLAP_BRANCHES
        if aggregate == 'add':
            self.fc = nn.Linear(hidden_channels, out_channels)
        elif aggregate == 'cat':
            self.fc = nn.Linear(2 * hidden_channels, out_channels)
        else:
            raise ValueError(f'Invalid aggregate type:{aggregate}')
        self.params1 = list(self.trans_conv.parameters())
        self.params2 = list(self.graph_conv.parameters()) if self.graph_conv is not None else []
        self.params2.extend(list(self.fc.parameters()))

    def _forward_on_gpu_from_host(self, x, edge_index):
        if not torch.cuda.is_available():
            ops._require_cuda(x)
        if torch.is_grad_enabled():
            raise RuntimeError("sgformer_amd: CPU tensors with autograd enabled — there is no CPU fallback "
                               "and training runs on MI355X only; move the model and inputs to the GPU")
        dev = torch.device("cuda", torch.cuda.current_device())
        state = {k: v.to(dev) for k, v in list(self.named_parameters()) + list(self.named_buffers())}
        out = torch.func.functional_call(self, state, (x.to(dev), edge_index.to(dev)))
        for k, v in self.named_buffers():
            v.copy_(state[k])
        return out.to(x.device)

    def forward(self, x, edge_index):
        return self._forward(x, edge_index)

    def forward_rows(self, x, edge_index, rows):
        if isinstance(rows, bool) or not (isinstance(rows, int) or torch.is_tensor(rows)):
            raise TypeError(f"forward_rows: rows must be an int, an int64 index tensor or a bool mask, got {type(rows).__name__}")
        return self._forward(x, edge_index, rows)

    def _forward(self, x, edge_index, rows=None, ce_labels=None):
        if rows is None and not x.is_cuda and ops.K.name == "hip" and not next(self.parameters()).is_cuda:
# ... 162 lines not shown
```

Measured before the change: 29.79 million.

## Fuse LayerNorm epilogue into attention row kernel and stem; single-output combine bwd

Adds an LN mode to the attention-from-input row kernel, which applies the residual mix, LayerNorm, affine and ReLU in the epilogue while the output tile is still in registers. This removes a separate LN kernel launch and a full read/write of the activations. It also adds a stem-pair variant with fused LN and a single-output combine_fc backward for the a==b case, which writes dx once and aliases it instead of writing two buffers. The LN epilogue adds register and LDS pressure to the row kernel and delays the next-tile prefetch for D=256, which could reduce occupancy or overlap.

```diff
diff --git a/include/sgf.h b/include/sgf.h
--- a/include/sgf.h
+++ b/include/sgf.h
@@ -8,7 +8,7 @@
 extern "C" {
 #endif
 
-#define SGF_VERSION 666
+#define SGF_VERSION 667
 
 #define SGF_F32 0
 #define SGF_BF16 1
@@ -201,6 +201,11 @@
 int sgf_attn_h_fwd(const void* h, int64_t ldh, int64_t n, int32_t d, int32_t dtype, const float* M,
                    const float* m, const float* w, const float* beta, void* out, int64_t ldo,
                    float* den, void* stream);
+int32_t sgf_attn_h_ln_supported(int32_t d, int32_t dtype);
+int sgf_attn_h_ln_fwd(const void* h, int64_t ldh, int64_t n, int32_t d, int32_t dtype, const float* M, const float* m,
+                      const float* w, const float* beta, void* out, int64_t ldo, float* den, float a, float b,
+                      const float* ln_gamma, const float* ln_beta, int32_t relu, float eps, void* y, int64_t ldy,
+                      float* ln_mean, float* ln_rstd, void* stream);
 int sgf_attn_h_bwd_reduce(const void* h, int64_t ldh, const void* g, int64_t ldg, const void* o,
                           int64_t ldo, const float* den, int64_t n, int32_t d, int32_t dtype,
                           float* hstats, void* workspace, size_t workspace_bytes, void* stream);
@@ -308,6 +313,9 @@
 int sgf_combine_fc_bwd_g(const float* dlogits, int64_t lddl, const float* w, int64_t n, int32_t d, int32_t classes, float a,
                          float b, int32_t dtype, void* dx1, int64_t ld1, void* dx2, int64_t ld2, const int32_t* row_map,
                          void* g_out, int64_t ldg, void* stream);
+int sgf_combine_fc_bwd_g_single(const float* dlogits, int64_t lddl, const float* w, int64_t n, int32_t d, int32_t classes,
+                                float a, int32_t dtype, void* dx, int64_t ldx, const int32_t* row_map, void* g_out,
+                                int64_t ldg, void* stream);
 
 int32_t sgf_gcn_epilogue_supported(int32_t d_in, int32_t d_out, int32_t dtype);
 size_t sgf_gcn_epilogue_workspace_bytes(int64_t n, int32_t d_out);
@@ -354,6 +362,11 @@
                   const float* bias0, const void* w1, int64_t ldw1, const float* bias1, int32_t d_out, int32_t dtype,
                   void* y0, int64_t ldy0, void* y1, int64_t ldy1, const float* shift0, float* stats0, void* workspace,
                   size_t workspace_bytes, void* stream);
+int sgf_stem_pair_ln(const void* x, int64_t ldx, int64_t n, int32_t d_in, const void* w0, int64_t ldw0, const float* bias0,
+                     const void* w1, int64_t ldw1, const float* bias1, int32_t d_out, int32_t dtype, void* y0, int64_t ldy0,
+                     void* y1, int64_t ldy1, const float* shift0, float* stats0, const float* ln_gamma, const float* ln_beta,
+                     int32_t relu, float eps, void* yn, int64_t ldyn, float* ln_mean, float* ln_rstd, void* workspace,
+                     size_t workspace_bytes, void* stream);
 
 int sgf_gemm(const void* a, int64_t a_rs, int64_t a_cs, int32_t a_dtype, const void* b, int64_t b_rs, int64_t b_cs,
              int32_t b_dtype, int64_t m, int32_t n, int64_t k, float alpha, const float* alpha_dev, const float* bias,
diff --git a/sgformer_amd/_lib.py b/sgformer_amd/_lib.py
--- a/sgformer_amd/_lib.py
+++ b/sgformer_amd/_lib.py
@@ -112,6 +112,9 @@
                                            _P, c_int64, _P, c_int64, _P, c_int64, _P]),
     "sgf_attn_h_bstats_len": (c_int64, [c_int32]),
     "sgf_attn_h_fwd": (c_int32, [_P, c_int64, c_int64, c_int32, c_int32, _P, _P, _P, _P, _P, c_int64, _P, _P]),
+    "sgf_attn_h_ln_supported": (c_int32, [c_int32, c_int32]),
+    "sgf_attn_h_ln_fwd": (c_int32, [_P, c_int64, c_int64, c_int32, c_int32, _P, _P, _P, _P, _P, c_int64, _P, c_float, c_float,
+                                    _P, _P, c_int32, c_float, _P, c_int64, _P, _P, _P]),
     "sgf_attn_h_bwd_reduce": (c_int32, [_P, c_int64, _P, c_int64, _P, c_int64, _P, c_int64, c_int32, c_int32,
                                         _P, _P, c_size_t, _P]),
     "sgf_attn_h_bwd_apply": (c_int32, [_P, c_int64, _P, c_int64, _P, c_int64, _P, c_int64, c_int32, c_int32,
@@ -212,6 +215,8 @@
                                      c_int32, _P, c_int64, _P, _P]),
     "sgf_combine_fc_bwd_g": (c_int32, [_P, c_int64, _P, c_int64, c_int32, c_int32, c_float, c_float, c_int32, _P, c_int64, _P,
                                        c_int64, _P, _P, c_int64, _P]),
+    "sgf_combine_fc_bwd_g_single": (c_int32, [_P, c_int64, _P, c_int64, c_int32, c_int32, c_float, c_int32, _P, c_int64, _P, _P,
+                                              c_int64, _P]),
     "sgf_combine_fc_bwd_mapped": (c_int32, [_P, c_int64, _P, c_int64, c_int32, c_int32, c_float, c_float, c_int32, _P,
                                      c_int64, _P, c_int64, _P, _P]),
     "sgf_gcn_epilogue_supported": (c_int32, [c_int32, c_int32, c_int32]),
@@ -243,6 +248,9 @@
     "sgf_stem_pair_supported": (c_int32, [c_int32, c_int32, c_int32]),
     "sgf_stem_pair": (c_int32, [_P, c_int64, c_int64, c_int32, _P, c_int64, _P, _P, c_int64, _P, c_int32, c_int32, _P,
                                 c_int64, _P, c_int64, _P, _P, _P, c_size_t, _P]),
+    "sgf_stem_pair_ln": (c_int32, [_P, c_int64, c_int64, c_int32, _P, c_int64, _P, _P, c_int64, _P, c_int32, c_int32, _P,
+                                   c_int64, _P, c_int64, _P, _P, _P, _P, c_int32, c_float, _P, c_int64, _P, _P, _P, c_size_t,
+                                   _P]),
     "sgf_gemm": (c_int32, [_P, c_int64, c_int64, c_int32, _P, c_int64, c_int64, c_int32, c_int64, c_int32, c_int64, c_float,
                            _P, _P, c_float, _P, c_int64, c_int32, _P, c_int64, c_int32, _P]),
     "sgf_comm_available": (c_int32, []),
diff --git a/sgformer_amd/csrc/head.hip b/sgformer_amd/csrc/head.hip
--- a/sgformer_amd/csrc/head.hip
+++ b/sgformer_amd/csrc/head.hip
@@ -207,6 +207,7 @@
       }
 #pragma unroll
       for (int which = 0; which < 2; ++which) {
+        if (which == 1 && dx2 == nullptr) break;
         const float sc = which == 0 ? a : b;
         uint16_t* const dst = which == 0 ? dx1 : dx2;
         const int64_t ld = which == 0 ? ld1 : ld2;
@@ -345,7 +346,8 @@
 
 static int combine_fc_bwd_impl(const char* fn, const float* dlogits, int64_t lddl, const float* w, int64_t n, int32_t d,
                                int32_t classes, float a, float b, int32_t dtype, void* dx1, int64_t ld1, void* dx2,
-                               int64_t ld2, const int32_t* rmap, void* stream, void* gout = nullptr, int64_t ldgo = 0) {
+                               int64_t ld2, const int32_t* rmap, void* stream, void* gout = nullptr, int64_t ldgo = 0,
+                               bool single = false) {
   int rc = check_head(fn, n, d, classes, dtype);
   if (rc != SGF_OK) return rc;
   if (n == 0) return SGF_OK;
@@ -363,7 +365,11 @@
     return linear_f32_dual(dlogits, lddl, nullptr, 0, 1.f, 0.f, n, classes, d, w, d, 0, nullptr, dx1, ld1, dx2, ld2, a, b, 0, 1,
                            static_cast<hipStream_t>(stream));
   }
-  SGF_REQUIRE(dlogits && w && dx1 && dx2 && lddl >= classes && ld1 >= d && ld2 >= d && ld1 % 8 == 0 && ld2 % 8 == 0 &&
+  if (single) {
+    dx2 = nullptr;
+    ld2 = ld1;
+  }
+  SGF_REQUIRE(dlogits && w && dx1 && (dx2 || single) && lddl >= classes && ld1 >= d && ld2 >= d && ld1 % 8 == 0 && ld2 % 8 == 0 &&
                   reinterpret_cast<uintptr_t>(dx1) % 16 == 0 && reinterpret_cast<uintptr_t>(dx2) % 16 == 0,
               SGF_E_INVALID, "%s: bad pointer / ld (dx1 / dx2: 16-byte aligned, ld %% 8 == 0)", fn);
   SGF_REQUIRE(n < (static_cast<int64_t>(1) << 31), SGF_E_UNSUPPORTED, "%s: more than 2^31 - 1 rows", fn);
@@ -399,6 +405,18 @@
   return combine_fc_bwd_impl(fn, dlogits, lddl, w, n, d, classes, a, b, dtype, dx1, ld1, dx2, ld2, row_map, stream, g_out, ldg);
 }
 
+extern "C" int sgf_combine_fc_bwd_g_single(const float* dlogits, int64_t lddl, const float* w, int64_t n, int32_t d,
+                                           int32_t classes, float a, int32_t dtype, void* dx, int64_t ldx,
+                                           const int32_t* row_map, void* g_out, int64_t ldg, void* stream) {
+  const char* fn = "sgf_combine_fc_bwd_g_single";
+  SGF_REQUIRE(dtype == SGF_BF16 && classes >= 1 && classes <= kMaxClasses, SGF_E_UNSUPPORTED,
+              "%s: bf16 storage and at most %d classes", fn, kMaxClasses);
+  SGF_REQUIRE(n == 0 || (g_out && ldg >= (classes + 15) / 16 * 16 && ldg % 8 == 0 && reinterpret_cast<uintptr_t>(g_out) % 16 == 0),
+              SGF_E_INVALID, "%s: g_out must be 16-byte aligned with ldg %% 8 == 0 and ldg >= classes rounded up to 16", fn);
+  return combine_fc_bwd_impl(fn, dlogits, lddl, w, n, d, classes, a, a, dtype, dx, ldx, nullptr, ldx, row_map, stream, g_out, ldg,
+                             true);
+}
+
 extern "C" int sgf_combine_fc_bwd_mapped(const float* dlogits, int64_t lddl, const float* w, int64_t n, int32_t d,
                                          int32_t classes, float a, float b, int32_t dtype, void* dx1, int64_t ld1,
                                          void* dx2, int64_t ld2, const int32_t* row_map, void* stream) {
diff --git a/sgformer_amd/csrc/rowgemm.hip b/sgformer_amd/csrc/rowgemm.hip
--- a/sgformer_amd/csrc/rowgemm.hip
+++ b/sgformer_amd/csrc/rowgemm.hip
@@ -874,7 +874,87 @@
   }
 }
 
-constexpr int kHF = 0, kHB1 = 1, kHB2 = 2;
+template <int NU>
+__device__ __forceinline__ float ln8_row_sum(const float (&part)[NU]) {
+  static_assert(NU == 1 || NU == 2 || NU == 4, "rows of 64 / 128 / 256 columns");
+  float v = NU == 4 ? (part[0] + part[NU == 4 ? 2 : 0]) + (part[NU == 4 ? 1 : 0] + part[NU == 4 ? 3 : 0])
+                    : (NU == 2 ? part[0] + part[NU - 1] : part[0]);
+  v += __shfl_xor(v, 4, 64);
+  v += __shfl_xor(v, 2, 64);
+  v += __shfl_xor(v, 1, 64);
+  return v;
+}
+
+template <int D, bool RES>
+__device__ __forceinline__ void ln8_row_epilogue(const uint4 (&keep)[D / 64], const uint4 (&res)[D / 64], const float* gb,
+                                                 float a, float b, float eps, int relu, int lane, bool ok, uint16_t* yrow,
+                                                 float* mean, float* rstd) {
+  constexpr int NU = D / 64;
+  constexpr float inv_d = 1.0f / static_cast<float>(D);
+  auto unpack = [&](int u, float (&v)[8]) {
+    const uint32_t xu[4] = {keep[u].x, keep[u].y, keep[u].z, keep[u].w};
+#pragma unroll
+    for (int e = 0; e < 4; ++e) {
+      v[2 * e] = a * __uint_as_float(xu[e] << 16);
+      v[2 * e + 1] = a * __uint_as_float(xu[e] & 0xffff0000u);
+    }
+    if (RES) {
+      const uint32_t ru[4] = {res[u].x, res[u].y, res[u].z, res[u].w};
+#pragma unroll
+      for (int e = 0; e < 4; ++e) {
+        v[2 * e] = fmaf(b, __uint_as_float(ru[e] << 16), v[2 * e]);
+        v[2 * e + 1] = fmaf(b, __uint_as_float(ru[e] & 0xffff0000u), v[2 * e + 1]);
+      }
+    }
+  };
+  float ps[NU];
+#pragma unroll
+  for (int u = 0; u < NU; ++u) {
+    float v[8];
+    unpack(u, v);
+    ps[u] = ((v[0] + v[1]) + (v[2] + v[3])) + ((v[4] + v[5]) + (v[6] + v[7]));
+  }
+  const float mu = ln8_row_sum<NU>(ps) * inv_d;
+#pragma unroll
+  for (int u = 0; u < NU; ++u) {
+    float v[8];
+    unpack(u, v);
+    float sq = 0.f;
+#pragma unroll
+    for (int e = 0; e < 8; ++e) sq = fmaf(v[e] - mu, v[e] - mu, sq);
+    ps[u] = sq;
+  }
+  const float rs = 1.0f / sqrtf(ln8_row_sum<NU>(ps) * inv_d + eps);
+  if ((lane & 7) == 0 && ok) {
+    *mean = mu;
+    *rstd = rs;
+  }
+#pragma unroll
+  for (int u = 0; u < NU; ++u) {
+    const float* gp = gb + 64 * u + 8 * (lane & 7);
+    const float4 g0 = *reinterpret_cast<const float4*>(gp), g1 = *reinterpret_cast<const float4*>(gp + 4);
+    const float4 b0 = *reinterpret_cast<const float4*>(gp + D), b1 = *reinterpret_cast<const float4*>(gp + D + 4);
+    const float g[8] = {g0.x, g0.y, g0.z, g0.w, g1.x, g1.y, g1.z, g1.w};
+    const float be[8] = {b0.x, b0.y, b0.z, b0.w, b1.x, b1.y, b1.z, b1.w};
+    float v[8], o[8];
+    unpack(u, v);
+#pragma unroll
+    for (int e = 0; e < 8; ++e) {
+      o[e] = (v[e] - mu) * rs * g[e] + be[e];
+      if (relu) o[e] = fmaxf(o[e], 0.f);
+    }
+    if (ok) {
+      uint4 ov;
+      ov.x = static_cast<uint32_t>(f32_to_bf16(o[0])) | (static_cast<uint32_t>(f32_to_bf16(o[1])) << 16);
+      ov.y = static_cast<uint32_t>(f32_to_bf16(o[2])) | (static_cast<uint32_t>(f32_to_bf16(o[3])) << 16);
+      ov.z = static_cast<uint32_t>(f32_to_bf16(o[4])) | (static_cast<uint32_t>(f32_to_bf16(o[5])) << 16);
+      ov.w = static_cast<uint32_t>(f32_to_bf16(o[6])) | (static_cast<uint32_t>(f32_to_bf16(o[7])) << 16);
+      *reinterpret_cast<uint4*>(yrow + 64 * u) = ov;
+    }
+  }
+}
+
+constexpr int kHF = 0, kHB1 = 1, kHB2 = 2, kHFLN = 3;
 
 struct HRowArgs {
   const uint16_t* a; int64_t lda;
@@ -888,13 +968,19 @@
   int64_t n;
   float2* rowscal;
   const uint16_t* addend; int64_t ldadd;
+  float ln_a, ln_b; const float* ln_g; const float* ln_bt; int ln_relu; float ln_eps;
+  uint16_t* y; int64_t ldy; float* ln_mean; float* ln_rstd;
 };
 
-template <int D, int MODE>
+template <int D, int MODE_>
 __global__ __launch_bounds__(kRgThreads, 2) void k_hrow_bf16(HRowArgs p) {
+  constexpr bool LN = MODE_ == kHFLN;
+  constexpr int MODE = LN ? kHF : MODE_;
+  constexpr bool LATE = LN && D == 256;
   constexpr int KS = D / 16, NS = D / 32;
   constexpr int BT = D * 2 + 16;
-  __shared__ __attribute__((aligned(16))) unsigned char lds[D * BT + kRgWaves * kStageBytes + D * 4 + 2 * D * 2];
+  __shared__ __attribute__((aligned(16))) unsigned char lds[D * BT + kRgWaves * kStageBytes + D * 4 + 2 * D * 2 + (LN ? 2 * D * 4 : 0)];
+  float* const lngb = reinterpret_cast<float*>(lds + D * BT + kRgWaves * kStageBytes + D * 4 + 2 * D * 2);
   unsigned char* const ldsB = lds;
   const int tid = threadIdx.x;
   const int lane = tid & 63;
@@ -934,6 +1020,10 @@
       wdot[c] = static_cast<uint16_t>(whi);
       wdot[D + c] = static_cast<uint16_t>(cvt_pk_bf16(wv - __uint_as_float(whi << 16), 0.f) & 0xffffu);
     }
+    if (LN) {
+      lngb[c] = p.ln_g[c];
+      lngb[D + c] = p.ln_bt[c];
+    }
   }
   __syncthreads();
   const float beta = MODE == kHF ? p.beta[0] : 0.f;
@@ -956,20 +1046,23 @@
   if (t < ntiles) load_tile(t, cur);
   for (; t < ntiles; t += nwaves) {
     const int64_t tn = t + nwaves;
-    if (tn < ntiles) load_tile(tn, nxt);
+    if (!LATE && tn < ntiles) load_tile(tn, nxt);
     const int64_t row0 = t * 32;
     const bool tail = row0 + 32 > p.n;
     uint16_t* const yrow = p.out + (row0 + (lane >> 3)) * p.ldo + 8 * (lane & 7);
     uint4* const ptile = MODE != kHF ? p.part + t * (NS * 2 * 64) + lane : nullptr;
 
     float rs[16], rc[16];
+    uint4 keep[2][2][NS / 2];
     if (MODE == kHF) {
       f32x16 dacc;
 #pragma unroll
       for (int r = 0; r < 16; ++r) dacc[r] = 0.f;
+      int woff = 16 * hi;
+      if (LN) asm volatile("" : "+v"(woff));
 #pragma unroll
       for (int s = 0; s < KS; ++s) {
-        const unsigned char* wb = reinterpret_cast<const unsigned char*>(wdot) + 32 * s + 16 * hi;
+        const unsigned char* wb = reinterpret_cast<const unsigned char*>(wdot) + 32 * s + woff;
         const bf16x8 b = *reinterpret_cast<const bf16x8*>(wb);
         const bf16x8 bl = *reinterpret_cast<const bf16x8*>(wb + 2 * D);
         dacc = __builtin_amdgcn_mfma_f32_32x32x16_bf16(cur[s], b, dacc, 0, 0, 0);
@@ -1121,12 +1214,45 @@
             }
             *reinterpret_cast<uint4*>(yrow + (16 * hh + 8 * q) * p.ldo + 64 * u) = v;
           }
+          if (LN) keep[hh][q][u] = v;
         }
         wave_lds_sync();
       }
     }
-#pragma unroll
-    for (int s = 0; s < KS; ++s) cur[s] = nxt[s];
+    if (LN) {
+      uint4 hrow[2][2][NS / 2];
+#pragma unroll
+      for (int u = 0; u < NS / 2; ++u) {
+#pragma unroll
+        for (int hh = 0; hh < 2; ++hh) {
+          if ((i31 >> 4) == hh) {
+#pragma unroll
+            for (int j = 0; j < 4; ++j)
+              *reinterpret_cast<bf16x8*>(stg + (i31 & 15) * kStageStride + 32 * j + 16 * hi) = cur[4 * u + j];
+          }
+          wave_lds_sync();
+#pragma unroll
+          for (int q = 0; q < 2; ++q) hrow[hh][q][u] = *reinterpret_cast<const uint4*>(st_r + 8 * q * kStageStride);
+          wave_lds_sync();
+        }
+      }
+      if (LATE && tn < ntiles) load_tile(tn, cur);
+#pragma unroll
+      for (int hh = 0; hh < 2; ++hh)
+#pragma unroll
+        for (int q = 0; q < 2; ++q) {
+          const int64_t row = row0 + 16 * hh + 8 * q + (lane >> 3);
+          const bool ok = !tail || row < p.n;
+          const int64_t rr = ok ? row : 0;
+          ln8_row_epilogue<D, true>(keep[hh][q], hrow[hh][q], lngb, p.ln_a, p.ln_b, p.ln_eps, p.ln_relu, lane, ok,
+                                    p.y + rr * p.ldy + 8 * (lane & 7), p.ln_mean + rr, p.ln_rstd + rr);
+          __builtin_amdgcn_sched_barrier(0);
+        }
+    }
+    if (!LATE) {
+#pragma unroll
+      for (int s = 0; s < KS; ++s) cur[s] = nxt[s];
+    }
   }
 }
 
@@ -1142,13 +1268,15 @@
   uint16_t* y0; int64_t ldy0;
   uint16_t* y1; int64_t ldy1;
   int64_t n;
+  const float* ln_g; const float* ln_b; float ln_a; float ln_eps; int ln_relu;
+  uint16_t* yn; int64_t ldyn; float* ln_mean; float* ln_rstd;
 };
 
-template <int D, bool STATS>
+template <int D, bool STATS, bool LN = false>
 __global__ __launch_bounds__(kRgThreads, 2) void k_stem_bf16(StemArgs p) {
   constexpr int NS1 = D / 32;
   constexpr int BT = kStemMaxK * 2 + 16;
-  __shared__ __attribute__((aligned(16))) unsigned char lds[2 * D * BT + kRgWaves * kStageBytes + 3 * D * 4];
+  __shared__ __attribute__((aligned(16))) unsigned char lds[2 * D * BT + kRgWaves * kStageBytes + 3 * D * 4 + (LN ? 2 * D * 4 : 0)];
   const int tid = threadIdx.x;
   const int lane = tid & 63;
   const int wave = __builtin_amdgcn_readfirstlane(tid >> 6);
@@ -1171,6 +1299,10 @@
     cvec[c] = p.b0 ? p.b0[c] : 0.f;
     cvec[D + c] = (p.w1 && p.b1) ? p.b1[c] : 0.f;
     cvec[2 * D + c] = (STATS && p.shift) ? p.shift[c] : 0.f;
+    if (LN) {
+      cvec[3 * D + c] = p.ln_g[c];
+      cvec[4 * D + c] = p.ln_b[c];
+    }
   }
   __syncthreads();
 
@@ -1213,6 +1345,7 @@
       uint16_t* const yrow = (o == 0 ? p.y0 + (row0 + (lane >> 3)) * p.ldy0 : p.y1 + (row0 + (lane >> 3)) * p.ldy1) +
                              8 * (lane & 7);
       const int64_t ldy = o == 0 ? p.ldy0 : p.ldy1;
+      uint4 keep[2][2][NS1 / 2];
 #pragma unroll
       for (int u = 0; u < NS1 / 2; ++u) {
         f32x16 acc[2];
@@ -1269,9 +1402,23 @@
             const uint4 v = *reinterpret_cast<const uint4*>(st_r + 8 * q * kStageStride);
             if (!tail || row0 + 16 * hh + 8 * q + (lane >> 3) < p.n)
               *reinterpret_cast<uint4*>(yrow + (16 * hh + 8 * q) * ldy + 64 * u) = v;
+            if (LN) keep[hh][q][u] = v;
           }
           wave_lds_sync();
         }
+      }
+      if (LN && o == 1) {
+#pragma unroll
+        for (int hh = 0; hh < 2; ++hh)
+#pragma unroll
+          for (int q = 0; q < 2; ++q) {
+            const int64_t row = row0 + 16 * hh + 8 * q + (lane >> 3);
+            const bool ok = !tail || row < p.n;
+            const int64_t rr = ok ? row : 0;
+            ln8_row_epilogue<D, false>(keep[hh][q], keep[hh][q], cvec + 3 * D, p.ln_a, 0.f, p.ln_eps, p.ln_relu, lane, ok,
+                                       p.yn + rr * p.ldyn + 8 * (lane & 7), p.ln_mean + rr, p.ln_rstd + rr);
+            __builtin_amdgcn_sched_barrier(0);
+          }
       }
     }
 #pragma unroll
@@ -1464,6 +1611,14 @@
              const float* beta, void* out, int64_t ldo, float* den, hipStream_t st) {
   HRowArgs a{bf(h), ldh, nullptr, 0, M, 0, m, w, beta, den, bf(out), ldo, nullptr, n, nullptr, nullptr, 0};
   return launch_hrow<kHF>("hrow_fwd", a, d, st);
+}
+
+int hrow_ln_fwd(const void* h, int64_t ldh, int64_t n, int d, const float* M, const float* m, const float* w,
+                const float* beta, void* out, int64_t ldo, float* den, float a, float b, const float* gamma,
+                const float* lbeta, int relu, float eps, void* y, int64_t ldy, float* mean, float* rstd, hipStream_t st) {
+  HRowArgs args{bf(h), ldh, nullptr, 0, M, 0, m, w, beta, den, bf(out), ldo, nullptr, n, nullptr, nullptr, 0,
+                a, b, gamma, lbeta, relu, eps, bf(y), ldy, mean, rstd};
+  return launch_hrow<kHFLN>("hrow_ln_fwd", args, d, st);
 }
 
 int hrow_bwd_pre(const void* g, int64_t ldg, const void* o, int64_t ldo, const float* den, int64_t n, int d,
@@ -1798,9 +1953,64 @@
   int rc = stats_partials(fn, stats0, workspace, workspace_bytes, n, d_out, &spart);
   if (rc != SGF_OK) return rc;
   const int blocks = grid_blocks(n);
-  StemArgs a{bf(x), ldx, d_in, bf(w0), ldw0, bias0, bf(w1), ldw1, bias1, shift0, spart, bf(y0), ldy0, bf(y1), ldy1, n};
+  StemArgs a{bf(x), ldx, d_in, bf(w0), ldw0, bias0, bf(w1), ldw1, bias1, shift0, spart, bf(y0), ldy0, bf(y1), ldy1, n,
+             nullptr, nullptr, 1.f, 0.f, 0, nullptr, 0, nullptr, nullptr};
   rc = by_width(fn, d_out, [&](auto w_) {
     return by_flag(stats0, [&](auto s) { return launch(k_stem_bf16<decltype(w_)::value, decltype(s)::value>, blocks, a, st); });
   });
   return finalize_stats(rc, spart, blocks, d_out, stats0, st);
 }
+
+extern "C" int sgf_stem_pair_ln(const void* x, int64_t ldx, int64_t n, int32_t d_in, const void* w0, int64_t ldw0,
+                                const float* bias0, const void* w1, int64_t ldw1, const float* bias1, int32_t d_out,
+                                int32_t dtype, void* y0, int64_t ldy0, void* y1, int64_t ldy1, const float* shift0,
+                                float* stats0, const float* ln_gamma, const float* ln_beta, int32_t relu, float eps, void* yn,
+                                int64_t ldyn, float* ln_mean, float* ln_rstd, void* workspace, size_t workspace_bytes,
+                                void* stream) {
+  const char* fn = "sgf_stem_pair_ln";
+  SGF_REQUIRE(n >= 0, SGF_E_INVALID, "%s: negative n", fn);
+  SGF_REQUIRE(sgf_stem_pair_supported(d_in, d_out, dtype), SGF_E_UNSUPPORTED,
+              "%s: bf16 storage, d_in %% 4 == 0, d_in <= %d, d_out in {64, 128, 256} (got %d -> %d, dtype %d)", fn,
+              kStemMaxK, d_in, d_out, dtype);
+  hipStream_t st = static_cast<hipStream_t>(stream);
+  if (n == 0) return zero_stats(stats0, d_out, st);
+  SGF_REQUIRE(x && w0 && y0 && w1 && y1 && ln_gamma && ln_beta && yn && ln_mean && ln_rstd, SGF_E_INVALID, "%s: null pointer",
+              fn);
+  SGF_REQUIRE(ldx >= d_in && ldx % 4 == 0 && reinterpret_cast<uintptr_t>(x) % 8 == 0 && ldw0 >= d_in && ldw0 % 4 == 0 &&
+                  reinterpret_cast<uintptr_t>(w0) % 8 == 0 && ldw1 >= d_in && ldw1 % 4 == 0 &&
+                  reinterpret_cast<uintptr_t>(w1) % 8 == 0,
+              SGF_E_INVALID, "%s: rows of x / W must be 8-byte aligned (pointers %% 8, leading dims %% 4 elements)", fn);
+  SGF_REQUIRE(ldy0 >= d_out && rows16(y0, ldy0) && ldy1 >= d_out && rows16(y1, ldy1) && ldyn >= d_out && rows16(yn, ldyn),
+              SGF_E_INVALID, "%s: rows of y must be 16-byte aligned", fn);
+  float* spart;
+  int rc = stats_partials(fn, stats0, workspace, workspace_bytes, n, d_out, &spart);
+  if (rc != SGF_OK) return rc;
+  const int blocks = grid_blocks(n);
+  StemArgs a{bf(x), ldx, d_in, bf(w0), ldw0, bias0, bf(w1), ldw1, bias1, shift0, spart, bf(y0), ldy0, bf(y1), ldy1, n,
+             ln_gamma, ln_beta, 1.f, eps, relu, bf(yn), ldyn, ln_mean, ln_rstd};
+  rc = by_width(fn, d_out, [&](auto w_) {
+    return by_flag(stats0, [&](auto s) {
+      return launch(k_stem_bf16<decltype(w_)::value, decltype(s)::value, true>, blocks, a, st);
+    });
+  });
+  return finalize_stats(rc, spart, blocks, d_out, stats0, st);
+}
+
+extern "C" int32_t sgf_attn_h_ln_supported(int32_t d, int32_t dtype) { return bf16_rows(d, dtype) ? 1 : 0; }
+
+extern "C" int sgf_attn_h_ln_fwd(const void* h, int64_t ldh, int64_t n, int32_t d, int32_t dtype, const float* M, const float* m,
+                                 const float* w, const float* beta, void* out, int64_t ldo, float* den, float a, float b,
+                                 const float* ln_gamma, const float* ln_beta, int32_t relu, float eps, void* y, int64_t ldy,
+                                 float* ln_mean, float* ln_rstd, void* stream) {
+  const char* fn = "sgf_attn_h_ln_fwd";
+  int rc = check_bf16_rows(fn, n, d, dtype);
+  if (rc != SGF_OK) return rc;
+  if (n == 0) return SGF_OK;
+  SGF_REQUIRE(h && M && m && w && beta && out && den && ln_gamma && ln_beta && y && ln_mean && ln_rstd, SGF_E_INVALID,
+              "%s: null pointer", fn);
+  SGF_REQUIRE(ldh >= d && ldo >= d && ldy >= d && rows16(h, ldh) && rows16(out, ldo) && rows16(y, ldy) &&
+                  reinterpret_cast<uintptr_t>(den) % 16 == 0,
+              SGF_E_INVALID, "%s: rows of h / out / y and den must be 16-byte aligned", fn);
+  return hrow_ln_fwd(h, ldh, n, d, M, m, w, beta, out, ldo, den, a, b, ln_gamma, ln_beta, relu, eps, y, ldy, ln_mean, ln_rstd,
+                     static_cast<hipStream_t>(stream));
+}
diff --git a/sgformer_amd/linear.py b/sgformer_amd/linear.py
--- a/sgformer_amd/linear.py
+++ b/sgformer_amd/linear.py
@@ -13,6 +13,7 @@
 _BF16 = torch.bfloat16
 
 from .graph import K, _has
+from . import row_fusions as _rf
 
 
 def _f32c(t):
@@ -160,10 +161,13 @@
     return out, _f32c(mean), _f32c(rstd), count, used
 
 
-def _stem_launch(x, w0c, w1c, b32):
+def _stem_launch(x, w0c, w1c, b32, ln=None):
     def launch(rows, shift, want_stats):
         if rows is not None:
             return None, K.stem_pair(x[:rows], w0c, b32[0], None, None, None, want_stats0=True)[2]
+        if ln is not None:
+            y0, y1, st, *ln["out"] = ln["fn"](x, w0c, b32[0], w1c, b32[1], shift, want_stats, *ln["args"])
+            return (y0, y1), st
         y0, y1, st = K.stem_pair(x, w0c, b32[0], w1c, b32[1], shift, want_stats0=want_stats)
         return (y0, y1), st
     return launch
@@ -208,7 +212,12 @@
         K.check(x)
         dt = x.dtype
         w0c, w1c = w0.to(dt), w1.to(dt)
-        (y0, y1), mean, rstd, n_tot, training = _batchnorm_of(book, _stem_launch(x, w0c, w1c, [_f32c(b0), _f32c(b1)]),
+        lg32, lb32 = (_f32c(ln_gamma), _f32c(ln_beta)) if (ln_cfg is not None and ln_cfg[2]) else (None, None)
+        fused_ln = None
+        stem_ln = _rf.entry("stem_pair_ln") if (lg32 is not None and lb32 is not None) else None
+        if stem_ln is not None:
+            fused_ln = {"fn": stem_ln, "args": (lg32, lb32, bool(ln_cfg[1]), float(ln_cfg[0]))}
+        (y0, y1), mean, rstd, n_tot, training = _batchnorm_of(book, _stem_launch(x, w0c, w1c, [_f32c(b0), _f32c(b1)], fused_ln),
                                                               w0.shape[0], x.shape[0], x.device, shard)
         g32, be32 = _f32c(gamma), _f32c(beta)
         if pack is not None:
@@ -218,8 +227,10 @@
         out1, ln_saved = y1, (None, None, None, None, None)
         if ln_cfg is not None:
             eps, ln_relu, affine = ln_cfg
-            lg32, lb32 = (_f32c(ln_gamma), _f32c(ln_beta)) if affine else (None, None)
-            out1, lmean, lrstd = K.ln_fwd(_rows(y1), None, 1.0, 0.0, lg32, lb32, bool(ln_relu), float(eps))
+            if fused_ln is not None:
+                out1, lmean, lrstd = fused_ln["out"]
+            else:
+                out1, lmean, lrstd = K.ln_fwd(_rows(y1), None, 1.0, 0.0, lg32, lb32, bool(ln_relu), float(eps))
             ln_saved = (y1, lmean, lrstd, lg32, lb32)
         ctx.save_for_backward(x, w0c, w1c, y0, g32, be32, mean, rstd, *ln_saved)
         ctx.meta = (w0.dtype, None if b0 is None else b0.dtype, w1.dtype, None if b1 is None else b1.dtype,
diff --git a/sgformer_amd/ops.py b/sgformer_amd/ops.py
--- a/sgformer_amd/ops.py
+++ b/sgformer_amd/ops.py
@@ -136,7 +136,7 @@
 class _AttentionFromInput(torch.autograd.Function):
 
     @staticmethod
-    def forward(ctx, h, wq, bq, wk, bk, wv, bv, shard, n_override, sum_v=False, tap=None):
+    def forward(ctx, h, wq, bq, wk, bk, wv, bv, shard, n_override, sum_v=False, tap=None, ln=None, ln_gamma=None, ln_beta=None):
         K.check(h)
         h = _rows(h)
         n, d = h.shape
@@ -167,18 +167,33 @@
             M, m, w, beta, saved = K.attn_h_small_fwd(G, s, n_rows, n_total, f32[0], f32[1], f32[2], f32[3],
                                                       None if wv is None else f32[4], None if wv is None else f32[5])
             ctx.small = (None, None, saved)
-        out, den = K.attn_h_fwd(h, M, m, w, beta)
-        ctx.save_for_backward(h, out, den, G, s, M, w, *f32)
+        ctx.ln = None
+        if ln is not None:
+            a, b, relu, eps = ln
+            g32, b32 = _f32c(ln_gamma), _f32c(ln_beta)
+            out, den, y, mean, rstd = _rf.entry("attn_h_ln_fwd")(h, M, m, w, beta, a, b, g32, b32, relu, eps)
+            ctx.ln = (float(a), float(b), bool(relu), ln_gamma.dtype)
+            ln_saved = (y if relu else None, g32, mean, rstd)
+        else:
+            out, den = K.attn_h_fwd(h, M, m, w, beta)
+            ln_saved = (None, None, None, None)
+        ctx.save_for_backward(*ln_saved, h, out, den, G, s, M, w, *f32)
         ctx.meta = (n_rows, n_total, shard, wv is None,
                     [None if t is None else t.dtype for t in (wq, bq, wk, bk, wv, bv)], bool(sum_v))
-        return out
-
-    @staticmethod
-    def backward(ctx, g):
-        h, out, den, G, s, M, w, *f32 = ctx.saved_tensors
+        return out if ln is None else y
+
+    @staticmethod
+    def backward(ctx, g):
+        y, g32, mean, rstd, h, out, den, G, s, M, w, *f32 = ctx.saved_tensors
         n_rows, n_total, shard, v_is_h, dtypes, sum_v = ctx.meta
         d = h.shape[1]
         g = _rows(g.contiguous())
+        ln_extra, ln_dgamma, ln_dbeta = None, None, None
+        if ctx.ln is not None:
+            a, b, relu, pdtype = ctx.ln
+            g, ln_extra, ln_dgamma, ln_dbeta = K.ln_bwd(g, y, out, h, a, b, g32, relu, mean, rstd)
+            ln_dgamma, ln_dbeta = ln_dgamma.to(pdtype), ln_dbeta.to(pdtype)
+            g = _rows(g.contiguous())
         split = K.attn_h_bwd_split_supported(h, g, out)
         if split:
             rowscal = K.attn_h_bwd_pre(g, out, den, M, w)
@@ -201,7 +216,7 @@
         else:
             D, ds, *pgr = K.attn_h_small_bwd(dM, dw_, dm, dbeta, n_total, saved, di, do, want_v=not v_is_h)
             grads = (None, None, *pgr)
-        extra = None
+        extra = ln_extra
         if ctx.tap is not None:
             extra = ctx.tap.pop("grad", None)
             if extra is None:
@@ -221,11 +236,21 @@
         if v_is_h:
             pg[4] = pg[5] = None
         pg = [None if (t is None or dt is None) else t.to(dt) for t, dt in zip(pg, dtypes)]
-        return (dh, *pg, None, None, None, None)
+        return (dh, *pg, None, None, None, None, None, ln_dgamma, ln_dbeta)
+
+
+def attention_ln_supported(h, gamma) -> bool:
+    ok = _rf.entry("attn_h_ln_supported")
+    return gamma is not None and h.dim() == 2 and ok is not None and bool(ok(_rows(h))) and _rf.entry("attn_h_ln_fwd") is not None
+
+
+def attention_ln_from_input(h, wq, bq, wk, bk, wv, bv, shard, a, b, gamma, beta, relu, eps):
+    return _AttentionFromInput.apply(h, wq, bq, wk, bk, wv, bv, shard, None, False, None,
+                                     (float(a), float(b), bool(relu), float(eps)), gamma, beta)
 
 
 def attention_from_input(h, wq, bq, wk, bk, wv=None, bv=None, shard=None, n_total=None, sum_v=False, tap=None):
-    return _AttentionFromInput.apply(h, wq, bq, wk, bk, wv, bv, shard, n_total, sum_v, tap)
+    return _AttentionFromInput.apply(h, wq, bq, wk, bk, wv, bv, shard, n_total, sum_v, tap, None, None, None)
 
 
 class _GradTap(torch.autograd.Function):
@@ -542,7 +567,11 @@
             g = F.pad(g, (0, w32.shape[0] - g.shape[1]))
         g = g.contiguous()
         row_map = ctx.row_map
-        if x1.dtype == _BF16 and _has(K, "combine_fc_bwd_g") and g.shape[1] <= 64:
+        single = _rf.entry("combine_fc_bwd_g_single") if (x1.dtype == _BF16 and a == b and g.shape[1] <= 64) else None
+        if single is not None:
+            dx1, gp = single(g, w32, a, row_map)
+            dx2 = dx1
+        elif x1.dtype == _BF16 and _has(K, "combine_fc_bwd_g") and g.shape[1] <= 64:
             dx1, dx2, gp = K.combine_fc_bwd_g(g, w32, a, b, row_map)
         else:
             dx1, dx2 = K.combine_fc_bwd(g, w32, a, b, x1.dtype) if row_map is None else K.combine_fc_bwd(g, w32, a, b, x1.dtype,
@@ -573,6 +602,7 @@
 
 
 from . import linear as _linear
+from . import row_fusions as _rf
 from .linear import *
 from .linear import (_BN_SAMPLE_ROWS, _Linear, _LinearBNActRes, _StemPair, _StemPairBN, _acc_in_place, _fused_bwd, _linear_param_grads,
                      _linear_with_stats, _streaming_linear, _streaming_linear_ok)
diff --git a/sgformer_amd/ours.py b/sgformer_amd/ours.py
--- a/sgformer_amd/ours.py
+++ b/sgformer_amd/ours.py
@@ -328,6 +328,17 @@
         kv = ops.linear(source_input, torch.cat(ws[1:], 0), torch.cat(bs[1:], 0))
         return torch.cat([q, kv], 1)
 
+    def fused_ln_ok(self, x, ln_weight) -> bool:
+        d = self.out_channels
+        return (self.num_heads == 1 and self._shard is None and x.dim() == 2 and x.shape[1] == d
+                and ops.attention_ln_supported(x, ln_weight))
+
+    def forward_ln(self, x, a, b, ln, relu):
+        ops._require_cuda(x)
+        wv, bv = (self.Wv.weight, self.Wv.bias) if self.use_weight else (None, None)
+        return ops.attention_ln_from_input(x, self.Wq.weight, self.Wq.bias, self.Wk.weight, self.Wk.bias, wv, bv,
+                                           self._shard, a, b, ln.weight, ln.bias, relu, ln.eps)
+
     def forward(self, query_input, source_input, output_attn=False, grad_tap=None):
         ops._require_cuda(query_input, source_input)
         h, d = self.num_heads, self.out_channels
@@ -406,7 +417,10 @@
         layer_ = [x]
         a, b = self._mix()
         for i, conv in enumerate(self.convs):
-            if self.use_residual and layer_[i] is x:
+            if (self.use_residual and layer_[i] is x and self.use_bn and type(conv).forward is TransConvLayer.forward
+                    and conv.fused_ln_ok(x, self.bns[i + 1].weight)):
+                x = conv.forward_ln(x, a, b, self.bns[i + 1], self.use_act)
+            elif self.use_residual and layer_[i] is x:
                 holder = {}
                 h = conv(x, x, grad_tap=holder)
                 x = self._ln(self.bns[i + 1], h, ops.grad_tap(x, holder), a, b, self.use_act)
diff --git a/sgformer_amd/row_fusions.py b/sgformer_amd/row_fusions.py
--- /dev/null
+++ b/sgformer_amd/row_fusions.py
@@ -0,0 +1,72 @@
+from __future__ import annotations
+
+import os
+
+import torch
+
+from . import _lib, graph
+from .kernels import HipKernels, _code, _launch, _ld, _stats_scratch
+
+_F32 = torch.float32
+_BF16 = torch.bfloat16
+
+
+def enabled() -> bool:
+    return os.environ.get("SGF_ROW_FUSE", "1") != "0"
+
+
+class _Hip:
+    @staticmethod
+    def combine_fc_bwd_g_single(g, w, a: float, row_map=None):
+        n, c = g.shape
+        d = w.shape[1]
+        HipKernels._check_row_map(row_map, n, g.device)
+        dx = torch.empty((n, d), dtype=_BF16, device=g.device)
+        gp = torch.empty((n, (c + 15) // 16 * 16), dtype=_BF16, device=g.device)
+        _launch(g.device, "sgf_combine_fc_bwd_g_single", g, g.stride(0), w, n, d, c, float(a), _code(dx), dx, dx.stride(0),
+                row_map, gp, gp.stride(0))
+        return dx, gp
+
+    @staticmethod
+    def stem_pair_ln(x, w0, b0, w1, b1, shift0, want_stats0, ln_gamma, ln_beta, relu: bool, eps: float):
+        n, d_in = x.shape
+        d_out = w0.shape[0]
+        dev = x.device
+        y0 = torch.empty((n, d_out), dtype=x.dtype, device=dev)
+        y1 = torch.empty((n, d_out), dtype=x.dtype, device=dev)
+        yn = torch.empty((n, d_out), dtype=x.dtype, device=dev)
+        mean = torch.empty(n, dtype=_F32, device=dev)
+        rstd = torch.empty(n, dtype=_F32, device=dev)
+        stats = torch.empty(2 * d_out, dtype=_F32, device=dev) if want_stats0 else None
+        _launch(dev, "sgf_stem_pair_ln", x, _ld(x), n, d_in, w0, w0.stride(0), b0, w1, _ld(w1), b1, d_out, _code(x), y0, _ld(y0),
+                y1, _ld(y1), shift0, stats, ln_gamma, ln_beta, int(relu), float(eps), yn, _ld(yn), mean, rstd,
+                *_stats_scratch(dev, n, d_out, want_stats0))
+        return y0, y1, stats, yn, mean, rstd
+
+    @staticmethod
+    def attn_h_ln_supported(h) -> bool:
+        return (h.dtype == _BF16 and h.dim() == 2 and h.stride(1) == 1 and h.stride(0) % 8 == 0 and h.data_ptr() % 16 == 0
+                and bool(_lib.load().sgf_attn_h_ln_supported(h.shape[1], _lib.SGF_BF16)))
+
+    @staticmethod
+    def attn_h_ln_fwd(h, M, m, w, beta, a: float, b: float, gamma, lbeta, relu: bool, eps: float):
+        n, d = h.shape
+        dev = h.device
+        out = torch.empty((n, d), dtype=h.dtype, device=dev)
+        y = torch.empty((n, d), dtype=h.dtype, device=dev)
+        den = torch.empty((n, 1), dtype=_F32, device=dev)
+        mean = torch.empty(n, dtype=_F32, device=dev)
+        rstd = torch.empty(n, dtype=_F32, device=dev)
+        _launch(dev, "sgf_attn_h_ln_fwd", h, _ld(h), n, d, _code(h), M, m, w, beta, out, out.stride(0), den, float(a), float(b),
+                gamma, lbeta, int(relu), float(eps), y, y.stride(0), mean, rstd)
+        return out, den, y, mean, rstd
+
+
+def entry(name: str):
+    if not enabled():
+        return None
+    k = graph.K
+    fn = getattr(k, name, None)
+    if fn is None and getattr(k, "name", None) == "hip":
+        fn = getattr(_Hip, name)
+    return fn
```

New measurement: 29.89 million, median of 6. Within noise of the previous version (+0.3%).
